# srv902/FOCUS

Hardware: AMD Instinct MI355X
Metric: clips/sec (fwd+bwd+opt step) ORViT-MF 16x224 (higher is better)
Workload: dtype bf16; 1 GPU; ORViT-Motionformer 16x224, 4 objects, batch=8 per GPU (BASELINE configs[1]); global_batch=8, frames=16, crop=224, objects=4, parallelism=dp1, optimizer=adamw+clipnorm

## Files before the change

### focus_amd/csrc/misc.hip

```cpp
#include "focus_common.h"
#include "focus_debug.h"

namespace {

template <typename T>
__global__ __launch_bounds__(256) void colsum_kernel(const T* __restrict__ x, float* __restrict__ out, int M, int N,
                                                     int64_t ld_, int rows_per_block, int accumulate) {
    __shared__ float red[4][64];
    const int c = blockIdx.x * 64 + (threadIdx.x & 63), r4 = threadIdx.x >> 6;
    const int m_begin = blockIdx.y * rows_per_block;
    const int m_end = min(M, m_begin + rows_per_block);
    float s = 0.f;
    if (c < N)
        for (int m = m_begin + r4; m < m_end; m += 4) s += ld<T>(x + (int64_t)m * ld_ + c);
    red[r4][threadIdx.x & 63] = s;
    __syncthreads();
    if (r4 == 0 && c < N) {
        const int l = threadIdx.x;
        const float t = red[0][l] + red[1][l] + red[2][l] + red[3][l];
        if (gridDim.y == 1 && !accumulate) out[c] = t; else atomicAdd(out + c, t);
    }
}

__global__ __launch_bounds__(256) void colsum_bf16_vec_kernel(const bf16_t* __restrict__ x, float* __restrict__ out,
// ... 118 lines not shown
                                                      const int64_t* __restrict__ target,
                                                      float* __restrict__ loss_rows, float* __restrict__ dlogits, int R,
                                                      int Ncls, float smoothing) {
    __shared__ float red[16];
    const int r = blockIdx.x;
    const float* x = logits + (int64_t)r * Ncls;
    float m = -INFINITY;
    for (int i = threadIdx.x; i < Ncls; i += 256) m = fmaxf(m, x[i]);
    m = block_max(m, red);
    float s = 0.f, sx = 0.f;
    for (int i = threadIdx.x; i < Ncls; i += 256) { s += expf(x[i] - m); sx += x[i]; }
    s = block_sum(s, red);
    sx = block_sum(sx, red);
    const float lse = m + logf(s);
    const int t = (int)target[r];
    const float conf = 1.f - smoothing;
    if (threadIdx.x == 0) {
        const float nll = lse - x[t];
        const float smooth = lse - sx / (float)Ncls;
        loss_rows[r] = conf * nll + smoothing * smooth;
    }
    for (int i = threadIdx.x; i < Ncls; i += 256) {
        const float p = expf(x[i] - lse);
        dlogits[(int64_t)r * Ncls + i] = (p - (i == t ? conf : 0.f) - smoothing / (float)Ncls) / (float)R;
    }
}

__device__ __forceinline__ float sigm(float x) { return 1.f / (1.f + expf(-x)); }
template <typename T>
__global__ void gru_fwd_kernel(T* __restrict__ gi, T* __restrict__ gh, const T* __restrict__ h, T* __restrict__ hn,
                               const float* __restrict__ b_ih, const float* __restrict__ b_hh, int R, int D) {
    const int64_t i = (int64_t)blockIdx.x * blockDim.x + threadIdx.x;
    if (i >= (int64_t)R * D) return;
    const int64_t r = i / D;
    const int c = (int)(i % D);
    T* a = gi + r * 3 * D;
    T* b = gh + r * 3 * D;
    float ar = ld<T>(a + c), az = ld<T>(a + D + c), an = ld<T>(a + 2 * D + c);
    float br = ld<T>(b + c), bz = ld<T>(b + D + c), bn = ld<T>(b + 2 * D + c);
    if (b_ih) {
        ar += b_ih[c]; az += b_ih[D + c]; an += b_ih[2 * D + c];
        br += b_hh[c]; bz += b_hh[D + c]; bn += b_hh[2 * D + c];
        st<T>(a + c, ar); st<T>(a + D + c, az); st<T>(a + 2 * D + c, an);
        st<T>(b + c, br); st<T>(b + D + c, bz); st<T>(b + 2 * D + c, bn);
        ar = ld<T>(a + c); az = ld<T>(a + D + c); an = ld<T>(a + 2 * D + c);
        br = ld<T>(b + c); bz = ld<T>(b + D + c); bn = ld<T>(b + 2 * D + c);
    }
    const float rg = sigm(ar + br);
    const float zg = sigm(az + bz);
    const float ng = tanhf(an + rg * bn);
    st<T>(hn + i, (1.f - zg) * ng + zg * ld<T>(h + i));
}
template <typename T>
__global__ void gru_bwd_kernel(const T* __restrict__ gi, const T* __restrict__ gh, const T* __restrict__ h,
                               const T* __restrict__ dhn, T* __restrict__ dgi, T* __restrict__ dgh,
                               T* __restrict__ dh, T* __restrict__ zero_out, int R, int D) {
    const int64_t i = (int64_t)blockIdx.x * blockDim.x + threadIdx.x;
    if (i >= (int64_t)R * D) return;
    if (zero_out) st<T>(zero_out + i, 0.f);
    const int64_t r = i / D;
    const int c = (int)(i % D);
    const T* a = gi + r * 3 * D;
    const T* b = gh + r * 3 * D;
    const float hn_ = ld<T>(b + 2 * D + c);
    const float rg = sigm(ld<T>(a + c) + ld<T>(b + c));
    const float zg = sigm(ld<T>(a + D + c) + ld<T>(b + D + c));
    const float ng = tanhf(ld<T>(a + 2 * D + c) + rg * hn_);
    const float hv = ld<T>(h + i), g = ld<T>(dhn + i);
    const float dn = g * (1.f - zg), dz = g * (hv - ng);
    const float dpre_n = dn * (1.f - ng * ng);
    const float dr = dpre_n * hn_;
    const float dpre_r = dr * rg * (1.f - rg), dpre_z = dz * zg * (1.f - zg);
    st<T>(dgi + r * 3 * D + c, dpre_r);
    st<T>(dgi + r * 3 * D + D + c, dpre_z);
    st<T>(dgi + r * 3 * D + 2 * D + c, dpre_n);
    st<T>(dgh + r * 3 * D + c, dpre_r);
    st<T>(dgh + r * 3 * D + D + c, dpre_z);
    st<T>(dgh + r * 3 * D + 2 * D + c, dpre_n * rg);
    st<T>(dh + i, g * zg);
}

template <typename T>
__global__ void cell_amax_fwd_kernel(const T* __restrict__ x, T* __restrict__ y, int32_t* __restrict__ arg, int K,
                                     int cells, int C) {
    const int64_t i = (int64_t)blockIdx.x * blockDim.x + threadIdx.x;
    if (i >= (int64_t)K * C) return;
    const int64_t k = i / C;
    const int c = (int)(i % C);
    const T* p = x + k * cells * C + c;
    float m = ld<T>(p);
    int a = 0;
    for (int j = 1; j < cells; ++j) {
        const float v = ld<T>(p + (int64_t)j * C);
        if (v > m) { m = v; a = j; }
    }
    st<T>(y + i, m);
    arg[i] = a;
}
__global__ __launch_bounds__(256) void cell_amax_fwd_vec_kernel(const bf16_t* __restrict__ x, bf16_t* __restrict__ y,
                                                                int32_t* __restrict__ arg, int cells, int C) {
    __shared__ float sm[8][256];
    __shared__ int sa[8][256];
    const int k = blockIdx.y, cb = blockIdx.x * 256;
    const int cg = threadIdx.x & 31, ph = threadIdx.x >> 5;
    const bf16_t* p = x + (int64_t)k * cells * C + cb + cg * 8;
    float m[8];
    int a[8];
#pragma unroll
    for (int e = 0; e < 8; ++e) { m[e] = -INFINITY; a[e] = 0x7fffffff; }
#pragma unroll 5
    for (int j = ph; j < cells; j += 8) {
        const uint4 r = *reinterpret_cast<const uint4*>(p + (int64_t)j * C);
        const float v[8] = {__uint_as_float(r.x << 16), __uint_as_float(r.x & 0xffff0000u), __uint_as_float(r.y << 16),
                            __uint_as_float(r.y & 0xffff0000u), __uint_as_float(r.z << 16), __uint_as_float(r.z & 0xffff0000u),
                            __uint_as_float(r.w << 16), __uint_as_float(r.w & 0xffff0000u)};
#pragma unroll
        for (int e = 0; e < 8; ++e)
            if (v[e] > m[e] || a[e] == 0x7fffffff) { m[e] = v[e]; a[e] = j; }
    }
#pragma unroll
    for (int e = 0; e < 8; ++e) { sm[ph][cg * 8 + e] = m[e]; sa[ph][cg * 8 + e] = a[e]; }
    __syncthreads();
    const int c = threadIdx.x;
    float bm = sm[0][c];
    int ba = sa[0][c];
#pragma unroll
    for (int q = 1; q < 8; ++q) {
        const float vm = sm[q][c];
        const int va = sa[q][c];
        if (va != 0x7fffffff && (ba == 0x7fffffff || vm > bm || (vm == bm && va < ba))) { bm = vm; ba = va; }
    }
    y[(int64_t)k * C + cb + c] = f32_to_bf16(bm);
    arg[(int64_t)k * C + cb + c] = ba == 0x7fffffff ? 0 : ba;
}
template <typename T>
__global__ void cell_amax_bwd_kernel(const T* __restrict__ dy, const int32_t* __restrict__ arg, T* __restrict__ dx,
                                     int K, int cells, int C) {
    const int64_t i = (int64_t)blockIdx.x * blockDim.x + threadIdx.x;
    if (i >= (int64_t)K * cells * C) return;
    const int c = (int)(i % C);
    const int j = (int)((i / C) % cells);
    const int64_t k = i / ((int64_t)C * cells);
    st<T>(dx + i, arg[k * C + c] == j ? ld<T>(dy + k * C + c) : 0.f);
}
__global__ __launch_bounds__(256) void cell_amax_bwd_vec_kernel(const bf16_t* __restrict__ dy, const int32_t* __restrict__ arg,
                                                                bf16_t* __restrict__ dx, int64_t n8, int cells, int C) {
    const int64_t i = (int64_t)blockIdx.x * 256 + threadIdx.x;
    if (i >= n8) return;
    const int c8 = C >> 3;
    const int cg = (int)(i % c8);
    const int j = (int)((i / c8) % cells);
    const int64_t k = i / ((int64_t)c8 * cells);
    const int4 a0 = *reinterpret_cast<const int4*>(arg + k * C + cg * 8);
    const int4 a1 = *reinterpret_cast<const int4*>(arg + k * C + cg * 8 + 4);
    const uint4 g = *reinterpret_cast<const uint4*>(dy + k * C + cg * 8);
    uint4 o;
    o.x = (a0.x == j ? (g.x & 0x0000ffffu) : 0u) | (a0.y == j ? (g.x & 0xffff0000u) : 0u);
    o.y = (a0.z == j ? (g.y & 0x0000ffffu) : 0u) | (a0.w == j ? (g.y & 0xffff0000u) : 0u);
    o.z = (a1.x == j ? (g.z & 0x0000ffffu) : 0u) | (a1.y == j ? (g.z & 0xffff0000u) : 0u);
    o.w = (a1.z == j ? (g.w & 0x0000ffffu) : 0u) | (a1.w == j ? (g.w & 0xffff0000u) : 0u);
    *reinterpret_cast<uint4*>(dx + i * 8) = o;
}

inline unsigned nblk(int64_t n, int per) { return (unsigned)cdiv64(n, per); }

}

#define DISPATCH_T(dtype, EXPR_T)                       \
    do {                                                \
        if ((dtype) == FOCUS_BF16) { typedef bf16_t T; EXPR_T; } \
        else { typedef float T; EXPR_T; }               \
    } while (0)

extern "C" int focus_colsum(const void* x, float* out, int M, int N, int64_t row_stride, int accumulate, int dtype,
                            void* stream) {
    if (!x || !out) return FOCUS_ERR_NULL;
    if (M <= 0 || N <= 0) return FOCUS_OK;
    hipStream_t s = (hipStream_t)stream;
    const bool vec = dtype == FOCUS_BF16 && (N & 7) == 0 && (row_stride & 7) == 0 && focus_aligned(x, 16);
    const bool small = (int64_t)M * N <= (4 << 20);
    const bool one_strip = small || M <= (vec ? 512 : 256);
    if (!accumulate && !one_strip && hipMemsetAsync(out, 0, sizeof(float) * N, s) != hipSuccess) return FOCUS_ERR_LAUNCH;
    if (vec) {
        const int rpb = one_strip ? M : 512;
        hipLaunchKernelGGL(colsum_bf16_vec_kernel, dim3((N + 255) / 256, (M + rpb - 1) / rpb), dim3(256), 0, s,
                           (const bf16_t*)x, out, M, N, row_stride, rpb, accumulate);
        FOCUS_CHECK_LAUNCH();
        return FOCUS_OK;
    }
    const int rpb = one_strip ? M : 256;
    dim3 grid((N + 63) / 64, (M + rpb - 1) / rpb);
    DISPATCH_T(dtype, hipLaunchKernelGGL((colsum_kernel<T>), grid, dim3(256), 0, s, (const T*)x, out, M, N,
                                         row_stride, rpb, accumulate));
    FOCUS_CHECK_LAUNCH();
    return FOCUS_OK;
}

__global__ __launch_bounds__(256) void shadow_refresh_kernel(const focus_shadow_item* __restrict__ items) {
    __shared__ bf16_t tile[64][68];
    const focus_shadow_item it = items[blockIdx.y];
    const int tiles_c = (it.cols + 63) >> 6, tiles_r = (it.rows + 63) >> 6;
    if ((int)blockIdx.x >= tiles_r * tiles_c) return;
    const int tr = blockIdx.x / tiles_c, tc = blockIdx.x - tr * tiles_c;
    const int t = threadIdx.x, lr = t >> 4, lc = (t & 15) * 4;
    bf16_t* dst = static_cast<bf16_t*>(it.dst);
    bf16_t* dstT = static_cast<bf16_t*>(it.dstT);
#pragma unroll
    for (int k = 0; k < 4; ++k) {
        const int r = tr * 64 + lr + 16 * k, c = tc * 64 + lc;
        uint2 o = make_uint2(0, 0);
        if (r < it.rows && c < it.cols) {
            const float4 v = *reinterpret_cast<const float4*>(it.src + (int64_t)r * it.cols + c);
            o.x = (uint32_t)f32_to_bf16(v.x) | ((uint32_t)f32_to_bf16(v.y) << 16);
            o.y = (uint32_t)f32_to_bf16(v.z) | ((uint32_t)f32_to_bf16(v.w) << 16);
            if (dst) *reinterpret_cast<uint2*>(dst + (int64_t)r * it.cols + c) = o;
        }
        *reinterpret_cast<uint2*>(&tile[lr + 16 * k][lc]) = o;
    }
    if (!dstT) return;
    __syncthreads();
#pragma unroll
    for (int k = 0; k < 4; ++k) {
        const int oc = tc * 64 + lr + 16 * k, orr = tr * 64 + lc;
        if (oc < it.cols && orr < it.rows) {
            uint2 o;
            o.x = (uint32_t)tile[lc + 0][lr + 16 * k] | ((uint32_t)tile[lc + 1][lr + 16 * k] << 16);
            o.y = (uint32_t)tile[lc + 2][lr + 16 * k] | ((uint32_t)tile[lc + 3][lr + 16 * k] << 16);
            *reinterpret_cast<uint2*>(dstT + (int64_t)oc * it.rows + orr) = o;
        }
    }
}

extern "C" int focus_shadow_refresh(const focus_shadow_item* items, int n_items, int max_rows, int max_cols, void* stream) {
    if (!items) return FOCUS_ERR_NULL;
    if (n_items <= 0) return FOCUS_OK;
    if (n_items > 65535 || max_rows <= 0 || max_cols <= 0) return FOCUS_ERR_SHAPE;
    const int tiles = ((max_rows + 63) / 64) * ((max_cols + 63) / 64);
    hipLaunchKernelGGL(shadow_refresh_kernel, dim3(tiles, n_items), dim3(256), 0, (hipStream_t)stream, items);
// ... 29 lines not shown
    dim3 grid((Cc + 63) / 64, (unsigned)cdiv64(dst_ld, 64), batch);
    if (grid.y > 65535) return FOCUS_ERR_SHAPE;
#define TP(TS, TD) hipLaunchKernelGGL((transpose_pad_kernel<TS, TD>), grid, dim3(256), 0, s, (const TS*)src, src_ld, src_bs, (TD*)dst, dst_ld, dst_bs, R, Cc)
    if (sd == FOCUS_F32 && dd == FOCUS_F32) TP(float, float);
    else if (sd == FOCUS_F32 && dd == FOCUS_BF16) TP(float, bf16_t);
    else if (sd == FOCUS_BF16 && dd == FOCUS_BF16) TP(bf16_t, bf16_t);
    else TP(bf16_t, float);
#undef TP
    FOCUS_CHECK_LAUNCH();
    return FOCUS_OK;
}

extern "C" int focus_diag_gather(const void* xt, void* xdiag, int B, int S, int F, int C, int dtype, void* stream) {
    if (!xt || !xdiag) return FOCUS_ERR_NULL;
    if ((C & 3) || F <= 0 || S % F) return FOCUS_ERR_SHAPE;
    const int64_t rows = (int64_t)B * S;
    DISPATCH_T(dtype, hipLaunchKernelGGL((diag_gather_kernel<T>), dim3(nblk(rows * C / 4, 256)), dim3(256), 0,
                                         (hipStream_t)stream, (const T*)xt, (T*)xdiag, rows, S, F, S / F, C));
    FOCUS_CHECK_LAUNCH();
    return FOCUS_OK;
}
extern "C" int focus_diag_scatter_add(const void* dxdiag, void* dxt, int B, int S, int F, int C, int dtype,
                                      void* stream) {
    if (!dxdiag || !dxt) return FOCUS_ERR_NULL;
    if ((C & 3) || F <= 0 || S % F) return FOCUS_ERR_SHAPE;
    const int64_t rows = (int64_t)B * S;
    DISPATCH_T(dtype, hipLaunchKernelGGL((diag_scatter_add_kernel<T>), dim3(nblk(rows * C / 4, 256)), dim3(256), 0,
                                         (hipStream_t)stream, (const T*)dxdiag, (T*)dxt, rows, S, F, S / F, C));
    FOCUS_CHECK_LAUNCH();
    return FOCUS_OK;
}

extern "C" int focus_im2col_patches(const float* x, void* cols, int B, int Cin, int Tn, int H, int W, int kt, int kh,
                                    int kw, int dtype, void* stream) {
    if (!x || !cols) return FOCUS_ERR_NULL;
    if (kt <= 0 || kh <= 0 || kw <= 0 || Tn % kt || H % kh || W % kw || (kw & 3) || (W & 3)) return FOCUS_ERR_SHAPE;
    if (!focus_aligned(x, 16)) return FOCUS_ERR_ALIGN;
    const int64_t total = (int64_t)B * (Tn / kt) * (H / kh) * (W / kw) * Cin * kt * kh * kw / 4;
    DISPATCH_T(dtype, hipLaunchKernelGGL((im2col_kernel<T>), dim3(nblk(total, 256)), dim3(256), 0,
                                         (hipStream_t)stream, x, (T*)cols, B, Cin, Tn, H, W, kt, kh, kw));
    FOCUS_CHECK_LAUNCH();
    return FOCUS_OK;
}

extern "C" int focus_embed_assemble(const void* patch, const float* cls, const float* pos, const float* temp,
                                    void* tokens, int B, int Tn, int P, int C, int dtype, void* stream) {
    if (!patch || !cls || !pos || !temp || !tokens) return FOCUS_ERR_NULL;
    if (C & 3) return FOCUS_ERR_SHAPE;
    const int64_t total = (int64_t)B * (1 + (int64_t)Tn * P) * C / 4;
    DISPATCH_T(dtype, hipLaunchKernelGGL((embed_assemble_kernel<T>), dim3(nblk(total, 256)), dim3(256), 0,
                                         (hipStream_t)stream, (const T*)patch, cls, pos, temp, (T*)tokens, B, Tn, P, C));
    FOCUS_CHECK_LAUNCH();
    return FOCUS_OK;
}

extern "C" int focus_xent_ls(const float* logits, const int64_t* target, float* loss_rows, float* dlogits, int R,
                             int Ncls, float smoothing, void* stream) {
    if (!logits || !target || !loss_rows || !dlogits) return FOCUS_ERR_NULL;
    if (R <= 0 || Ncls <= 0) return FOCUS_ERR_SHAPE;
    hipLaunchKernelGGL(xent_ls_kernel, dim3(R), dim3(256), 0, (hipStream_t)stream, logits, target, loss_rows, dlogits,
                       R, Ncls, smoothing);
    FOCUS_CHECK_LAUNCH();
    return FOCUS_OK;
}

extern "C" int focus_gru_gates_fwd(void* gi, void* gh, const void* h, void* hn, const float* b_ih, const float* b_hh, int R,
                                   int D, int dtype, void* stream) {
    if (!gi || !gh || !h || !hn || (!b_ih != !b_hh)) return FOCUS_ERR_NULL;
    DISPATCH_T(dtype, hipLaunchKernelGGL((gru_fwd_kernel<T>), dim3(nblk((int64_t)R * D, 256)), dim3(256), 0,
                                         (hipStream_t)stream, (T*)gi, (T*)gh, (const T*)h, (T*)hn, b_ih, b_hh, R, D));
    FOCUS_CHECK_LAUNCH();
    return FOCUS_OK;
}
extern "C" int focus_gru_gates_bwd(const void* gi, const void* gh, const void* h, const void* dhn, void* dgi,
                                   void* dgh, void* dh, void* zero_out, int R, int D, int dtype, void* stream) {
    if (!gi || !gh || !h || !dhn || !dgi || !dgh || !dh) return FOCUS_ERR_NULL;
    DISPATCH_T(dtype, hipLaunchKernelGGL((gru_bwd_kernel<T>), dim3(nblk((int64_t)R * D, 256)), dim3(256), 0,
                                         (hipStream_t)stream, (const T*)gi, (const T*)gh, (const T*)h, (const T*)dhn,
                                         (T*)dgi, (T*)dgh, (T*)dh, (T*)zero_out, R, D));
    FOCUS_CHECK_LAUNCH();
    return FOCUS_OK;
}

extern "C" int focus_cell_amax_fwd(const void* x, void* y, int32_t* arg, int K, int cells, int C, int dtype,
                                   void* stream) {
    if (!x || !y || !arg) return FOCUS_ERR_NULL;
    if (cells <= 0) return FOCUS_ERR_SHAPE;
    if (K <= 0) return FOCUS_OK;
    if (dtype == FOCUS_BF16 && (C & 255) == 0 && K <= 65535 && focus_aligned(x, 16)) {
        hipLaunchKernelGGL(cell_amax_fwd_vec_kernel, dim3(C / 256, K), dim3(256), 0, (hipStream_t)stream, (const bf16_t*)x,
                           (bf16_t*)y, arg, cells, C);
        FOCUS_CHECK_LAUNCH();
        return FOCUS_OK;
    }
    DISPATCH_T(dtype, hipLaunchKernelGGL((cell_amax_fwd_kernel<T>), dim3(nblk((int64_t)K * C, 256)), dim3(256), 0,
                                         (hipStream_t)stream, (const T*)x, (T*)y, arg, K, cells, C));
    FOCUS_CHECK_LAUNCH();
    return FOCUS_OK;
}
extern "C" int focus_cell_amax_bwd(const void* dy, const int32_t* arg, void* dx, int K, int cells, int C, int dtype,
                                   void* stream) {
    if (!dy || !arg || !dx) return FOCUS_ERR_NULL;
    if (K <= 0 || cells <= 0) return FOCUS_OK;
    if (dtype == FOCUS_BF16 && (C & 7) == 0 && focus_aligned(dy, 16) && focus_aligned(dx, 16) && focus_aligned(arg, 16)) {
        const int64_t n8 = (int64_t)K * cells * (C >> 3);
        hipLaunchKernelGGL(cell_amax_bwd_vec_kernel, dim3(nblk(n8, 256)), dim3(256), 0, (hipStream_t)stream,
                           (const bf16_t*)dy, arg, (bf16_t*)dx, n8, cells, C);
        FOCUS_CHECK_LAUNCH();
        return FOCUS_OK;
    }
    DISPATCH_T(dtype, hipLaunchKernelGGL((cell_amax_bwd_kernel<T>), dim3(nblk((int64_t)K * cells * C, 256)),
                                         dim3(256), 0, (hipStream_t)stream, (const T*)dy, arg, (T*)dx, K, cells, C));
    FOCUS_CHECK_LAUNCH();
    return FOCUS_OK;
}

template <typename T>
__global__ void scale_add_kernel(const T* __restrict__ x, const T* __restrict__ y, const float* __restrict__ scale,
                                 float keep, T* __restrict__ out, int64_t total, int64_t per) {
    const int64_t i = ((int64_t)blockIdx.x * blockDim.x + threadIdx.x) * 8;
    if (i >= total) return;
    float sc = scale[i / per];
    if (keep > 0.f) sc = __fdiv_rn(floorf(__fadd_rn(keep, sc)), keep);
    float a[8] = {0.f, 0.f, 0.f, 0.f, 0.f, 0.f, 0.f, 0.f}, b[8];
    ld8<T>(y + i, b);
    if (x) ld8<T>(x + i, a);
#pragma unroll
    for (int e = 0; e < 8; ++e) a[e] += sc * b[e];
    st8<T>(out + i, a);
}
extern "C" int focus_scale_add(const void* x, const void* y, const float* scale, float keep, void* out, int B,
                               int64_t per, int dtype, void* stream) {
    if (!y || !scale || !out) return FOCUS_ERR_NULL;
    if (B <= 0 || per <= 0) return FOCUS_OK;
    if (per & 7) return FOCUS_ERR_SHAPE;
    if (!focus_aligned(y, 16) || !focus_aligned(out, 16) || (x && !focus_aligned(x, 16))) return FOCUS_ERR_ALIGN;
    const int64_t total = (int64_t)B * per;
    DISPATCH_T(dtype, hipLaunchKernelGGL((scale_add_kernel<T>), dim3(nblk(total / 8, 256)), dim3(256), 0,
                                         (hipStream_t)stream, (const T*)x, (const T*)y, scale, keep, (T*)out, total, per));
    FOCUS_CHECK_LAUNCH();
    return FOCUS_OK;
}

typedef __attribute__((ext_vector_type(4))) short s16x4;
__global__ void tr16_probe_kernel(int16_t* out) {
    __shared__ __attribute__((aligned(16))) int16_t img[16 * 64];
    for (int i = threadIdx.x; i < 16 * 64; i += 64) img[i] = (int16_t)(100 * (i / 64) + (i % 64));
    __syncthreads();
    const int l = threadIdx.x, g = l >> 4, q = (l & 15) >> 2, pp = l & 3;
    auto* ptr = (__attribute__((address_space(3))) s16x4*)(img + (4 * g + q) * 64 + 4 * pp);
    const s16x4 v = __builtin_amdgcn_ds_read_tr16_b64_v4i16(ptr);
    for (int i = 0; i < 4; ++i) out[l * 4 + i] = v[i];
}
extern "C" int focus_debug_tr16_probe(int16_t* out, void* stream) {
    if (!out) return FOCUS_ERR_NULL;
    hipLaunchKernelGGL(tr16_probe_kernel, dim3(1), dim3(64), 0, (hipStream_t)stream, out);
    FOCUS_CHECK_LAUNCH();
    return FOCUS_OK;
}

static const char* kErr[] = {"ok", "bad shape", "unsupported dtype", "misaligned pointer or stride",
                             "HIP launch failure", "null pointer", "workspace too small"};
extern "C" const char* focus_strerror(int status) {
    const int i = -status;
    return (i >= 0 && i <= 6) ? kErr[i] : "unknown focus status";
}
extern "C" int focus_abi_version(void) { return 2; }
```

### focus_amd/csrc/orvit_tokens.hip

```cpp
#include "focus_common.h"

namespace {

struct RowMap { int b, t, p; bool cls; };
__device__ __forceinline__ RowMap map_all_row(int64_t r, int T, int HW, int O) {
    const int per = 1 + T * (HW + O);
    RowMap m;
    m.b = (int)(r / per);
    const int lr = (int)(r - (int64_t)m.b * per);
    m.cls = lr == 0;
    m.t = m.cls ? 0 : (lr - 1) / (HW + O);
    m.p = m.cls ? 0 : (lr - 1) - m.t * (HW + O);
    return m;
}

template <bool FWD>
__global__ __launch_bounds__(256) void orvit_assemble_kernel(const uint4* __restrict__ a, const uint4* __restrict__ o_in,
                                                             uint4* __restrict__ out_a, uint4* __restrict__ out_o, int64_t npieces,
                                                             int vpr, int T, int HW, int O) {
    const int64_t i = (int64_t)blockIdx.x * 256 + threadIdx.x;
    if (i >= npieces) return;
    const int64_t r = i / vpr;
    const int v = (int)(i - r * vpr);
    const RowMap m = map_all_row(r, T, HW, O);
    const int64_t xrow = (int64_t)m.b * (1 + T * HW) + (m.cls ? 0 : 1 + m.t * HW + m.p);
    const int64_t orow = ((int64_t)m.b * T + m.t) * O + (m.p - HW);
    const bool is_obj = !m.cls && m.p >= HW;
    if (FWD) out_a[i] = is_obj ? o_in[orow * vpr + v] : a[xrow * vpr + v];
    else if (is_obj) out_o[orow * vpr + v] = a[i];
    else out_a[xrow * vpr + v] = a[i];
}

template <typename T> struct Vec;
template <> struct Vec<float> { static constexpr int N = 4; };
template <> struct Vec<bf16_t> { static constexpr int N = 8; };
template <typename T> __device__ __forceinline__ void unpack(const uint4& r, float* v);
template <> __device__ __forceinline__ void unpack<float>(const uint4& r, float* v) {
    v[0] = __uint_as_float(r.x); v[1] = __uint_as_float(r.y); v[2] = __uint_as_float(r.z); v[3] = __uint_as_float(r.w);
}
template <> __device__ __forceinline__ void unpack<bf16_t>(const uint4& r, float* v) {
    v[0] = __uint_as_float(r.x << 16); v[1] = __uint_as_float(r.x & 0xffff0000u);
    v[2] = __uint_as_float(r.y << 16); v[3] = __uint_as_float(r.y & 0xffff0000u);
    v[4] = __uint_as_float(r.z << 16); v[5] = __uint_as_float(r.z & 0xffff0000u);
    v[6] = __uint_as_float(r.w << 16); v[7] = __uint_as_float(r.w & 0xffff0000u);
}
template <typename T> __device__ __forceinline__ uint4 pack(const float* v);
template <> __device__ __forceinline__ uint4 pack<float>(const float* v) {
    return make_uint4(__float_as_uint(v[0]), __float_as_uint(v[1]), __float_as_uint(v[2]), __float_as_uint(v[3]));
}
template <> __device__ __forceinline__ uint4 pack<bf16_t>(const float* v) {
    uint4 o;
    o.x = (uint32_t)f32_to_bf16(v[0]) | ((uint32_t)f32_to_bf16(v[1]) << 16);
    o.y = (uint32_t)f32_to_bf16(v[2]) | ((uint32_t)f32_to_bf16(v[3]) << 16);
    o.z = (uint32_t)f32_to_bf16(v[4]) | ((uint32_t)f32_to_bf16(v[5]) << 16);
    o.w = (uint32_t)f32_to_bf16(v[6]) | ((uint32_t)f32_to_bf16(v[7]) << 16);
    return o;
}

template <typename T>
__global__ __launch_bounds__(256) void orvit_merge_kernel(const uint4* __restrict__ x, const uint4* __restrict__ y,
                                                          const uint4* __restrict__ mm, const float* __restrict__ scale,
                                                          uint4* __restrict__ out, int64_t npieces, int vpr, int Tn, int HW,
                                                          int O) {
    const int64_t i = (int64_t)blockIdx.x * 256 + threadIdx.x;
    if (i >= npieces) return;
    const int64_t r = i / vpr;
    const int v = (int)(i - r * vpr);
    const int per = 1 + Tn * HW;
    const int b = (int)(r / per), lr = (int)(r - (int64_t)b * per);
    const int t = lr ? (lr - 1) / HW : 0, p = lr ? (lr - 1) - t * HW : 0;
    const int64_t yrow = (int64_t)b * (1 + Tn * (HW + O)) + (lr ? 1 + t * (HW + O) + p : 0);
    constexpr int N = Vec<T>::N;
    float xv[N], yv[N];
    unpack<T>(x[i], xv);
    unpack<T>(y[yrow * vpr + v], yv);
    if (mm && lr) {
        float mv[N];
        unpack<T>(mm[((int64_t)b * Tn * HW + (lr - 1)) * vpr + v], mv);
#pragma unroll
        for (int e = 0; e < N; ++e) yv[e] += mv[e];
    }
    const float s = scale ? scale[b] : 1.f;
#pragma unroll
    for (int e = 0; e < N; ++e) xv[e] = fmaf(s, yv[e], xv[e]);
    out[i] = pack<T>(xv);
}

template <typename T>
__global__ __launch_bounds__(256) void orvit_merge_bwd_kernel(const uint4* __restrict__ dout, const float* __restrict__ scale,
                                                              uint4* __restrict__ dy, uint4* __restrict__ dmm, int64_t npieces,
                                                              int vpr, int Tn, int HW, int O) {
    const int64_t i = (int64_t)blockIdx.x * 256 + threadIdx.x;
    if (i >= npieces) return;
    const int64_t r = i / vpr;
    const int v = (int)(i - r * vpr);
    const RowMap m = map_all_row(r, Tn, HW, O);
    if (!m.cls && m.p >= HW) { dy[i] = make_uint4(0, 0, 0, 0); return; }
    const int lr = m.cls ? 0 : 1 + m.t * HW + m.p;
    uint4 g = dout[((int64_t)m.b * (1 + Tn * HW) + lr) * vpr + v];
    if (scale) {
        constexpr int N = Vec<T>::N;
        float gv[N];
        unpack<T>(g, gv);
        const float s = scale[m.b];
#pragma unroll
        for (int e = 0; e < N; ++e) gv[e] *= s;
        g = pack<T>(gv);
    }
    dy[i] = g;
    if (dmm && lr) dmm[((int64_t)m.b * Tn * HW + (lr - 1)) * vpr + v] = g;
}

inline int64_t cdiv(int64_t a, int64_t b) { return (a + b - 1) / b; }
inline int esize(int dtype) { return dtype == FOCUS_BF16 ? 2 : 4; }
inline bool shape_ok(int B, int T, int HW, int O, int C, int dtype) {
    return B > 0 && T > 0 && HW > 0 && O >= 0 && C > 0 && (dtype == FOCUS_BF16 || dtype == FOCUS_F32) && (C * esize(dtype)) % 16 == 0 &&
           (int64_t)B * (1 + (int64_t)T * (HW + O)) * C < (1LL << 40);
}

}

extern "C" int focus_orvit_assemble(const void* x, const void* obj, void* all, int B, int T, int HW, int O, int C, int dtype,
                                    void* stream) {
    if (!x || !all || (O > 0 && !obj)) return FOCUS_ERR_NULL;
    if (!shape_ok(B, T, HW, O, C, dtype)) return FOCUS_ERR_SHAPE;
    if (!focus_aligned(x, 16) || !focus_aligned(all, 16) || (obj && !focus_aligned(obj, 16))) return FOCUS_ERR_ALIGN;
    const int vpr = C * esize(dtype) / 16;
    const int64_t n = (int64_t)B * (1 + (int64_t)T * (HW + O)) * vpr;
    hipLaunchKernelGGL((orvit_assemble_kernel<true>), dim3((unsigned)cdiv(n, 256)), dim3(256), 0, (hipStream_t)stream,
                       (const uint4*)x, (const uint4*)obj, (uint4*)all, (uint4*)nullptr, n, vpr, T, HW, O);
    FOCUS_CHECK_LAUNCH();
    return FOCUS_OK;
}

extern "C" int focus_orvit_assemble_bwd(const void* dall, void* dx, void* dobj, int B, int T, int HW, int O, int C, int dtype,
                                        void* stream) {
    if (!dall || !dx || (O > 0 && !dobj)) return FOCUS_ERR_NULL;
    if (!shape_ok(B, T, HW, O, C, dtype)) return FOCUS_ERR_SHAPE;
    if (!focus_aligned(dall, 16) || !focus_aligned(dx, 16) || (dobj && !focus_aligned(dobj, 16))) return FOCUS_ERR_ALIGN;
    const int vpr = C * esize(dtype) / 16;
    const int64_t n = (int64_t)B * (1 + (int64_t)T * (HW + O)) * vpr;
    hipLaunchKernelGGL((orvit_assemble_kernel<false>), dim3((unsigned)cdiv(n, 256)), dim3(256), 0, (hipStream_t)stream,
                       (const uint4*)dall, (const uint4*)nullptr, (uint4*)dx, (uint4*)dobj, n, vpr, T, HW, O);
    FOCUS_CHECK_LAUNCH();
    return FOCUS_OK;
}

extern "C" int focus_orvit_merge(const void* x, const void* y, const void* mm, const float* scale, void* out, int B, int T,
                                 int HW, int O, int C, int dtype, void* stream) {
    if (!x || !y || !out) return FOCUS_ERR_NULL;
    if (!shape_ok(B, T, HW, O, C, dtype)) return FOCUS_ERR_SHAPE;
    if (!focus_aligned(x, 16) || !focus_aligned(y, 16) || !focus_aligned(out, 16) || (mm && !focus_aligned(mm, 16)))
        return FOCUS_ERR_ALIGN;
    const int vpr = C * esize(dtype) / 16;
    const int64_t n = (int64_t)B * (1 + (int64_t)T * HW) * vpr;
    const dim3 grid((unsigned)cdiv(n, 256));
    if (dtype == FOCUS_BF16)
        hipLaunchKernelGGL((orvit_merge_kernel<bf16_t>), grid, dim3(256), 0, (hipStream_t)stream, (const uint4*)x, (const uint4*)y,
                           (const uint4*)mm, scale, (uint4*)out, n, vpr, T, HW, O);
    else
        hipLaunchKernelGGL((orvit_merge_kernel<float>), grid, dim3(256), 0, (hipStream_t)stream, (const uint4*)x, (const uint4*)y,
                           (const uint4*)mm, scale, (uint4*)out, n, vpr, T, HW, O);
    FOCUS_CHECK_LAUNCH();
    return FOCUS_OK;
}

extern "C" int focus_orvit_merge_bwd(const void* dout, const float* scale, void* dy, void* dmm, int B, int T, int HW, int O,
                                     int C, int dtype, void* stream) {
    if (!dout || !dy) return FOCUS_ERR_NULL;
    if (!shape_ok(B, T, HW, O, C, dtype)) return FOCUS_ERR_SHAPE;
    if (!focus_aligned(dout, 16) || !focus_aligned(dy, 16) || (dmm && !focus_aligned(dmm, 16))) return FOCUS_ERR_ALIGN;
    const int vpr = C * esize(dtype) / 16;
    const int64_t n = (int64_t)B * (1 + (int64_t)T * (HW + O)) * vpr;
    const dim3 grid((unsigned)cdiv(n, 256));
    if (dtype == FOCUS_BF16)
        hipLaunchKernelGGL((orvit_merge_bwd_kernel<bf16_t>), grid, dim3(256), 0, (hipStream_t)stream, (const uint4*)dout, scale,
                           (uint4*)dy, (uint4*)dmm, n, vpr, T, HW, O);
    else
        hipLaunchKernelGGL((orvit_merge_bwd_kernel<float>), grid, dim3(256), 0, (hipStream_t)stream, (const uint4*)dout, scale,
                           (uint4*)dy, (uint4*)dmm, n, vpr, T, HW, O);
    FOCUS_CHECK_LAUNCH();
    return FOCUS_OK;
}
```

### focus_amd/csrc/traj_time2.hip

```cpp
#include "focus_common.h"
#include <cstdlib>
#include "traj_internal.h"

namespace {

typedef __attribute__((ext_vector_type(8))) __bf16 bf16x8;
typedef __attribute__((ext_vector_type(4))) float f32x4;

constexpr int CH = 64;
constexpr int TQ = 16;
constexpr int MAXH = 16;

union Pk4 { uint2 u; bf16_t e[4]; };

__device__ __forceinline__ void unpack8(const uint4& r, float* v) {
    v[0] = __uint_as_float(r.x << 16); v[1] = __uint_as_float(r.x & 0xffff0000u);
    v[2] = __uint_as_float(r.y << 16); v[3] = __uint_as_float(r.y & 0xffff0000u);
    v[4] = __uint_as_float(r.z << 16); v[5] = __uint_as_float(r.z & 0xffff0000u);
    v[6] = __uint_as_float(r.w << 16); v[7] = __uint_as_float(r.w & 0xffff0000u);
}
__device__ __forceinline__ uint4 pack8(const float* v) {
    uint4 o;
    o.x = (uint32_t)f32_to_bf16(v[0]) | ((uint32_t)f32_to_bf16(v[1]) << 16);
    o.y = (uint32_t)f32_to_bf16(v[2]) | ((uint32_t)f32_to_bf16(v[3]) << 16);
// ... 346 lines not shown
#pragma unroll
        for (int i = 0; i < NFR; ++i) {
            const int fi = min(w + 8 * i, FT - 1);
#pragma unroll
            for (int ks = 0; ks < 2; ++ks) xf[i][ks] = *reinterpret_cast<const bf16x8*>(sx + (16 * fi + col) * XP + (32 * ks + 8 * kg) * 2);
#pragma unroll
            for (int j = 0; j < QPF; ++j)
#pragma unroll
                for (int ks = 0; ks < 2; ++ks)
                    ub[i][j][ks] = *reinterpret_cast<const bf16x8*>(sU + (QPF * fi + j) * urow + hl * FWD_HP + (32 * ks + 8 * kg) * 2);
        }
        QFrag<NHW> qf;
        read_q(qf, k ^ 1);
        lds_barrier();
        asm volatile("s_waitcnt vmcnt(%0)" ::"n"(LG) : "memory");
        __builtin_amdgcn_sched_barrier(0);
        pin_pre(pre[k]);
        stash(pre[k], k);
        asm volatile("" ::: "memory");
        pin_pre(pre[k]);
        issue(pre[k], t + 4);
        if (it + 1 < niter) compute_u_tile<UPW, false>(wf, qf, sUb + (k ^ 1) * (TQ * urow), urow, heads, w, lane);
#pragma unroll
        for (int i = 0; i < NFR; ++i) {
            f32x4 acc[QPF];
#pragma unroll
            for (int j = 0; j < QPF; ++j) {
                acc[j] = (f32x4){0.f, 0.f, 0.f, 0.f};
#pragma unroll
                for (int ks = 0; ks < 2; ++ks)
                    acc[j] = __builtin_amdgcn_mfma_f32_16x16x32_bf16(xf[i][ks], ub[i][j][ks], acc[j], 0, 0, 0);
            }
            f32x4 v = acc[0];
#pragma unroll
            for (int j = 1; j < QPF; ++j)
                if ((4 * kg) / FT == j) v = acc[j];
            const int fi = w + 8 * i;
            const int jq = (4 * kg) / FT, f0 = (4 * kg) % FT;
            const int row = row0 + QPF * fi + jq;
            if (fi < FT && row < rows && col < heads) {
                float4 o = make_float4(v[0] * scale, v[1] * scale, v[2] * scale, v[3] * scale);
                *reinterpret_cast<float4*>(slab + (((int64_t)cc * rows + row) * heads + col) * FT + f0) = o;
            }
        }
        lds_barrier();
      }
    }
    asm volatile("s_waitcnt vmcnt(0)" ::: "memory");
}

template <int FT>
__global__ __launch_bounds__(256) void time2_softmax_kernel(const float* __restrict__ slab, float* __restrict__ attn2,
                                                            int64_t n, int nchunk) {
    const int64_t i = (int64_t)blockIdx.x * 256 + threadIdx.x;
    if (i >= n) return;
    float lg[FT];
#pragma unroll
    for (int f = 0; f < FT; ++f) lg[f] = 0.f;
#pragma unroll 4
    for (int c = 0; c < nchunk; ++c) {
        const float4* p = reinterpret_cast<const float4*>(slab + ((int64_t)c * n + i) * FT);
#pragma unroll
        for (int f4 = 0; f4 < FT / 4; ++f4) {
            const float4 v = p[f4];
            lg[4 * f4] += v.x; lg[4 * f4 + 1] += v.y; lg[4 * f4 + 2] += v.z; lg[4 * f4 + 3] += v.w;
        }
    }
    float m = -INFINITY;
#pragma unroll
    for (int f = 0; f < FT; ++f) m = fmaxf(m, lg[f]);
    float den = 0.f;
#pragma unroll
    for (int f = 0; f < FT; ++f) { lg[f] = __expf(lg[f] - m); den += lg[f]; }
    const float inv = 1.f / den;
    float4* o = reinterpret_cast<float4*>(attn2 + i * FT);
#pragma unroll
    for (int f4 = 0; f4 < FT / 4; ++f4)
        o[f4] = make_float4(lg[4 * f4] * inv, lg[4 * f4 + 1] * inv, lg[4 * f4 + 2] * inv, lg[4 * f4 + 3] * inv);
}

template <int FT>
__global__ __launch_bounds__(256) void time2_out_kernel(const bf16_t* __restrict__ xt, const float* __restrict__ attn2,
                                                        bf16_t* __restrict__ out, int64_t obs, int64_t ngroups, int S,
                                                        int heads) {
    const int64_t gi = (int64_t)blockIdx.x * 256 + threadIdx.x;
    const bool act = gi < ngroups;
    const int64_t g = act ? gi : ngroups - 1;
    const int gpr = heads * 8;
    const int row = (int)(g / gpr);
    const int cg = (int)(g - (int64_t)row * gpr);
    const int C = gpr * 8;
    uint4 xr[FT];
#pragma unroll
    for (int f = 0; f < FT; ++f) xr[f] = *reinterpret_cast<const uint4*>(xt + (((int64_t)row * FT + f) * C) + cg * 8);
    const float* arow = attn2 + ((int64_t)row * heads + (cg >> 3)) * FT;
    float o[8] = {0.f, 0.f, 0.f, 0.f, 0.f, 0.f, 0.f, 0.f};
#pragma unroll
    for (int f = 0; f < FT; ++f) {
        const float a = arow[f];
        float xv[8];
        unpack8(xr[f], xv);
#pragma unroll
        for (int e = 0; e < 8; ++e) o[e] = fmaf(a, xv[e], o[e]);
    }
    const int b = row / S, s = row - b * S;
    if (act) *reinterpret_cast<uint4*>(out + b * obs + (int64_t)s * C + cg * 8) = pack8(o);
}

template <int FT>
__global__ __launch_bounds__(256) void time2_dlg_kernel(const bf16_t* __restrict__ xt, const float* __restrict__ attn2,
                                                        const bf16_t* __restrict__ dout, int64_t dobs,
                                                        bf16_t* __restrict__ dl, bf16_t* __restrict__ gout, int rows,
                                                        int S, int HEADS, int RPB, float scale) {
    const int GPR = HEADS * 8, C = HEADS * CH;
    __shared__ float sdl[32][FT][MAXH];
    const int tid = threadIdx.x, rl = min(tid / GPR, RPB - 1), cg = tid - (tid / GPR) * GPR, h = cg >> 3;
    const int row_raw = blockIdx.x * RPB + rl;
    const bool act = row_raw < rows && tid < RPB * GPR;
    const int row = act ? row_raw : rows - 1;
    const int b = row / S, s = row - b * S;
    uint4 xr[FT];
#pragma unroll
    for (int f = 0; f < FT; ++f) xr[f] = *reinterpret_cast<const uint4*>(xt + (((int64_t)row * FT + f) * C) + cg * 8);
    float gv[8];
    unpack8(*reinterpret_cast<const uint4*>(dout + b * dobs + (int64_t)s * C + cg * 8), gv);
    const float* arow = attn2 + ((int64_t)row * HEADS + h) * FT;
    float a[FT], da[FT], dot = 0.f;
#pragma unroll
    for (int f = 0; f < FT; ++f) {
        a[f] = arow[f];
        float xv[8];
        unpack8(xr[f], xv);
        float p = 0.f;
#pragma unroll
        for (int e = 0; e < 8; ++e) p = fmaf(gv[e], xv[e], p);
        da[f] = sum8lanes(p);
        dot = fmaf(a[f], da[f], dot);
    }
    if (tid < RPB * GPR && (cg & 7) == 0) {
#pragma unroll
        for (int f = 0; f < FT; ++f) sdl[rl][f][h] = scale * a[f] * (da[f] - dot);
    }
    if (tid < RPB * GPR && cg < MAXH - HEADS) {
#pragma unroll
        for (int f = 0; f < FT; ++f) sdl[rl][f][HEADS + cg] = 0.f;
    }
    __syncthreads();
    if (act) {
        for (int pc = cg; pc < FT * 2; pc += GPR) {
            const int f = pc >> 1, h0 = (pc & 1) * 8;
            float v[8];
#pragma unroll
            for (int k = 0; k < 8; ++k) v[k] = sdl[rl][f][h0 + k];
            *reinterpret_cast<uint4*>(dl + ((int64_t)row * FT + f) * MAXH + h0) = pack8(v);
        }
    }
    float xv[FT][8];
#pragma unroll
    for (int f = 0; f < FT; ++f) unpack8(xr[f], xv[f]);
    for (int hh = 0; hh < HEADS; ++hh) {
        float g8[8] = {0.f, 0.f, 0.f, 0.f, 0.f, 0.f, 0.f, 0.f};
#pragma unroll
        for (int f = 0; f < FT; ++f) {
            const float d = sdl[rl][f][hh];
#pragma unroll
            for (int k = 0; k < 8; ++k) g8[k] = fmaf(d, xv[f][k], g8[k]);
        }
        if (act) *reinterpret_cast<uint4*>(gout + ((int64_t)hh * rows + row) * C + cg * 8) = pack8(g8);
    }
// ... 269 lines not shown
        QFrag<NHW> qf;
        read_q(qf, k ^ 1);
        lds_barrier();
        asm volatile("s_waitcnt vmcnt(%0)" ::"n"(NQP + 2 * NX) : "memory");
        __builtin_amdgcn_sched_barrier(0);
        pin_pq(pq[k]);
        stash_q(pq[k], k);
        asm volatile("" ::: "memory");
        pin_pq(pq[k]);
        issue_q(pq[k], t + 4);
        asm volatile("s_waitcnt vmcnt(%0)" ::"n"(2 * NQP + NX) : "memory");
        __builtin_amdgcn_sched_barrier(0);
        pin_d(dr[k]);
        if (it + 1 < niter) compute_u_tile<UPW, true>(wf, qf, smem + (k ^ 1) * (TQ * BWD_UROW), 0, heads, w, lane);
        uint4 o[NNT][2];
#pragma unroll
        for (int i = 0; i < NNT; ++i) {
            f32x4 acc[4];
#pragma unroll
            for (int mt = 0; mt < 4; ++mt) acc[mt] = (f32x4){0.f, 0.f, 0.f, 0.f};
#pragma unroll
            for (int ks = 0; ks < KS; ++ks) {
                const int jp = QPF >= 2 ? (kg & 1) + 2 * ks : 0;
                const bool keep = QPF >= 2 ? jp == j : kg < 2;
                bf16x8 bfr = dr[k].dl[i];
#pragma unroll
                for (int e = 0; e < 8; ++e) bfr[e] = keep ? bfr[e] : (__bf16)0.f;
#pragma unroll
                for (int mt = 0; mt < 4; ++mt)
                    acc[mt] = __builtin_amdgcn_mfma_f32_16x16x32_bf16(af[i][ks][mt].v, bfr, acc[mt], 0, 0, 0);
            }
            float dv[16], v[16];
            unpack8(*reinterpret_cast<const uint4*>(&dr[k].dout[i][0]), dv);
            unpack8(*reinterpret_cast<const uint4*>(&dr[k].dout[i][1]), dv + 8);
            const float av = dr[k].a[i];
#pragma unroll
            for (int mt = 0; mt < 4; ++mt)
#pragma unroll
                for (int r = 0; r < 4; ++r) v[4 * mt + r] = fmaf(av, dv[4 * mt + r], acc[mt][r]);
            o[i][0] = pack8(v);
            o[i][1] = pack8(v + 8);
            pin(o[i][0]); pin(o[i][1]);
        }
        asm volatile("" ::: "memory");
        pin_d(dr[k]);
        load_d(dr[k], t + 2);
#pragma unroll
        for (int i = 0; i < NNT; ++i) {
            const int nt = w + 8 * i;
            const int row = row0 + QPF * nt + j;
            if (nt < FT && row < rows) {
                uint4* dp = reinterpret_cast<uint4*>(dxt + ((int64_t)row * FT + f) * C + cc * CH + 16 * kg);
                dp[0] = o[i][0];
                dp[1] = o[i][1];
            }
        }
        lds_barrier();
      }
    }
    asm volatile("s_waitcnt vmcnt(0)" ::: "memory");
}

int spread_mode() {
    static const int v = getenv("FOCUS_T2_SPREAD") ? atoi(getenv("FOCUS_T2_SPREAD")) : 0;
    return v;
}

size_t time2_lds_fwd(int heads) { return (size_t)2 * TQ * fwd_urow(heads); }
size_t time2_lds_bwd() { return (size_t)2 * TQ * BWD_UROW; }

}

bool focus_traj_time2_ok(int F, int heads, int d, int dtype) {
    static const bool enabled = !(getenv("FOCUS_TIME2") && atoi(getenv("FOCUS_TIME2")) == 0);
    return enabled && dtype == FOCUS_BF16 && d == CH && heads >= 1 && heads <= MAXH && (F == 4 || F == 8 || F == 16) &&
           time2_lds_fwd(heads) <= 160 * 1024;
}

extern "C" size_t focus_traj_time2_workspace_bytes(int B, int S, int F, int heads, int d) {
    if (B <= 0 || S <= 0 || F <= 0 || heads <= 0 || d != CH) return 0;
    return (size_t)heads * B * heads * S * F * sizeof(float);
}

extern "C" int focus_traj_time2_fwd(const void* q2, const void* xt, const void* wkT, int64_t ldw, void* out,
                                    int64_t out_bstride, float* attn2, void* ws, size_t ws_bytes, int B, int S, int F,
                                    int heads, int d, int dtype, void* stream) {
    if (!q2 || !xt || !wkT || !out || !attn2 || !ws) return FOCUS_ERR_NULL;
    if (B <= 0 || S <= 0 || !focus_traj_time2_ok(F, heads, d, dtype)) return FOCUS_ERR_SHAPE;
    const int C = heads * CH;
    const int64_t rows = (int64_t)B * S;
    if (ldw < C || (ldw & 7) || (out_bstride & 7) || out_bstride < (int64_t)S * C || rows * F * C > 0x7fffffffLL * 8)
        return FOCUS_ERR_SHAPE;
    if (!focus_aligned(q2, 16) || !focus_aligned(xt, 16) || !focus_aligned(wkT, 16) || !focus_aligned(out, 16) ||
        !focus_aligned(ws, 16) || !focus_aligned(attn2, 16))
        return FOCUS_ERR_ALIGN;
    if (ws_bytes < focus_traj_time2_workspace_bytes(B, S, F, heads, d)) return FOCUS_ERR_WORKSPACE;
    hipStream_t s = (hipStream_t)stream;
    const int nchunk = C / CH;
    const float scale = 1.f / sqrtf((float)d);
    const int upw = (2 * heads + 7) / 8;
    static const bool staged_on = !(getenv("FOCUS_T2_LDS") && atoi(getenv("FOCUS_T2_LDS")) == 0);
    const bool staged = staged_on && F <= 8 && time2_lds_staged(heads, F) <= 160 * 1024;
    const size_t lds = staged ? time2_lds_staged(heads, F) : time2_lds_fwd(heads);
#define TL(FT, UPW) do { \
        if (staged) { \
            static bool once_s = (hipFuncSetAttribute((const void*)time2_logits_lds_kernel<FT, UPW>, hipFuncAttributeMaxDynamicSharedMemorySize, 160 * 1024) == hipSuccess); \
            (void)once_s; \
            hipLaunchKernelGGL((time2_logits_lds_kernel<FT, UPW>), dim3(256), dim3(512), lds, s, (const bf16_t*)q2, (const bf16_t*)xt, (const bf16_t*)wkT, ldw, (float*)ws, (int)rows, heads, scale, spread_mode()); \
            break; } \
        static bool once = (hipFuncSetAttribute((const void*)time2_logits_kernel<FT, UPW>, hipFuncAttributeMaxDynamicSharedMemorySize, 160 * 1024) == hipSuccess); \
        (void)once; \
        hipLaunchKernelGGL((time2_logits_kernel<FT, UPW>), dim3(256), dim3(512), lds, s, (const bf16_t*)q2, (const bf16_t*)xt, (const bf16_t*)wkT, ldw, (float*)ws, (int)rows, heads, scale, spread_mode()); } while (0)
#define TLU(FT) do { if (upw == 1) TL(FT, 1); else if (upw == 2) TL(FT, 2); else if (upw == 3) TL(FT, 3); else TL(FT, 4); } while (0)
    if (F == 8) TLU(8); else if (F == 4) TLU(4); else TLU(16);
#undef TLU
#undef TL
    FOCUS_CHECK_LAUNCH();
    const int64_t n = rows * heads;
#define TS(FT) hipLaunchKernelGGL((time2_softmax_kernel<FT>), dim3((unsigned)cdiv64(n, 256)), dim3(256), 0, s, (const float*)ws, attn2, n, nchunk)
    if (F == 8) TS(8); else if (F == 4) TS(4); else TS(16);
#undef TS
    FOCUS_CHECK_LAUNCH();
    const int64_t ng = rows * heads * 8;
    dim3 gv((unsigned)cdiv64(ng, 256));
#define TO(FT) hipLaunchKernelGGL((time2_out_kernel<FT>), gv, dim3(256), 0, s, (const bf16_t*)xt, attn2, (bf16_t*)out, out_bstride, ng, S, heads)
    if (F == 8) TO(8); else if (F == 4) TO(4); else TO(16);
#undef TO
    FOCUS_CHECK_LAUNCH();
    return FOCUS_OK;
}

extern "C" int focus_traj_time2_bwd(const void* q2, const void* xt, const void* wkT, int64_t ldw, const float* attn2,
                                    const void* dout, int64_t dout_bstride, void* dxt, void* g, void* dl, int B, int S,
                                    int F, int heads, int d, int dtype, void* stream) {
    if (!q2 || !xt || !wkT || !attn2 || !dout || !dxt || !g || !dl) return FOCUS_ERR_NULL;
    if (B <= 0 || S <= 0 || !focus_traj_time2_ok(F, heads, d, dtype)) return FOCUS_ERR_SHAPE;
    const int C = heads * CH;
    const int64_t rows = (int64_t)B * S;
    if (ldw < C || (ldw & 7) || (dout_bstride & 7) || dout_bstride < (int64_t)S * C || rows * F * C > 0x7fffffffLL * 8)
        return FOCUS_ERR_SHAPE;
    if (!focus_aligned(q2, 16) || !focus_aligned(xt, 16) || !focus_aligned(wkT, 16) || !focus_aligned(dout, 16) ||
        !focus_aligned(dxt, 16) || !focus_aligned(g, 16) || !focus_aligned(dl, 16))
        return FOCUS_ERR_ALIGN;
    hipStream_t s = (hipStream_t)stream;
    const int nchunk = C / CH;
    const float scale = 1.f / sqrtf((float)d);
    {
        const int gpr = heads * 8, rpb = 256 / gpr;
        dim3 gd((unsigned)cdiv64(rows, rpb));
#define TD(FT) hipLaunchKernelGGL((time2_dlg_kernel<FT>), gd, dim3(256), 0, s, (const bf16_t*)xt, attn2, (const bf16_t*)dout, dout_bstride, (bf16_t*)dl, (bf16_t*)g, (int)rows, S, heads, rpb, scale)
        if (F == 8) TD(8); else if (F == 4) TD(4); else TD(16);
#undef TD
        FOCUS_CHECK_LAUNCH();
    }
    const int upw = (2 * heads + 7) / 8;
    static const bool staged_on = !(getenv("FOCUS_T2_LDS") && atoi(getenv("FOCUS_T2_LDS")) == 0);
    const size_t lds_staged = time2_lds_bwd() + (size_t)2 * TQ * q_pitch(heads);
    const bool staged = staged_on && lds_staged <= 160 * 1024 && !(upw == 4 && F != 8);
    const size_t lds = staged ? lds_staged : time2_lds_bwd();
#define TB(FT, UPW) do { \
        if constexpr (!((UPW) == 4 && (FT) != 8)) if (staged) { \
            static bool once_s = (hipFuncSetAttribute((const void*)time2_dx_lds_kernel<FT, UPW>, hipFuncAttributeMaxDynamicSharedMemorySize, 160 * 1024) == hipSuccess); \
            (void)once_s; \
            hipLaunchKernelGGL((time2_dx_lds_kernel<FT, UPW>), dim3(256), dim3(512), lds, s, (const bf16_t*)q2, (const bf16_t*)wkT, ldw, attn2, (const bf16_t*)dl, (const bf16_t*)dout, dout_bstride, (bf16_t*)dxt, (int)rows, S, heads, spread_mode()); \
            break; } \
        static bool once = (hipFuncSetAttribute((const void*)time2_dx_kernel<FT, UPW>, hipFuncAttributeMaxDynamicSharedMemorySize, 160 * 1024) == hipSuccess); \
        (void)once; \
        hipLaunchKernelGGL((time2_dx_kernel<FT, UPW>), dim3(256), dim3(512), lds, s, (const bf16_t*)q2, (const bf16_t*)wkT, ldw, attn2, (const bf16_t*)dl, (const bf16_t*)dout, dout_bstride, (bf16_t*)dxt, (int)rows, S, heads, spread_mode()); } while (0)
#define TBU(FT) do { if (upw == 1) TB(FT, 1); else if (upw == 2) TB(FT, 2); else if (upw == 3) TB(FT, 3); else TB(FT, 4); } while (0)
    if (F == 8) TBU(8); else if (F == 4) TBU(4); else TBU(16);
#undef TBU
#undef TB
    FOCUS_CHECK_LAUNCH();
    return FOCUS_OK;
}
```

### focus_amd/csrc/traj_time2_gw.hip

```cpp
#include "focus_common.h"
#include <algorithm>

namespace {

typedef __attribute__((ext_vector_type(8))) __bf16 bf16x8;
typedef __attribute__((ext_vector_type(4))) short s16x4;
typedef __attribute__((ext_vector_type(4))) float f32x4;
typedef __attribute__((address_space(3))) s16x4 lds_s16x4;

constexpr int HD = 64, TR = 32;
constexpr int C_ = 768;
constexpr int NSUB = C_ / 128;
constexpr int GT_BYTES = TR * C_ * 2, QT_BYTES = TR * HD * 2, STAGE = GT_BYTES + QT_BYTES;

union Frag { bf16x8 v; s16x4 t[2]; uint4 u; };

__device__ __forceinline__ int offb(int row, int ch) { return 256 * row + 16 * (ch ^ (((row & 3) << 2) | ((row >> 2) & 3))); }

__device__ __forceinline__ bf16x8 tr_frag_g(const char* sub, int r0, int c0, int lane) {
    const int i = lane & 15, q = i >> 2, p = i & 3;
    const int ch = (c0 >> 3) + (p >> 1), bo = 8 * (p & 1);
    Frag f;
    f.t[0] = __builtin_amdgcn_ds_read_tr16_b64_v4i16((lds_s16x4*)(sub + offb(r0 + q, ch) + bo));
    f.t[1] = __builtin_amdgcn_ds_read_tr16_b64_v4i16((lds_s16x4*)(sub + offb(r0 + 4 + q, ch) + bo));
// ... 22 lines not shown

    bf16x8 wf[C_ / 32];
    {
        const bf16_t* wrow = wk + (int64_t)(h * HD + nbq * 16 + row16_) * wk_ld + kq_ * 8;
#pragma unroll
        for (int ks = 0; ks < C_ / 32; ++ks) wf[ks] = *reinterpret_cast<const bf16x8*>(wrow + ks * 32);
    }
    f32x4 accw[4][6];
#pragma unroll
    for (int a = 0; a < 4; ++a)
#pragma unroll
        for (int j = 0; j < 6; ++j) accw[a][j] = (f32x4){0.f, 0.f, 0.f, 0.f};
    asm volatile("s_waitcnt vmcnt(0)" ::: "memory");
#pragma unroll
    for (int ks = 0; ks < C_ / 32; ++ks) asm volatile("" : "+v"(wf[ks]));

    const uint32_t sm_a = lds_addr_of(smem);
    auto dma = [&](int t, int st) __attribute__((always_inline)) {
        const int64_t r0 = (int64_t)t * TR;
        const uint32_t base = sm_a + st * STAGE;
#pragma unroll
        for (int j = 0; j < 6; ++j) {
            const int p = w * 6 + j, sub = p >> 3, rg = p & 7;
            const int row = rg * 4 + (lane >> 4), pos = lane & 15;
            const int ch = pos ^ (((row & 3) << 2) | ((row >> 2) & 3));
            glds16(gh + (r0 + row) * C_ + sub * 128 + ch * 8, __builtin_amdgcn_readfirstlane(base + sub * 8192 + rg * 1024));
        }
        if (w < 4) {
            const int row = w * 8 + (lane >> 3);
            glds16(q2 + (r0 + row) * (int64_t)(heads * HD) + h * HD + (lane & 7) * 8,
                   __builtin_amdgcn_readfirstlane(base + GT_BYTES + w * 1024));
        }
    };
    if (t_begin >= t_end) return;
    dma(t_begin, 0);
    int st = 0;
    for (int t = t_begin; t < t_end; ++t) {
        const bool more = t + 1 < t_end;
        if (more) dma(t + 1, st ^ 1);
        if (more) { if (w < 4) asm volatile("s_waitcnt vmcnt(7)" ::: "memory"); else asm volatile("s_waitcnt vmcnt(6)" ::: "memory"); }
        else asm volatile("s_waitcnt vmcnt(0)" ::: "memory");
        __builtin_amdgcn_s_barrier();
        const char* gt = smem + st * STAGE;
        const char* qt = gt + GT_BYTES;
        int lane_o = lane;
        asm volatile("" : "+v"(lane_o));
        const int row16 = lane_o & 15, kq = lane_o >> 4;
        f32x4 accq = {0.f, 0.f, 0.f, 0.f};
#pragma unroll
        for (int ks = 0; ks < C_ / 32; ++ks) {
            const int col = ks * 32 + kq * 8;
            const bf16x8 af = *reinterpret_cast<const bf16x8*>(gt + (col >> 7) * 8192 + offb(mb * 16 + row16, (col & 127) >> 3));
            accq = __builtin_amdgcn_mfma_f32_16x16x32_bf16(af, wf[ks], accq, 0, 0, 0);
        }
        {
            bf16_t* o = dq2 + ((int64_t)t * TR + mb * 16 + kq * 4) * (heads * HD) + h * HD + nbq * 16 + row16;
#pragma unroll
            for (int r = 0; r < 4; ++r) o[(int64_t)r * (heads * HD)] = f32_to_bf16(accq[r]);
        }
#pragma unroll
        for (int j = 0; j < 6; ++j) {
            const int c = w * 96 + j * 16;
            const bf16x8 gb = tr_frag_g(gt + (c >> 7) * 8192, 8 * kq, c & 127, lane_o);
#pragma unroll
            for (int a = 0; a < 4; ++a) {
                const bf16x8 qa = tr_frag_q(qt, 8 * kq, a * 16, lane_o);
                accw[a][j] = __builtin_amdgcn_mfma_f32_16x16x32_bf16(qa, gb, accw[a][j], 0, 0, 0);
            }
        }
        asm volatile("s_waitcnt lgkmcnt(0)" ::: "memory");
        __builtin_amdgcn_s_barrier();
        st ^= 1;
    }
    float* out = slabs + ((int64_t)sp * heads * HD + h * HD) * C_;
#pragma unroll
    for (int a = 0; a < 4; ++a)
#pragma unroll
        for (int j = 0; j < 6; ++j)
#pragma unroll
            for (int r = 0; r < 4; ++r) out[(int64_t)(a * 16 + kq_ * 4 + r) * C_ + w * 96 + j * 16 + row16_] = accw[a][j][r];
}

__global__ __launch_bounds__(256) void time2_gw_reduce_kernel(const float* __restrict__ slabs, float* __restrict__ dwk, int64_t n4,
                                                              int splits) {
    const int64_t i = (int64_t)blockIdx.x * 256 + threadIdx.x;
    if (i >= n4) return;
    float4 s = reinterpret_cast<const float4*>(slabs)[i];
#pragma unroll 4
    for (int k = 1; k < splits; ++k) {
        const float4 v = reinterpret_cast<const float4*>(slabs)[(int64_t)k * n4 + i];
        s.x += v.x; s.y += v.y; s.z += v.z; s.w += v.w;
    }
    reinterpret_cast<float4*>(dwk)[i] = s;
}

int gw_splits(int R, int heads) {
    const int tiles = R / TR;
    return std::max(1, std::min(tiles, 256 / std::max(heads, 1)));
}

}

extern "C" int focus_traj_time2_gw_ok(int R, int heads, int d, int dtype) {
    return dtype == FOCUS_BF16 && d == HD && heads * d == C_ && R >= TR && R % TR == 0;
}

extern "C" size_t focus_traj_time2_gw_workspace_bytes(int R, int heads, int d) {
    if (!focus_traj_time2_gw_ok(R, heads, d, FOCUS_BF16)) return 0;
    return (size_t)gw_splits(R, heads) * C_ * C_ * sizeof(float);
}

extern "C" int focus_traj_time2_gw(const void* g, const void* q2, const void* wk, int64_t wk_ld, void* dq2, float* dwk, void* ws,
                                   size_t ws_bytes, int R, int heads, int d, int dtype, void* stream) {
    if (!g || !q2 || !wk || !dq2 || !dwk || !ws) return FOCUS_ERR_NULL;
    if (!focus_traj_time2_gw_ok(R, heads, d, dtype) || (wk_ld & 7)) return FOCUS_ERR_SHAPE;
    if (!focus_aligned(g, 16) || !focus_aligned(q2, 16) || !focus_aligned(wk, 16) || !focus_aligned(dwk, 16)) return FOCUS_ERR_ALIGN;
    if (ws_bytes < focus_traj_time2_gw_workspace_bytes(R, heads, d)) return FOCUS_ERR_WORKSPACE;
    hipStream_t s = static_cast<hipStream_t>(stream);
    const int splits = gw_splits(R, heads), tiles = R / TR;
    const int tps = (tiles + splits - 1) / splits;
    const int used = (tiles + tps - 1) / tps;
    auto k = time2_gw_kernel;
    const size_t lds = 2 * (size_t)STAGE;
    static bool once = (hipFuncSetAttribute((const void*)k, hipFuncAttributeMaxDynamicSharedMemorySize, lds) == hipSuccess);
    (void)once;
    hipLaunchKernelGGL(k, dim3(used, heads), dim3(512), lds, s, (const bf16_t*)g, (const bf16_t*)q2, (const bf16_t*)wk, wk_ld,
                       (bf16_t*)dq2, (float*)ws, R, heads, tps);
    FOCUS_CHECK_LAUNCH();
    const int64_t n4 = (int64_t)C_ * C_ / 4;
    hipLaunchKernelGGL(time2_gw_reduce_kernel, dim3((unsigned)cdiv64(n4, 256)), dim3(256), 0, s, (const float*)ws, dwk, n4, used);
    FOCUS_CHECK_LAUNCH();
    return FOCUS_OK;
}
```

### focus_amd/ops.py

```python
import ctypes
import weakref

import torch

from . import _lib
from ._lib import BF16, F32, GemmDesc

EPI_NONE, EPI_GELU, EPI_RELU, EPI_TANH = _lib.EPI_NONE, _lib.EPI_GELU, _lib.EPI_RELU, _lib.EPI_TANH
_DEPI = {EPI_GELU: _lib.EPI_DGELU, EPI_RELU: _lib.EPI_DRELU, EPI_TANH: _lib.EPI_DTANH}


def _dt(t):
    if t.dtype == torch.float32:
        return F32
    if t.dtype == torch.bfloat16:
        return BF16
    raise RuntimeError("focus_amd: unsupported dtype %s (float32 or bfloat16)" % t.dtype)


def _need_gpu(*ts):
    for t in ts:
        if t is not None and not t.is_cuda:
            raise RuntimeError("focus_amd: the hot path runs on the MI355X only (got a %s tensor); "
                               "there is no CPU fallback" % t.device)
# ... 33 lines not shown
    d.batch0, d.batch1 = batch
    (ta, oa), (tb, ob), (tc, oc) = A, B, C
    d.A, d.B, d.C = _p(ta, oa).value, _p(tb, ob).value, _p(tc, oc).value
    d.rsA, d.csA, d.bsA0, d.bsA1 = sA
    d.rsB, d.csB, d.bsB0, d.bsB1 = sB
    d.rsC, d.csC, d.bsC0, d.bsC1 = sC
    d.bias = bias.data_ptr() if bias is not None else None
    d.residual = (residual[0].data_ptr() + residual[1] * residual[0].element_size()) if residual is not None else None
    d.aux = (aux[0].data_ptr() + aux[1] * aux[0].element_size()) if aux is not None else None
    d.alpha = alpha
    d.accumulate = int(accumulate)
    d.epilogue = epilogue
    d.dtype_ab = _dt(ta)
    d.dtype_c = _dt(tc)
    if b_scale is not None:
        assert tb.dtype == torch.uint8 and ta.dtype == torch.bfloat16, "fp8 weights go with bf16 activations"
        d.dtype_b = _lib.FP8_E4M3
        d.b_scale = b_scale.data_ptr()
    else:
        assert ta.dtype == tb.dtype
    kind = _mfma_path(ta, sA, sB, K) if GEMM_TIMING is not None else None
    if kind:
        e0, e1 = torch.cuda.Event(enable_timing=True), torch.cuda.Event(enable_timing=True)
        e0.record()
        _lib.check(_lib.lib().focus_gemm(ctypes.byref(d), _stream()), "gemm")
        e1.record()
        if kind == "nt" and _lib.lib().focus_gemm_last_kernel() == 2:
            kind = "nt_ws8" if b_scale is not None else "nt_ws"
        GEMM_TIMING.append((2.0 * M * N * K * batch[0] * batch[1], e0, e1, kind, (M, N, K, batch[0] * batch[1], epilogue)))
        return
    _lib.check(_lib.lib().focus_gemm(ctypes.byref(d), _stream()), "gemm")


def mm_nt(a, b, bias=None, residual=None, aux=None, epilogue=EPI_NONE, out_dtype=None, alpha=1.0, out=None, b_scale=None):
    M, K = a.shape
    N = b.shape[0]
    c = out if out is not None else torch.empty(M, N, device=a.device, dtype=out_dtype or a.dtype)
    gemm(M, N, K, (a, 0), (a.stride(0), 1, 0, 0), (b, 0), (1, b.stride(0), 0, 0), (c, 0), (N, 1, 0, 0),
         bias=bias, residual=(residual, 0) if residual is not None else None,
         aux=(aux, 0) if aux is not None else None, alpha=alpha, epilogue=epilogue, b_scale=b_scale)
    return c


def mm_nn(a, b, aux=None, epilogue=EPI_NONE, alpha=1.0):
    M, K = a.shape
    N = b.shape[1]
    c = torch.empty(M, N, device=a.device, dtype=a.dtype)
    gemm(M, N, K, (a, 0), (a.stride(0), 1, 0, 0), (b, 0), (b.stride(0), 1, 0, 0), (c, 0), (N, 1, 0, 0),
         aux=(aux, 0) if aux is not None else None, epilogue=epilogue, alpha=alpha)
    return c


def transpose_pad(x, pad_to=64, dtype=None):
    R, Cc = x.shape
    Rp = (R + pad_to - 1) // pad_to * pad_to
    out = torch.empty(Cc, Rp, device=x.device, dtype=dtype or x.dtype)
    _lib.check(_lib.lib().focus_transpose_pad(_p(x), _dt(x), x.stride(0), 0, _p(out), _dt(out), Rp, 0, R, Cc, 1,
                                              _stream()), "transpose_pad")
    return out


def mm_tn(a, b):
    M, N = a.shape
    K = b.shape[1]
    if a.dtype == torch.bfloat16 and USE_TN_GEMM and N % 8 == 0 and K % 8 == 0 and N >= 8 and K >= 8:
        c = torch.empty(N, K, device=a.device, dtype=torch.float32)
        nb = _lib.lib().focus_gemm_tn_workspace_bytes(N, K, M)
        ws = torch.empty(nb // 4, device=a.device, dtype=torch.float32)
        gemm(N, K, M, (a, 0), (1, a.stride(0), 0, 0), (b, 0), (b.stride(0), 1, 0, 0), (c, 0), (K, 1, 0, 0),
             aux=(ws, 0))
    elif a.dtype == torch.bfloat16:
        at, bt = transpose_pad(a), transpose_pad(b)
        Mp = at.shape[1]
        c = torch.zeros(N, K, device=a.device, dtype=torch.float32)
        gemm(N, K, Mp, (at, 0), (Mp, 1, 0, 0), (bt, 0), (1, Mp, 0, 0), (c, 0), (K, 1, 0, 0), accumulate=True)
    else:
        c = torch.empty(N, K, device=a.device, dtype=torch.float32)
        gemm(N, K, M, (a, 0), (1, a.stride(0), 0, 0), (b, 0), (b.stride(0), 1, 0, 0), (c, 0), (K, 1, 0, 0))
    return c


import os as _os


def wgrad_async(dy, x, want_bias):
    dw, db = linear_wgrad(dy, x, want_bias)
    return dw, db, None


def linear_wgrad(dy, x, want_bias):
    M, N = dy.shape
    K = x.shape[1]
    ok = (dy.dtype == torch.bfloat16 and USE_TN_GEMM and N % 8 == 0 and K % 8 == 0 and N >= 8 and K >= 8
          and dy.stride(1) == 1 and x.stride(1) == 1 and dy.stride(0) % 8 == 0 and x.stride(0) % 8 == 0)
    if not ok:
        return mm_tn(dy, x), (colsum(dy) if want_bias else None)
    L = _lib.lib()
    dw = torch.empty(N, K, device=dy.device, dtype=torch.float32)
    db = torch.empty(N, device=dy.device, dtype=torch.float32) if want_bias else None
    nb = L.focus_linear_wgrad_workspace_bytes(N, K, M)
    ws = torch.empty(max(nb, 16) // 4, device=dy.device, dtype=torch.float32)
    if GEMM_TIMING is not None:
        e0, e1 = torch.cuda.Event(enable_timing=True), torch.cuda.Event(enable_timing=True)
        e0.record()
    _lib.check(L.focus_linear_wgrad(_p(dy), _p(x), _p(dw), _p(db) if want_bias else None, _p(ws), nb, M, N, K,
                                    dy.stride(0), x.stride(0), _dt(dy), _stream()), "linear_wgrad")
    if GEMM_TIMING is not None:
        e1.record()
        GEMM_TIMING.append((2.0 * M * N * K, e0, e1, "tn", (N, K, M, 1, 0)))
    return dw, db


def colsum(x):
    M, N = x.shape
    out = torch.empty(N, device=x.device, dtype=torch.float32)
    _lib.check(_lib.lib().focus_colsum(_p(x), _p(out), M, N, x.stride(0), 0, _dt(x), _stream()), "colsum")
    return out


def cast(x, dtype):
    if x.dtype == dtype:
        return x
    x = x.contiguous()
    out = torch.empty(x.shape, device=x.device, dtype=dtype)
    _lib.check(_lib.lib().focus_cast(_p(x), _dt(x), _p(out), _dt(out), x.numel(), _stream()), "cast")
    return out


_shadow_cache = {}
_shadow_gen = 0
_shadow_epoch = 0


def shadow_epoch():
    return _shadow_epoch


def invalidate_shadows():
    global _shadow_gen
    _shadow_gen += 1
    _refresh_shadows_batched()
    if _stacked:
        refresh_stacked()
    if _fp8_cache:
        refresh_fp8_shadows()


_shadow_tables = {}


def _refresh_shadows_batched():
    import numpy as np
    by_dev = {}
    for key, (ref, stamp, out) in list(_shadow_cache.items()):
        w = ref()
        if w is None or key[1] != torch.bfloat16 or w.dtype != torch.float32 or w.dim() != 2 or not w.is_cuda:
            continue
        if w.shape[0] % 4 or w.shape[1] % 4 or not w.is_contiguous() or w.data_ptr() % 16:
            continue
        by_dev.setdefault(w.device, {}).setdefault(id(w), [w, None, None])[2 if key[2] else 1] = (key, out)
    for dev, ws in by_dev.items():
        sig = tuple((i, e[0].data_ptr(), e[1][1].data_ptr() if e[1] else 0, e[2][1].data_ptr() if e[2] else 0)
                    for i, e in sorted(ws.items()))
        tab = _shadow_tables.get(dev)
        if tab is None or tab[0] != sig:
            rec = np.zeros((len(sig), 4), dtype=np.int64)
            mr = mc = 0
            for n, (i, sp, dp, tp) in enumerate(sig):
                w = ws[i][0]
                rec[n, 0], rec[n, 1], rec[n, 2] = sp, dp, tp
                rec[n, 3] = int(w.shape[0]) | (int(w.shape[1]) << 32)
                mr, mc = max(mr, w.shape[0]), max(mc, w.shape[1])
            tab = (sig, torch.from_numpy(rec).to(dev), mr, mc)
            _shadow_tables[dev] = tab
        with torch.cuda.device(dev):
            _lib.check(_lib.lib().focus_shadow_refresh(_p(tab[1]), len(sig), tab[2], tab[3], _stream()), "shadow_refresh")
        for e in ws.values():
            w = e[0]
            for slot in (e[1], e[2]):
                if slot is not None:
                    key, out = slot
                    _shadow_cache[key] = (_shadow_cache[key][0], (w._version, w.data_ptr(), _shadow_gen), out)


def cached_shadow(w, dtype, transposed):
    hit = _shadow_cache.get((id(w), dtype, transposed))
    if hit is not None and hit[0]() is w:
        return hit[2]
    return None


def shadows_written(entries):
    global _shadow_gen
    _shadow_gen += 1
    for w, dst, dstT in entries:
        for out, tr in ((dst, False), (dstT, True)):
            if out is None:
                continue
            key = (id(w), torch.bfloat16, tr)
            hit = _shadow_cache.get(key)
            if hit is not None and hit[2] is out:
                _shadow_cache[key] = (hit[0], (w._version, w.data_ptr(), _shadow_gen), out)
    if _stacked:
        refresh_stacked()
    if _fp8_cache:
        refresh_fp8_shadows()


def drop_caches():
    global _shadow_epoch
    _shadow_epoch += 1
    _shadow_cache.clear()
    _shadow_tables.clear()
    _stacked.clear()
    _fp8_cache.clear()
    _fp8_tables.clear()


def shadow(w, dtype, transposed=False):
    w = getattr(w, "_focus_base", w)
    if dtype == torch.float32 and not transposed:
        return w.detach()
    key = (id(w), dtype, transposed)
    hit = _shadow_cache.get(key)
    if hit is not None and hit[0]() is w and hit[1] == (w._version, w.data_ptr(), _shadow_gen):
        return hit[2]
    wd = w.detach()
    if transposed:
        N, K = wd.shape
        out = torch.empty(K, N, device=w.device, dtype=dtype)
        _lib.check(_lib.lib().focus_transpose_pad(_p(wd), _dt(wd), K, 0, _p(out), _dt(out), N, 0, N, K, 1, _stream()),
                   "shadow^T")
    else:
        out = cast(wd, dtype)
    global _shadow_epoch
    _shadow_epoch += 1
    _shadow_cache[key] = (weakref.ref(w, lambda _r, k=key: _shadow_cache.pop(k, None)),
                          (w._version, w.data_ptr(), _shadow_gen), out)
    return out


FP8_WEIGHTS = False
_FP8_MIN_ROWS = 1024
_fp8_cache = {}
_fp8_tables = {}


class fp8_weights:
    def __init__(self, on=True):
        self.on = bool(on)

    def __enter__(self):
        global FP8_WEIGHTS
        self.prev = FP8_WEIGHTS
        FP8_WEIGHTS = self.on
        return self

    def __exit__(self, *exc):
        global FP8_WEIGHTS
        FP8_WEIGHTS = self.prev
        return False


def fp8_ok(w, rows, dtype):
    w = getattr(w, "_focus_base", w)
    return (FP8_WEIGHTS and dtype == torch.bfloat16 and w.dim() == 2 and w.dtype == torch.float32 and w.is_cuda
            and rows >= _FP8_MIN_ROWS and w.shape[0] % 64 == 0 and w.shape[1] % 64 == 0 and w.is_contiguous()
            and w.data_ptr() % 16 == 0)


def _fp8_run(dev, entries):
    import numpy as np
    sig = tuple((e[2].data_ptr(), e[3].data_ptr(), e[4].data_ptr(), w.data_ptr()) for w, e in entries)
    tab = _fp8_tables.get(dev)
    if tab is None or tab[0] != sig:
        rec = np.zeros((len(entries), 5), dtype=np.int64)
        mr = mc = 0
        for n, (w, e) in enumerate(entries):
            rec[n, 0], rec[n, 1], rec[n, 2], rec[n, 3] = w.data_ptr(), e[2].data_ptr(), e[3].data_ptr(), e[4].data_ptr()
            rec[n, 4] = int(w.shape[0]) | (int(w.shape[1]) << 32)
            mr, mc = max(mr, w.shape[0]), max(mc, w.shape[1])
        tab = (sig, torch.from_numpy(rec).to(dev), mr, mc, torch.empty(len(entries), dtype=torch.int32, device=dev))
        if len(entries) > 1:
            _fp8_tables[dev] = tab
    with torch.cuda.device(dev):
        _lib.check(_lib.lib().focus_fp8_refresh(_p(tab[1]), len(entries), tab[2], tab[3], _p(tab[4]), _stream()), "fp8_refresh")
    for w, e in entries:
        e[1] = (w._version, w.data_ptr(), _shadow_gen)


def refresh_fp8_shadows():
    by_dev = {}
    for key, e in list(_fp8_cache.items()):
        w = e[0]()
        if w is None:
            _fp8_cache.pop(key, None)
            continue
        by_dev.setdefault(w.device, []).append((w, e))
    for dev, entries in by_dev.items():
        _fp8_run(dev, entries)


def shadow_fp8(w, transposed=False):
    w = getattr(w, "_focus_base", w)
    e = _fp8_cache.get(id(w))
    if e is None or e[0]() is not w:
        N, K = w.shape
        e = _fp8_cache[id(w)] = [weakref.ref(w, lambda _r, k=id(w): _fp8_cache.pop(k, None)), None,
                                 torch.empty(N, K, dtype=torch.uint8, device=w.device),
                                 torch.empty(K, N, dtype=torch.uint8, device=w.device),
                                 torch.empty(1, dtype=torch.float32, device=w.device)]
        _fp8_tables.pop(w.device, None)
    if e[1] != (w._version, w.data_ptr(), _shadow_gen):
        _fp8_run(w.device, [(w.detach(), e)])
        e[1] = (w._version, w.data_ptr(), _shadow_gen)
    return (e[3] if transposed else e[2]), e[4]

# ... 843 lines not shown
        B, S, F_, C = xt.shape
        dout = dout.contiguous()
        dq2, dk2, dxt = torch.empty_like(q2), torch.empty_like(k2), torch.empty_like(xt)
        _lib.check(_lib.lib().focus_traj_time_bwd(_p(q2), _p(k2), _p(xt), _p(attn2), _p(dout), S * C, _p(dq2), _p(dk2),
                                                  _p(dxt), 0, B, S, F_, ctx.heads, C // ctx.heads, _dt(xt),
                                                  _stream()), "traj_time_bwd")
        return dq2, dk2, dxt, None


def traj_time(q2, k2, xt, heads):
    return _TrajTimeFn.apply(q2, k2, xt, heads)


class _TrajTimeBlockFn(torch.autograd.Function):

    @staticmethod
    def forward(ctx, q2, xt, w_kv, b_kv, cls_out, heads):
        _need_gpu(q2, xt, w_kv)
        q2, xt = q2.contiguous(), xt.contiguous()
        B, S, F_, C = xt.shape
        d = C // heads
        wk = shadow(w_kv, xt.dtype)[:C]
        bk = b_kv.detach()[:C] if b_kv is not None else None
        k2 = mm_nt(xt.view(-1, C), wk, bias=bk).view(B, S, F_, C)
        out = torch.empty(B, S + 1, C, device=xt.device, dtype=xt.dtype)
        out[:, 0].copy_(cls_out.reshape(B, C))
        attn2 = torch.empty(B, heads, S, F_, device=xt.device, dtype=torch.float32)
        _lib.check(_lib.lib().focus_traj_time_fwd(_p(q2), _p(k2), _p(xt), _p(out, C), (S + 1) * C, _p(attn2), B, S, F_,
                                                  heads, d, _dt(xt), _stream()), "traj_time_fwd")
        ctx.save_for_backward(q2, k2, xt, attn2, w_kv)
        ctx.heads, ctx.has_b, ctx.cls_shape = heads, b_kv is not None, cls_out.shape
        return out

    @staticmethod
    def backward(ctx, dcat):
        q2, k2, xt, attn2, w_kv = ctx.saved_tensors
        B, S, F_, C = xt.shape
        dcat = dcat.contiguous()
        dq2, dk2, dxt_a = torch.empty_like(q2), torch.empty_like(k2), torch.empty_like(xt)
        _lib.check(_lib.lib().focus_traj_time_bwd(_p(q2), _p(k2), _p(xt), _p(attn2), _p(dcat, C), (S + 1) * C, _p(dq2),
                                                  _p(dk2), _p(dxt_a), 0, B, S, F_, ctx.heads, C // ctx.heads, _dt(xt),
                                                  _stream()), "traj_time_bwd")
        dk2f, xt2 = dk2.view(-1, C), xt.view(-1, C)
        dw = db = dwk = dbk = None
        join = None
        if ctx.needs_input_grad[2]:
            dwk, dbk, join = wgrad_async(dk2f, xt2, ctx.has_b and ctx.needs_input_grad[3])
        dxt = None
        if ctx.needs_input_grad[1]:
            if xt.dtype == torch.bfloat16 and C % 64 == 0:
                wt = shadow(w_kv, xt.dtype, transposed=True)
                dxt = mm_nt(dk2f, wt[:, :C], residual=dxt_a.view(-1, C))
            else:
                dxt = mm_nn(dk2f, shadow(w_kv, xt.dtype)[:C]).add_(dxt_a.view(-1, C))
            dxt = dxt.view(B, S, F_, C)
        if join is not None:
            join()
        if dwk is not None:
            dw = torch.empty(2 * C, C, device=xt.device, dtype=torch.float32)
            dw[:C].copy_(dwk)
            dw[C:].zero_()
            if dbk is not None:
                db = torch.zeros(2 * C, device=xt.device, dtype=torch.float32)
                db[:C].copy_(dbk)
        dcls = dcat[:, :1].reshape(ctx.cls_shape) if ctx.needs_input_grad[4] else None
        return dq2, dxt, dw, db, dcls, None


def traj_time_block(q2, xt, w_kv, b_kv, cls_out, heads):
    return _TrajTimeBlockFn.apply(q2, xt, w_kv, b_kv, cls_out, heads)


class _TrajTime2BlockFn(torch.autograd.Function):

    @staticmethod
    def forward(ctx, q2, xt, w_kv, b_kv, cls_out, heads):
        _need_gpu(q2, xt, w_kv)
        q2, xt = q2.contiguous(), xt.contiguous()
        B, S, F_, C = xt.shape
        d = C // heads
        L = _lib.lib()
        wkT = shadow(w_kv, xt.dtype, transposed=True)
        out = torch.empty(B, S + 1, C, device=xt.device, dtype=xt.dtype)
        out[:, 0].copy_(cls_out.reshape(B, C))
        attn2 = torch.empty(B, S, heads, F_, device=xt.device, dtype=torch.float32)
        nb = L.focus_traj_time2_workspace_bytes(B, S, F_, heads, d)
        ws = torch.empty(nb // 4, device=xt.device, dtype=torch.float32)
        _lib.check(L.focus_traj_time2_fwd(_p(q2), _p(xt), _p(wkT), wkT.stride(0), _p(out, C), (S + 1) * C, _p(attn2),
                                          _p(ws), nb, B, S, F_, heads, d, _dt(xt), _stream()), "traj_time2_fwd")
        ctx.save_for_backward(q2, xt, attn2, w_kv)
        ctx.heads, ctx.has_b, ctx.cls_shape = heads, b_kv is not None, cls_out.shape
        return out

    @staticmethod
    def backward(ctx, dcat):
        q2, xt, attn2, w_kv = ctx.saved_tensors
        heads = ctx.heads
        B, S, F_, C = xt.shape
        d = C // heads
        dev = xt.device
        L = _lib.lib()
        dcat = dcat.contiguous()
        wkT = shadow(w_kv, xt.dtype, transposed=True)
        dxt = torch.empty_like(xt)
        g = torch.empty(heads, B * S, C, device=dev, dtype=xt.dtype)
        dl = torch.empty(B, S, F_, 16, device=dev, dtype=xt.dtype)
        _lib.check(L.focus_traj_time2_bwd(_p(q2), _p(xt), _p(wkT), wkT.stride(0), _p(attn2), _p(dcat, C), (S + 1) * C,
                                          _p(dxt), _p(g), _p(dl), B, S, F_, heads, d, _dt(xt), _stream()), "traj_time2_bwd")
        R = B * S
        dq2 = dw = db = None
        if (ctx.needs_input_grad[0] and ctx.needs_input_grad[2] and L.focus_traj_time2_gw_ok(R, heads, d, _dt(xt))
                and _os.environ.get("FOCUS_TIME2_GW", "1") != "0"):
            wk = shadow(w_kv, xt.dtype)
            dq2 = torch.empty(B, S, C, device=dev, dtype=xt.dtype)
            dw = torch.empty(2 * C, C, device=dev, dtype=torch.float32)
            nbw = L.focus_traj_time2_gw_workspace_bytes(R, heads, d)
            wsw = torch.empty(nbw // 4, device=dev, dtype=torch.float32)
            _lib.check(L.focus_traj_time2_gw(_p(g), _p(q2), _p(wk), wk.stride(0), _p(dq2), _p(dw), _p(wsw), nbw, R, heads, d,
                                             _dt(xt), _stream()), "traj_time2_gw")
            dw[C:].zero_()
            if ctx.has_b and ctx.needs_input_grad[3]:
                db = torch.zeros(2 * C, device=dev, dtype=torch.float32)
            dcls = dcat[:, :1].reshape(ctx.cls_shape) if ctx.needs_input_grad[4] else None
            return dq2, dxt, dw, db, dcls, None
        if ctx.needs_input_grad[0]:
            wk = shadow(w_kv, xt.dtype)
            dq2 = torch.empty(B, S, C, device=dev, dtype=xt.dtype)
            gemm(R, d, C, (g, 0), (C, 1, 0, R * C), (wk, 0), (1, C, 0, d * C), (dq2, 0), (C, 1, 0, d),
                 batch=(1, heads))
        if ctx.needs_input_grad[2]:
            dw = torch.empty(2 * C, C, device=dev, dtype=torch.float32)
            nbw = L.focus_gemm_tn_batched_workspace_bytes(d, C, R, heads)
            wsw = torch.empty(max(nbw, 16) // 4, device=dev, dtype=torch.float32)
            gemm(d, C, R, (q2, 0), (1, C, 0, d), (g, 0), (C, 1, 0, R * C), (dw, 0), (C, 1, 0, d * C),
                 batch=(1, heads), aux=(wsw, 0))
            dw[C:].zero_()
            if ctx.has_b and ctx.needs_input_grad[3]:
                db = torch.zeros(2 * C, device=dev, dtype=torch.float32)
        dcls = dcat[:, :1].reshape(ctx.cls_shape) if ctx.needs_input_grad[4] else None
        return dq2, dxt, dw, db, dcls, None


def traj_time2_ok(xt, heads):
    if _os.environ.get("FOCUS_TIME2", "1") == "0" or xt.dtype != torch.bfloat16:
        return False
    B, S, F_, C = xt.shape
    return C % heads == 0 and C // heads == 64 and heads <= 16 and F_ in (4, 8, 16)


def traj_time2_block(q2, xt, w_kv, b_kv, cls_out, heads):
    return _TrajTime2BlockFn.apply(q2, xt, w_kv, b_kv, cls_out, heads)


class _SmallAttnFn(torch.autograd.Function):

    @staticmethod
    def forward(ctx, q, k, v, heads, scale, causal, drop):
        _need_gpu(q, k, v)
        B, N, C = q.shape
        M = k.shape[1]
        d = C // heads
        dev, dt = q.device, q.dtype
        att = torch.empty(B, heads, N, M, device=dev, dtype=dt)
        L = _lib.lib()
        ctx.heads, ctx.scale = heads, scale

        def rows_ok(t):
            return t.stride(2) == 1 and t.stride(0) == t.shape[1] * t.stride(1) and t.stride(1) >= C

        ctx.fused = (not causal and drop is None and bool(L.focus_small_attn_ok(N, M, d))
                     and rows_ok(q) and rows_ok(k) and rows_ok(v))
        if ctx.fused:
            out = torch.empty(B, N, C, device=dev, dtype=dt)
            _lib.check(L.focus_small_attn_fwd(_p(q), _p(k), _p(v), q.stride(1), k.stride(1), v.stride(1), _p(att), _p(out), B,
                                              heads, N, M, d, scale, _dt(q), _stream()), "small_attn_fwd")
            ctx.save_for_backward(q, k, v, att, None)
            return out
        q, k, v = q.contiguous(), k.contiguous(), v.contiguous()
        sa = (M, 1, heads * N * M, N * M)
        gemm(N, M, d, (q, 0), (C, 1, N * C, d), (k, 0), (1, C, M * C, d), (att, 0), sa, batch=(B, heads))
        if causal:
            assert N == M, "causal self-attention"
            _lib.check(L.focus_softmax_causal_fwd(_p(att), _p(att), B * heads * N, M, M, N, scale, _dt(att), _stream()),
                       "softmax_causal_fwd")
        else:
            _lib.check(L.focus_softmax_fwd(_p(att), _p(att), B * heads * N, M, M, scale, _dt(att), _stream()),
                       "softmax_fwd")
        attd = att if drop is None else att * drop
        out = torch.empty(B, N, C, device=dev, dtype=dt)
        gemm(N, d, M, (attd, 0), sa, (v, 0), (C, 1, M * C, d), (out, 0), (C, 1, N * C, d), batch=(B, heads))
        ctx.save_for_backward(q, k, v, att, drop)
        return out

    @staticmethod
    def backward(ctx, dout):
        q, k, v, att, drop = ctx.saved_tensors
        heads, scale = ctx.heads, ctx.scale
        B, N, C = q.shape
        M = k.shape[1]
        d = C // heads
        dout = dout.contiguous()
        if ctx.fused:
            es = q.element_size()
            if (N == M and q.stride(1) == 3 * C == k.stride(1) == v.stride(1) and k.data_ptr() == q.data_ptr() + C * es
                    and v.data_ptr() == k.data_ptr() + C * es):
# ... 118 lines not shown
        if tok_T:
            B = feat.shape[0]
            assert feat.shape[1] == 1 + tok_T * H * W
            NI, ipb, bstride, off = B * tok_T, tok_T, (1 + tok_T * H * W) * C, C
        else:
            NI, HW, _ = feat.shape
            assert HW == H * W
            ipb, bstride, off = NI, NI * H * W * C, 0
        K = rois.shape[0]
        out = torch.empty(K, PH * PW, C, device=feat.device, dtype=feat.dtype)
        _lib.check(_lib.lib().focus_roi_align_fwd(_p(feat, off), H * W * C, ipb, bstride, _p(rois), _p(roi_img), _p(out), NI,
                                                  C, H, W, K, PH, PW, scale, sampling_ratio, int(aligned), int(relu),
                                                  _dt(feat), _stream()), "roi_align_fwd")
        ctx.relu = bool(relu)
        ctx.save_for_backward(rois, roi_img, out if relu else None)
        ctx.args = (NI, C, H, W, K, PH, PW, scale, sampling_ratio, int(aligned), feat.dtype, ipb, bstride, off, feat.shape)
        return out

    @staticmethod
    def backward(ctx, dout):
        rois, roi_img, relu_out = ctx.saved_tensors
        NI, C, H, W, K, PH, PW, scale, sr, al, dt, ipb, bstride, off, shp = ctx.args
        dout = dout.contiguous()
        L = _lib.lib()
        dfeat = torch.empty(shp, device=dout.device, dtype=dt)
        if off:
            dfeat[:, 0].zero_()
        nb = L.focus_roi_align_bwd_workspace_bytes(NI, C, H, W, PH, PW)
        ws = torch.empty(nb // 4, device=dout.device, dtype=torch.float32) if nb else None
        _lib.check(L.focus_roi_align_bwd(_p(dout), _p(relu_out), _p(rois), _p(roi_img), _p(dfeat, off), H * W * C, ipb, bstride,
                                         _p(ws), nb, NI, C, H, W, K, PH, PW, scale, sr, al, _dt(dout), _stream()),
                   "roi_align_bwd")
        return dfeat, None, None, None, None, None, None, None, None, None, None, None


def roi_align_tokens(feat, rois, roi_img, H, W, PH, PW, spatial_scale, sampling_ratio=-1, aligned=True):
    return _RoiAlignFn.apply(feat, rois, roi_img, 0, H, W, PH, PW, float(spatial_scale), sampling_ratio, aligned, False)


def roi_align_stream(x, rois, roi_img, T, H, W, PH, PW, spatial_scale, sampling_ratio=-1, aligned=True, relu=False):
    B, _, C = x.shape
    if _lib.lib().focus_roi_align_bwd_workspace_bytes(B * T, C, H, W, PH, PW):
        out = roi_align_tokens(x[:, 1:].reshape(B * T, H * W, C), rois, roi_img, H, W, PH, PW, spatial_scale,
                               sampling_ratio, aligned)
        return torch.relu(out) if relu else out
    return _RoiAlignFn.apply(x, rois, roi_img, T, H, W, PH, PW, float(spatial_scale), sampling_ratio, aligned, relu)


def roi_stream_supports_fused(x, T, H, W, PH, PW):
    B, _, C = x.shape
    return _lib.lib().focus_roi_align_bwd_workspace_bytes(B * T, C, H, W, PH, PW) == 0


class _OrvitAssembleFn(torch.autograd.Function):

    @staticmethod
    def forward(ctx, x, obj, T, HW):
        _need_gpu(x, obj)
        x, obj = x.contiguous(), obj.contiguous()
        B, _, C = x.shape
        O = obj.shape[2]
        assert x.shape[1] == 1 + T * HW and obj.shape[:2] == (B, T) and obj.dtype == x.dtype
        out = torch.empty(B, 1 + T * (HW + O), C, device=x.device, dtype=x.dtype)
        _lib.check(_lib.lib().focus_orvit_assemble(_p(x), _p(obj), _p(out), B, T, HW, O, C, _dt(x), _stream()),
                   "orvit_assemble")
        ctx.args = (B, T, HW, O, C)
        return out

    @staticmethod
    def backward(ctx, dall):
        B, T, HW, O, C = ctx.args
        dall = dall.contiguous()
        dx = torch.empty(B, 1 + T * HW, C, device=dall.device, dtype=dall.dtype)
        dobj = torch.empty(B, T, O, C, device=dall.device, dtype=dall.dtype)
        _lib.check(_lib.lib().focus_orvit_assemble_bwd(_p(dall), _p(dx), _p(dobj), B, T, HW, O, C, _dt(dall), _stream()),
                   "orvit_assemble_bwd")
        return dx, dobj, None, None


def orvit_assemble(x, obj, T, HW):
    return _OrvitAssembleFn.apply(x, obj, T, HW)


class _OrvitMergeFn(torch.autograd.Function):

    @staticmethod
    def forward(ctx, x, y, mm, draws, keep, T, HW):
        _need_gpu(x, y)
        x, y = x.contiguous(), y.contiguous()
        B, _, C = x.shape
        O = (y.shape[1] - 1) // T - HW
        assert y.shape[1] == 1 + T * (HW + O) and x.shape[1] == 1 + T * HW
        scale = None
        if draws is not None:
            scale = torch.floor(keep + draws) / keep
        if mm is not None:
            mm = mm.contiguous()
        out = torch.empty_like(x)
        _lib.check(_lib.lib().focus_orvit_merge(_p(x), _p(y), _p(mm) if mm is not None else None,
                                                _p(scale) if scale is not None else None, _p(out), B, T, HW, O, C, _dt(x),
                                                _stream()), "orvit_merge")
        ctx.scale = scale
        ctx.args = (B, T, HW, O, C, mm is not None)
        return out

    @staticmethod
    def backward(ctx, dout):
        B, T, HW, O, C, has_mm = ctx.args
        dout = dout.contiguous()
        dy = torch.empty(B, 1 + T * (HW + O), C, device=dout.device, dtype=dout.dtype)
        dmm = torch.empty(B, T * HW, C, device=dout.device, dtype=dout.dtype) if has_mm else None
        sc = ctx.scale
        _lib.check(_lib.lib().focus_orvit_merge_bwd(_p(dout), _p(sc) if sc is not None else None, _p(dy),
                                                    _p(dmm) if has_mm else None, B, T, HW, O, C, _dt(dout), _stream()),
                   "orvit_merge_bwd")
        return dout, dy, dmm, None, None, None, None


def orvit_merge(x, y, mm, T, HW, drop_prob=0.0, training=False):
    draws = None
    keep = 1.0 - drop_prob
    if drop_prob > 0.0 and training:
        draws = torch.rand(x.shape[0], dtype=torch.float32, device=x.device)
    return _OrvitMergeFn.apply(x, y, mm, draws, keep, T, HW)


def roi_align_indices(rois, H, W, PH, PW, spatial_scale, sampling_ratio=-1, aligned=True):
    _need_gpu(rois)
    K = rois.shape[0]
    grid = torch.empty(K, 2, device=rois.device, dtype=torch.int32)
    nbr = torch.empty(K, PH, PW, 4, device=rois.device, dtype=torch.int32)
    _lib.check(_lib.lib().focus_roi_align_indices(_p(rois), _p(grid), _p(nbr), H, W, K, PH, PW, float(spatial_scale),
                                                  sampling_ratio, int(aligned), _stream()), "roi_align_indices")
    return grid, nbr


class _CellAmaxFn(torch.autograd.Function):
    @staticmethod
    def forward(ctx, x):
        _need_gpu(x)
        x = x.contiguous()
        K, cells, C = x.shape
        y = torch.empty(K, C, device=x.device, dtype=x.dtype)
        arg = torch.empty(K, C, device=x.device, dtype=torch.int32)
        _lib.check(_lib.lib().focus_cell_amax_fwd(_p(x), _p(y), _p(arg), K, cells, C, _dt(x), _stream()), "cell_amax")
        ctx.save_for_backward(arg)
        ctx.cells = cells
        return y

    @staticmethod
    def backward(ctx, dy):
        (arg,) = ctx.saved_tensors
        K, C = arg.shape
        dy = dy.contiguous()
        dx = torch.empty(K, ctx.cells, C, device=dy.device, dtype=dy.dtype)
        _lib.check(_lib.lib().focus_cell_amax_bwd(_p(dy), _p(arg), _p(dx), K, ctx.cells, C, _dt(dy), _stream()),
                   "cell_amax_bwd")
        return dx


def cell_amax(x):
    return _CellAmaxFn.apply(x)


class _BoxLayoutFn(torch.autograd.Function):
    @staticmethod
    def forward(ctx, vecs, boxes, H, W):
        _need_gpu(vecs, boxes)
        vecs, boxes = vecs.contiguous(), boxes.contiguous().float()
        NF, O, C = vecs.shape
        out = torch.empty(NF, H * W, C, device=vecs.device, dtype=vecs.dtype)
        _lib.check(_lib.lib().focus_box_layout_fwd(_p(vecs), _p(boxes), _p(out), NF, O, C, H, W, _dt(vecs), _stream()),
                   "box_layout_fwd")
        ctx.save_for_backward(boxes)
        ctx.args = (NF, O, C, H, W)
        return out

    @staticmethod
    def backward(ctx, dout):
        (boxes,) = ctx.saved_tensors
        NF, O, C, H, W = ctx.args
        dout = dout.contiguous()
        dv = torch.empty(NF, O, C, device=dout.device, dtype=dout.dtype)
        _lib.check(_lib.lib().focus_box_layout_bwd(_p(dout), _p(boxes), _p(dv), NF, O, C, H, W, _dt(dout), _stream()),
                   "box_layout_bwd")
        return dv, None, None, None


def box_layout(vecs, boxes, H, W):
    return _BoxLayoutFn.apply(vecs, boxes, H, W)


def im2col_patches(x, kt, kh, kw, dtype):
    _need_gpu(x)
    x = x.contiguous().float()
    B, Cin, T, H, W = x.shape
    rows = B * (T // kt) * (H // kh) * (W // kw)
    cols = torch.empty(rows, Cin * kt * kh * kw, device=x.device, dtype=dtype)
    _lib.check(_lib.lib().focus_im2col_patches(_p(x), _p(cols), B, Cin, T, H, W, kt, kh, kw, _dt(cols), _stream()),
               "im2col")
    return cols


class _EmbedAssembleFn(torch.autograd.Function):
    @staticmethod
    def forward(ctx, patch, cls, pos, temp):
        _need_gpu(patch, cls, pos, temp)
        B, S, C = patch.shape
        T = temp.shape[0]
        P = S // T
        patch = patch.contiguous()
        tok = torch.empty(B, 1 + S, C, device=patch.device, dtype=patch.dtype)
        _lib.check(_lib.lib().focus_embed_assemble(_p(patch), _p(cls), _p(pos), _p(temp), _p(tok), B, T, P, C,
                                                   _dt(patch), _stream()), "embed_assemble")
        ctx.dims = (B, T, P, C)
        return tok

    @staticmethod
    def backward(ctx, dtok):
        B, T, P, C = ctx.dims
        g = dtok.float()
        gp = g[:, 1:].reshape(B, T, P, C)
        dcls = g[:, 0].sum(0)
        dpos = torch.cat([dcls[None], gp.sum((0, 1))], 0)
        dtemp = gp.sum((0, 2))
        return dtok[:, 1:], dcls, dpos, dtemp


def embed_assemble(patch, cls, pos, temp):
    return _EmbedAssembleFn.apply(patch, cls.contiguous(), pos.contiguous(), temp.contiguous())


def rows_ok(t):
    return (t.is_cuda and t.dim() == 2 and t.is_contiguous() and t.dtype in (torch.float32, torch.bfloat16)
            and t.data_ptr() % 16 == 0 and bool(_lib.lib().focus_rows_ok(t.shape[0], t.shape[1], _dt(t))))


class _XentLsFn(torch.autograd.Function):
    @staticmethod
    def forward(ctx, logits, target, smoothing):
        _need_gpu(logits, target)
        ctx.rows = rows_ok(logits)
        R, Ncls = logits.shape
        loss_rows = torch.empty(R, device=logits.device, dtype=torch.float32)
        if ctx.rows:
# ... 582 lines not shown
```

### focus_amd/slowfast/models/ORViT/orvit.py

```python
import torch
from torch import nn

from focus_amd import ops
from focus_amd.slowfast.models.attention import SeltAttentionBlock, TrajectoryAttention

from ..common import DropPath
from .utils import Mlp, ObjectsCrops, box2spatial_layout


import os

_SIDE_STREAMS = {}
_USE_SIDE_STREAM = os.environ.get("FOCUS_MOTION_SIDE_STREAM", "1") != "0"
_COMMUTE_PATCH_TO_D = os.environ.get("FOCUS_ORVIT_COMMUTE", "1") != "0"


def _side_stream(device):
    s = _SIDE_STREAMS.get(device)
    if s is None:
        s = _SIDE_STREAMS[device] = torch.cuda.Stream(device=device)
    return s


def _relu_pair(seq, x, dtype=None):
    hid = torch.relu(ops.linear(x.float(), seq[0].weight))
    if dtype is not None and dtype != hid.dtype:
        hid = hid.to(dtype)
    return torch.relu(ops.linear(hid, seq[2].weight))


class ORViT(nn.Module):
    def __init__(self, cfg, dim=768, dim_out=None, num_heads=12, attn_type="trajectory", mlp_ratio=4.0,
                 qkv_bias=False, drop=0.0, attn_drop=0.0, drop_path=0.0, act_layer=nn.GELU, norm_layer=nn.LayerNorm,
                 use_original_code=False, nb_frames=None):
        super().__init__()
        self.cfg = cfg
        self.in_dim = dim
        self.dim = dim
        self.nb_frames = nb_frames
        self.with_cls_token = True
        self.with_motion_stream = cfg.ORVIT.USE_MOTION_STREAM

        self.crop_layer = ObjectsCrops(cfg)
        self.patch_to_d = nn.Sequential(nn.Linear(dim, dim // 2, bias=False), nn.ReLU(inplace=True),
                                        nn.Linear(dim // 2, dim, bias=False), nn.ReLU())
        self.box_categories = nn.Parameter(torch.zeros(nb_frames, cfg.ORVIT.O, dim))
        self.c_coord_to_feature = nn.Sequential(nn.Linear(4, dim // 2, bias=False), nn.ReLU(inplace=True),
                                                nn.Linear(dim // 2, dim, bias=False), nn.ReLU())
        mlp_hidden_dim = int(dim * mlp_ratio)
        self.norm1 = norm_layer(dim)
        self.norm2 = norm_layer(dim)
        self.drop_path = DropPath(drop_path) if drop_path > 0.0 else nn.Identity()
        self.mlp = Mlp(in_features=dim, hidden_features=mlp_hidden_dim, act_layer=act_layer, drop=drop)
        self.attn = TrajectoryAttention(dim, num_heads=num_heads, qkv_bias=qkv_bias, attn_drop=attn_drop,
                                        proj_drop=drop)
        if self.with_motion_stream:
            self.motion_stream = MotionStream(cfg, dim=dim, num_heads=num_heads,
                                              attn_type=cfg.ORVIT.MOTION_STREAM_ATTN_TYPE, mlp_ratio=mlp_ratio,
                                              qkv_bias=qkv_bias, drop=drop, attn_drop=attn_drop, drop_path=drop_path,
                                              act_layer=act_layer, norm_layer=norm_layer, nb_frames=nb_frames)
            self.motion_mlp = Mlp(in_features=cfg.ORVIT.MOTION_STREAM_DIM if cfg.ORVIT.MOTION_STREAM_DIM > 0 else dim,
                                  hidden_features=mlp_hidden_dim, out_features=dim, act_layer=act_layer, drop=drop)
        if cfg.ORVIT.INIT_WEIGHTS:
            self.apply(self._init_weights)

    def _init_weights(self, m):
        if isinstance(m, nn.Linear):
            nn.init.trunc_normal_(m.weight, std=0.02)
            if m.bias is not None:
                nn.init.constant_(m.bias, 0)
        elif isinstance(m, nn.LayerNorm):
            nn.init.constant_(m.bias, 0)
            nn.init.constant_(m.weight, 1.0)
        else:
            for p in m.parameters():
                nn.init.normal_(p, std=0.02)

    def _linear_params(self):
        a, m, mm, p2d = self.attn, self.mlp, getattr(self, "motion_mlp", None), self.patch_to_d
        ps = [a.qkv.weight, a.qkv.bias, a.proj_q.weight, a.proj_q.bias, a.proj.weight, a.proj.bias,
              m.fc1.weight, m.fc1.bias, m.fc2.weight, m.fc2.bias, p2d[0].weight, p2d[2].weight]
        if mm is not None:
            ps += [mm.fc1.weight, mm.fc1.bias, mm.fc2.weight, mm.fc2.bias]
        return ps

    def forward(self, x, metadata, thw):
        with ops.wgrad_group(self._linear_params()):
            return self._forward(x, metadata, thw)

    def _forward(self, x, metadata, thw):
        box_tensors = metadata["orvit_bboxes"]
        assert box_tensors is not None
        BS, _, d = x.shape
        T, H, W = thw
        assert T == self.nb_frames
        Tratio = box_tensors.shape[1] // T
        box_tensors = box_tensors[:, ::Tratio].float()
        O = box_tensors.shape[-2]
        HW = H * W

        motion_emb, side = None, None
        if self.with_motion_stream:
            if x.is_cuda and _USE_SIDE_STREAM:
                main, side = torch.cuda.current_stream(), _side_stream(x.device)
                if torch.distributed.is_available() and torch.distributed.is_initialized():
                    from focus_amd import parallel
                    parallel.note_grad_stream(main)
                    parallel.note_grad_stream(side)
                side.wait_stream(main)
                box_tensors.record_stream(side)
                with torch.cuda.stream(side):
                    motion_emb = self.motion_stream(box_tensors, H, W, dtype=x.dtype)
            else:
                motion_emb = self.motion_stream(box_tensors, H, W, dtype=x.dtype)

        p2d = self.patch_to_d
        with ops.fp8_activations(False):
            if _COMMUTE_PATCH_TO_D:
                z = ops.linear(x, p2d[0].weight)
                crops = self.crop_layer.crop_stream(z, box_tensors, T, H, W, relu=True)
                pre = ops.linear(crops, p2d[2].weight)
            else:
                crops = self.crop_layer.crop_stream(x, box_tensors, T, H, W)
                pre = ops.mlp(crops, p2d[0].weight, None, p2d[2].weight, None, act=ops.EPI_RELU)
        obj = torch.relu(ops.cell_amax(pre)).view(BS, T, O, d)
        box_emb = _relu_pair(self.c_coord_to_feature, box_tensors, x.dtype)
        obj = obj + self.box_categories.to(x.dtype) + box_emb

        all_tokens = ops.orvit_assemble(x, obj, T, HW)
        n1 = self.norm1
        y, _ = self.attn(ops.layer_norm(all_tokens, n1.weight, n1.bias, n1.eps), [T, HW + O, 1])
        mm = None
        if self.with_motion_stream:
            if side is not None:
                torch.cuda.current_stream().wait_stream(side)
                motion_emb.record_stream(torch.cuda.current_stream())
            mm = self.motion_mlp(motion_emb)
        dp = 0.0 if isinstance(self.drop_path, nn.Identity) else self.drop_path.drop_prob
        x = ops.orvit_merge(x, y, mm, T, HW, dp, self.training)
        n2 = self.norm2
        xr, h = ops.layer_norm_fork(x, n2.weight, n2.bias, n2.eps)
        if dp == 0.0 or not self.training:
            x = self.mlp(h, residual=xr)
        else:
            x = ops.residual_drop_path(xr, self.mlp(h), dp, True)
        return x, thw


class Object2Spatial(nn.Module):
    def __init__(self, cfg, _type):
        super().__init__()
        self.cfg = cfg
        self._type = _type

    def forward(self, all_features, context, boxes, H, W, t_avg_pooling=False):
        BS, T, O, d = all_features.shape
        if self._type != "layout":
            raise NotImplementedError("%s: only the 'layout' mapping is used (orvit.py:252)" % self._type)
        ret = box2spatial_layout(boxes, all_features, H, W).permute(0, 2, 3, 4, 1)
        if t_avg_pooling:
            Tratio = int(T / self.cfg.MF.TEMPORAL_RESOLUTION)
            if Tratio > 1:
                ret = ret.reshape(BS, -1, Tratio, H, W, d).mean(2)
        return ret.flatten(1, 3)


class MotionStream(nn.Module):
    def __init__(self, cfg, dim=768, num_heads=12, attn_type="trajectory", mlp_ratio=4.0, qkv_bias=False, drop=0.0,
                 attn_drop=0.0, drop_path=0.0, act_layer=nn.GELU, norm_layer=nn.LayerNorm, nb_frames=None):
        super().__init__()
        self.cfg = cfg
        self.in_dim = cfg.ORVIT.MOTION_STREAM_DIM if cfg.ORVIT.MOTION_STREAM_DIM > 0 else dim
        self.dim = dim
        self.nb_frames = nb_frames
        if cfg.ORVIT.MOTION_STREAM_SEP_POS_EMB:
            self.box_categories_T = nn.Parameter(torch.zeros(nb_frames, 1, self.in_dim))
            self.box_categories_O = nn.Parameter(torch.zeros(1, cfg.ORVIT.O, self.in_dim))
        else:
            self.box_categories = nn.Parameter(torch.zeros(nb_frames, cfg.ORVIT.O, self.in_dim))
        self.c_coord_to_feature = nn.Sequential(nn.Linear(4, self.in_dim // 2, bias=False), nn.ReLU(inplace=True),
                                                nn.Linear(self.in_dim // 2, self.in_dim, bias=False), nn.ReLU())
        self.attn_type = attn_type
        if attn_type != "joint":
            raise NotImplementedError("ORVIT.MOTION_STREAM_ATTN_TYPE must be 'joint' (orvit.py:238)")
        self.attn = SeltAttentionBlock(dim=self.in_dim, num_heads=num_heads, mlp_ratio=mlp_ratio, qkv_bias=qkv_bias,
                                       drop_rate=attn_drop, drop_path=drop_path, act_layer=act_layer,
                                       norm_layer=norm_layer)
        self.obj2spatial = Object2Spatial(cfg, _type="layout")

    def forward(self, box_tensors, H, W, dtype=None):
        BS = box_tensors.shape[0]
        dtype = dtype or box_tensors.dtype
        box_emb = _relu_pair(self.c_coord_to_feature, box_tensors, dtype)
        if self.cfg.ORVIT.MOTION_STREAM_SEP_POS_EMB:
            shape = (self.nb_frames, self.cfg.ORVIT.O, self.in_dim)
            cat = self.box_categories_T.expand(shape) + self.box_categories_O.expand(shape)
        else:
            cat = self.box_categories
        box_emb = cat.to(dtype).unsqueeze(0) + box_emb
        oshape = box_emb.shape
        box_emb, _ = self.attn(box_emb.flatten(1, -2), None, None)
        box_emb = box_emb.reshape(oshape)
        return self.obj2spatial(box_emb, None, box_tensors, H, W, t_avg_pooling=True)
```

### focus_amd/slowfast/models/optimizer.py

```python
import os

import torch


class FusedAdamW(torch.optim.AdamW):

    def __init__(self, params, lr=1e-3, betas=(0.9, 0.999), eps=1e-8, weight_decay=1e-2):
        super().__init__(params, lr=lr, betas=betas, eps=eps, weight_decay=weight_decay, fused=False, foreach=False)
        self._table = None
        self._groups = None
        self._ws = None
        self.last_total_norm = None
        self.write_clipped_grads = True

    def load_state_dict(self, state_dict):
        super().load_state_dict(state_dict)
        self._table = None

    def _prepare(self):
        import numpy as np
        from focus_amd import _lib, ops
        L = _lib.lib()
        live = []
        for gi, group in enumerate(self.param_groups):
            if group.get("amsgrad") or group.get("maximize"):
                raise NotImplementedError("FusedAdamW: amsgrad / maximize are not built")
            for p in group["params"]:
                if p.grad is not None:
                    live.append((p, gi))
        if not live:
            return None
        dev = live[0][0].device
        ident = (tuple(id(p) for p, _ in live), ops.shadow_epoch())
        tab = self._table
        if tab is None or tab["ident"] != ident:
            n = len(live)
            for p, _ in live:
                if p.grad.is_sparse or p.dtype != torch.float32 or not p.is_cuda or not p.is_contiguous():
                    raise RuntimeError("FusedAdamW wants dense contiguous fp32 parameters on the GPU")
                st = self.state[p]
                if len(st) == 0:
                    st["step"] = torch.zeros((), dtype=torch.float32, device=p.device)
                    st["exp_avg"] = torch.zeros_like(p, memory_format=torch.preserve_format)
                    st["exp_avg_sq"] = torch.zeros_like(p, memory_format=torch.preserve_format)
            steps = torch.stack([self.state[p]["step"].to(dev, torch.float32).reshape(()) for p, _ in live])
            rec = np.zeros((n, 8), dtype=np.int64)
            unit, entries = 0, []
            for i, (p, gi) in enumerate(live):
                st = self.state[p]
                st["step"] = steps[i]
                rows, cols = (p.shape[0], p.numel() // p.shape[0]) if p.dim() >= 2 else (1, p.numel())
                tile = int(p.dim() == 2 and rows % 4 == 0 and cols % 4 == 0 and p.data_ptr() % 16 == 0
                           and st["exp_avg"].data_ptr() % 16 == 0 and st["exp_avg_sq"].data_ptr() % 16 == 0)
                dst = ops.cached_shadow(p, torch.bfloat16, False) if p.dim() == 2 else None
                dstT = ops.cached_shadow(p, torch.bfloat16, True) if tile else None
                rec[i, 0], rec[i, 1], rec[i, 2] = p.data_ptr(), st["exp_avg"].data_ptr(), st["exp_avg_sq"].data_ptr()
                rec[i, 3] = dst.data_ptr() if dst is not None else 0
                rec[i, 4] = dstT.data_ptr() if dstT is not None else 0
                rec[i, 5] = int(rows) | (int(cols) << 32)
                rec[i, 6] = int(gi) | (int(unit) << 32)
                rec[i, 7] = tile
                entries.append((p, dst, dstT))
                unit += L.focus_adamw_units(int(rows), int(cols), tile)
            tab = self._table = {"ident": ident, "items": torch.from_numpy(rec).pin_memory().to(dev, non_blocking=True),
                                 "units": unit, "steps": steps, "entries": entries, "tile": rec[:, 7].copy(),
                                 "gsig": None, "gptrs": None}
        grads = []
        for i, (p, _) in enumerate(live):
            g = p.grad
            if g.dtype != torch.float32 or not g.is_contiguous() or (tab["tile"][i] and g.data_ptr() % 16):
                p.grad = g = g.float().contiguous().clone() if tab["tile"][i] and g.data_ptr() % 16 else g.float().contiguous()
            grads.append(g.data_ptr())
        gsig = tuple(grads)
        if tab["gsig"] != gsig:
            tab["gsig"] = gsig
            tab["gptrs"] = torch.tensor(grads, dtype=torch.int64).pin_memory().to(dev, non_blocking=True)
        vals = tuple((float(g["lr"]), float(g["weight_decay"])) for g in self.param_groups)
        if self._groups is None or self._groups[0] != vals or self._groups[1].device != dev:
            self._groups = (vals, torch.tensor(vals, dtype=torch.float32).reshape(-1, 2).pin_memory().to(dev, non_blocking=True))
        if self._ws is None or self._ws.device != dev:
            self._ws = torch.empty(L.focus_adamw_workspace_bytes() // 4 + 1, dtype=torch.float32, device=dev)
        return dev

    @torch.no_grad()
    def step_clipped(self, max_norm=0.0, closure=None):
        import ctypes
        from focus_amd import _lib, ops
        loss = None
        if closure is not None:
            with torch.enable_grad():
                loss = closure()
        dev = self._prepare()
        if dev is None:
            return loss
        tab = self._table
        b1, b2 = self.param_groups[0]["betas"]
        eps = self.param_groups[0]["eps"]
        for g in self.param_groups[1:]:
            if tuple(g["betas"]) != (b1, b2) or g["eps"] != eps:
                raise NotImplementedError("FusedAdamW: one (betas, eps) for all groups")
        L = _lib.lib()
        vp = lambda t: ctypes.c_void_p(t.data_ptr())
        norm = self._ws[-1:]
        with torch.cuda.device(dev):
            _lib.check(L.focus_adamw_step(vp(tab["items"]), vp(tab["gptrs"]), len(tab["entries"]), tab["units"],
                                          vp(self._groups[1]), vp(tab["steps"]), vp(self._ws), (self._ws.numel() - 1) * 4,
                                          vp(norm), b1, b2, eps, float(max_norm or 0.0), int(self.write_clipped_grads),
                                          ctypes.c_void_p(torch.cuda.current_stream().cuda_stream)), "adamw_step")
        self.last_total_norm = norm[0]
        ops.shadows_written(tab["entries"])
        return loss

    def step(self, closure=None):
        return self.step_clipped(0.0, closure)


def construct_optimizer(model, cfg):
    skip = set()
    base = model.module if hasattr(model, "module") else model
    if hasattr(base, "no_weight_decay"):
        skip = base.no_weight_decay()
    decay, no_decay = [], []
    for name, p in base.named_parameters():
        if not p.requires_grad:
            continue
        if name in skip or (cfg.SOLVER.ZERO_WD_1D_PARAM and p.dim() == 1):
            no_decay.append(p)
        else:
            decay.append(p)
    groups = [{"params": decay, "weight_decay": cfg.SOLVER.WEIGHT_DECAY},
              {"params": no_decay, "weight_decay": 0.0}]
    assert len(decay) + len(no_decay) == len([p for p in base.parameters() if p.requires_grad])
    method = cfg.SOLVER.OPTIMIZING_METHOD
    if method == "adamw":
        on_gpu = all(p.is_cuda and p.dtype == torch.float32 for p in decay + no_decay)
        if on_gpu and os.environ.get("FOCUS_FUSED_OPT", "1") != "0":
            return FusedAdamW(groups, lr=cfg.SOLVER.BASE_LR, eps=1e-08)
# ... 38 lines not shown
```

### focus_amd/slowfast/models/stem_helper.py

```python
import torch.nn as nn
import torch.nn.functional as F

from focus_amd import ops


class PatchEmbed(nn.Module):
    def __init__(self, dim_in=3, dim_out=768, kernel=(1, 16, 16), stride=(1, 4, 4), padding=(1, 7, 7), conv_2d=False):
        super().__init__()
        if conv_2d:
            raise NotImplementedError("MVIT.PATCH_2D (image models) is not part of the video path")
        pads = list(padding) if hasattr(padding, "__iter__") else [padding] * 3
        self.patches = list(kernel) == list(stride) and all(p == 0 for p in pads)
        self.kernel = tuple(kernel)
        self.proj = nn.Conv3d(dim_in, dim_out, kernel_size=kernel, stride=stride, padding=padding)
        self.compute_dtype = None

    def forward(self, x):
        if not self.patches:
            y = F.conv3d(x.float(), self.proj.weight, self.proj.bias, self.proj.stride, self.proj.padding)
            return y.flatten(2).transpose(1, 2).to(self.compute_dtype or x.dtype).contiguous()
        kt, kh, kw = self.kernel
        B, Cin, T, H, W = x.shape
        cols = ops.im2col_patches(x, kt, kh, kw, self.compute_dtype or x.dtype)
        w = self.proj.weight.view(self.proj.weight.shape[0], -1)
        y = ops.linear(cols, w, self.proj.bias)
        return y.view(B, (T // kt) * (H // kh) * (W // kw), -1)
```

### include/focus_amd.h

```cpp
#ifndef FOCUS_AMD_H
#define FOCUS_AMD_H

#include <stddef.h>
#include <stdint.h>

#ifdef __cplusplus
extern "C" {
#endif

enum focus_dtype { FOCUS_F32 = 0, FOCUS_BF16 = 1, FOCUS_FP8_E4M3 = 2  };

enum focus_status {
    FOCUS_OK = 0,
    FOCUS_ERR_SHAPE = -1,
    FOCUS_ERR_DTYPE = -2,
    FOCUS_ERR_ALIGN = -3,
    FOCUS_ERR_LAUNCH = -4,
    FOCUS_ERR_NULL = -5,
    FOCUS_ERR_WORKSPACE = -6
};

const char* focus_strerror(int status);
int focus_abi_version(void);

// ... 19 lines not shown
    float alpha;
    int32_t accumulate;
    int32_t epilogue;
    int32_t dtype_ab;
    int32_t dtype_c;
    int32_t dtype_b;
    int32_t pad_;
    const float* b_scale;
} focus_gemm_desc;

int focus_gemm(const focus_gemm_desc* desc, void* stream);

enum focus_gemm_kernel {
    FOCUS_GEMM_KERNEL_GENERIC = 0,
    FOCUS_GEMM_KERNEL_NT = 1,
    FOCUS_GEMM_KERNEL_NT_WS = 2,
    FOCUS_GEMM_KERNEL_TN = 3,
    FOCUS_GEMM_KERNEL_NT_SMALL = 4,
    FOCUS_GEMM_KERNEL_NT_MX = 5
};
int focus_gemm_last_kernel(void);

int focus_gemm_tile_override(int bm);

int focus_mx_quant(const void* x, int64_t ldx, int rows, int cols, int dtype, void* codes, int64_t ld_codes, void* scales,
                   int64_t ld_scales, void* stream);

int focus_gemm_mx(const focus_gemm_desc* desc, const void* a_scales, int64_t ld_a_scales, void* stream);

size_t focus_gemm_tn_workspace_bytes(int M, int N, int K);
size_t focus_gemm_tn_batched_workspace_bytes(int M, int N, int K, int batch);

size_t focus_linear_wgrad_workspace_bytes(int N, int K, int M);
int focus_linear_wgrad(const void* dy, const void* x, float* dw, float* db, void* ws, size_t ws_bytes, int M, int N,
                       int K, int64_t ld_dy, int64_t ld_x, int dtype, void* stream);

int focus_linear_fwd(const void* x, const void* w, const float* bias, const void* residual, void* y,
                     void* aux, int M, int N, int K, int epilogue, int dtype, void* stream);

int focus_colsum(const void* x, float* out, int M, int N, int64_t row_stride, int accumulate, int dtype,
                 void* stream);

int focus_layernorm_fwd(const void* x, const float* gamma, const float* beta, void* y, float* mean,
                        float* rstd, int rows, int D, float eps, int dtype, void* stream);
int focus_layernorm_bwd_blocks(int rows);
int focus_layernorm_bwd(const void* dy, const void* x, const float* gamma, const float* mean,
                        const float* rstd, const void* dres, void* dx, float* dgamma, float* dbeta, float* partial,
                        int rows, int D, int dtype, void* stream);
int focus_layernorm_fwd_blocks(const void* x, int rows_per_block, int64_t block_stride, const float* gamma,
                               const float* beta, void* y, float* mean, float* rstd, int rows, int D, float eps, int dtype,
                               void* stream);
int focus_layernorm_bwd_blocks_strided(const void* dy, const void* x, int rows_per_block, int64_t block_stride,
                                       const float* gamma, const float* mean, const float* rstd, void* dx, float* dgamma,
                                       float* dbeta, float* partial, int rows, int D, int dtype, void* stream);

int focus_softmax_fwd(const void* x, void* y, int64_t rows, int L, int64_t stride, float scale, int dtype,
                      void* stream);
int focus_softmax_bwd(const void* dy, const void* y, void* dx, int64_t rows, int L, int64_t stride,
                      float scale, int dtype, void* stream);
int focus_softmax_causal_fwd(const void* x, void* y, int64_t rows, int L, int64_t stride, int period, float scale,
                             int dtype, void* stream);

size_t focus_traj_space_workspace_bytes(int B, int F, int P, int heads, int d, int dtype, int backward);
int focus_traj_space_fwd(const void* qkv, void* xt, void* xdiag, void* cls_out, float* lse, float* cls_lse,
                         void* workspace, size_t workspace_bytes, int B, int F, int P, int heads, int d,
                         int dtype, void* stream);
int focus_traj_space_bwd(const void* qkv, const void* xt, const void* cls_out, const float* lse,
                         const float* cls_lse, const void* dxt, const void* dxdiag, const void* dcls,
                         void* dqkv, void* workspace, size_t workspace_bytes, int B, int F, int P,
                         int heads, int d, int dtype, void* stream);
int focus_traj_time_fwd(const void* q2, const void* k2, const void* xt, void* out, int64_t out_bstride, float* attn2,
                        int B, int S, int F, int heads, int d, int dtype, void* stream);
int focus_traj_time_bwd(const void* q2, const void* k2, const void* xt, const float* attn2, const void* dout,
                        int64_t dout_bstride, void* dq2, void* dk2, void* dxt, int dxt_accumulate, int B, int S, int F,
                        int heads, int d, int dtype, void* stream);

size_t focus_traj_time2_workspace_bytes(int B, int S, int F, int heads, int d);
int focus_traj_time2_fwd(const void* q2, const void* xt, const void* wkT, int64_t ldw, void* out, int64_t out_bstride,
                         float* attn2, void* ws, size_t ws_bytes, int B, int S, int F, int heads, int d, int dtype,
                         void* stream);
int focus_traj_time2_bwd(const void* q2, const void* xt, const void* wkT, int64_t ldw, const float* attn2,
                         const void* dout, int64_t dout_bstride, void* dxt, void* g, void* dl, int B, int S, int F,
                         int heads, int d, int dtype, void* stream);

int focus_roi_align_fwd(const void* feat, int64_t img_stride, int imgs_per_batch, int64_t batch_stride,
                        const float* rois, const int32_t* roi_img, void* out, int NI, int C, int H, int W, int K,
                        int PH, int PW, float spatial_scale, int sampling_ratio, int aligned, int relu, int dtype,
                        void* stream);
size_t focus_roi_align_bwd_workspace_bytes(int NI, int C, int H, int W, int PH, int PW);
int focus_roi_align_bwd(const void* dout, const void* relu_out, const float* rois, const int32_t* roi_img, void* dfeat, int64_t img_stride,
                        int imgs_per_batch, int64_t batch_stride, void* ws, size_t ws_bytes, int NI, int C, int H, int W, int K, int PH, int PW, float spatial_scale,
                        int sampling_ratio, int aligned, int dtype, void* stream);
int focus_roi_align_indices(const float* rois, int32_t* grid, int32_t* nbr, int H, int W, int K, int PH,
                            int PW, float spatial_scale, int sampling_ratio, int aligned, void* stream);

int focus_cell_amax_fwd(const void* x, void* y, int32_t* arg, int K, int cells, int C, int dtype,
                        void* stream);
int focus_cell_amax_bwd(const void* dy, const int32_t* arg, void* dx, int K, int cells, int C, int dtype,
                        void* stream);

int focus_orvit_assemble(const void* x, const void* obj, void* all, int B, int T, int HW, int O, int C, int dtype,
                         void* stream);
int focus_orvit_assemble_bwd(const void* dall, void* dx, void* dobj, int B, int T, int HW, int O, int C, int dtype,
                             void* stream);
int focus_orvit_merge(const void* x, const void* y, const void* mm, const float* scale, void* out, int B, int T, int HW,
                      int O, int C, int dtype, void* stream);
int focus_orvit_merge_bwd(const void* dout, const float* scale, void* dy, void* dmm, int B, int T, int HW, int O, int C,
                          int dtype, void* stream);

int focus_box_layout_fwd(const void* vecs, const float* boxes, void* out, int NF, int O, int C, int H,
                         int W, int dtype, void* stream);
int focus_box_layout_bwd(const void* dout, const float* boxes, void* dvecs, int NF, int O, int C, int H,
                         int W, int dtype, void* stream);

size_t focus_slot_attn_workspace_bytes(int B, int N, int K, int D);
int focus_slot_attn_fwd(const void* k_t, const void* v_t, int64_t kv_bstride, const void* q, void* attn_vis,
                        int64_t attn_bstride, void* upd, float* colsum, void* partial, size_t partial_bytes,
                        int B, int N, int K, int D, float eps, int dtype, void* stream);
int focus_slot_attn_bwd(const void* k_t, const void* v_t, int64_t kv_bstride, const void* q,
                        const void* attn_vis, int64_t attn_bstride, const float* colsum, const void* upd,
                        const void* dupd,
                        const void* dattn_vis, void* dk_t, void* dv_t, int accumulate, void* dq, void* partial,
                        size_t partial_bytes, int B, int N, int K, int D, float eps, int dtype, void* wl, void* stream);
int focus_slot_kv_grad_ok(int K, int D, int dtype, int iters);
int focus_slot_kv_grad(const void* wl0, const void* wl1, const void* wl2, const void* wl3, const void* q0, const void* q1,
                       const void* q2, const void* q3, const void* du0, const void* du1, const void* du2, const void* du3,
                       int iters, void* dk_t, void* dv_t, int64_t kv_bstride, int64_t kv_ld, int B, int N, int K, int D,
                       int dtype, void* stream);

int focus_small_attn_ok(int N, int M, int d);
int focus_small_attn_fwd(const void* q, const void* k, const void* v, int64_t ldq, int64_t ldk, int64_t ldv, void* att,
                         void* out, int B, int heads, int N, int M, int d, float scale, int dtype, void* stream);
int focus_small_attn_bwd(const void* q, const void* k, const void* v, int64_t ldq, int64_t ldk, int64_t ldv, const void* att,
                         const void* dout, void* dq, void* dk, void* dv, int B, int heads, int N, int M, int d, float scale,
                         int dtype, void* stream);

int focus_gru_gates_fwd(void* gi, void* gh, const void* h, void* hn, const float* b_ih, const float* b_hh, int R, int D,
                        int dtype, void* stream);
int focus_gru_gates_bwd(const void* gi, const void* gh, const void* h, const void* dhn, void* dgi, void* dgh,
                        void* dh, void* zero_out, int R, int D, int dtype, void* stream);

int focus_im2col_patches(const float* x, void* cols, int B, int Cin, int T, int H, int W, int kt, int kh,
                         int kw, int dtype, void* stream);

int focus_embed_assemble(const void* patch, const float* cls, const float* pos, const float* temp,
                         void* tokens, int B, int T, int P, int C, int dtype, void* stream);

int focus_xent_ls(const float* logits, const int64_t* target, float* loss_rows, float* dlogits, int R,
                  int Ncls, float smoothing, void* stream);

int focus_transpose_pad(const void* src, int src_dtype, int64_t src_ld, int64_t src_bstride, void* dst,
                        int dst_dtype, int64_t dst_ld, int64_t dst_bstride, int R, int Cc, int batch,
                        void* stream);

typedef struct focus_shadow_item {
    const float* src; void* dst; void* dstT;
    int32_t rows, cols;
} focus_shadow_item;
int focus_shadow_refresh(const focus_shadow_item* items, int n_items, int max_rows, int max_cols, void* stream);

typedef struct focus_adamw_item {
    float* p; float* m; float* v; void* dst; void* dstT;
    int32_t rows, cols, group, unit0, tile_mode, pad_;
} focus_adamw_item;
int focus_adamw_units(int rows, int cols, int tile_mode);
size_t focus_adamw_workspace_bytes(void);
int focus_adamw_step(const focus_adamw_item* items, float* const* grads, int n_items, int n_units, const float* groups, float* steps,
                     void* workspace, size_t workspace_bytes, float* total_norm, double beta1, double beta2, float eps,
                     float max_norm, int write_clipped_grads, void* stream);

typedef struct focus_fp8_item {
    const float* src; void* dst; void* dstT; float* scale;
    int32_t rows, cols;
} focus_fp8_item;
int focus_fp8_refresh(const focus_fp8_item* items, int n_items, int max_rows, int max_cols, void* amax_scratch, void* stream);

typedef struct focus_wgrad_item {
    const void* dy; const void* x; float* dw; float* db;
    int64_t ld_dy, ld_x;
    int32_t M, N, K, pad_;
} focus_wgrad_item;
int focus_linear_wgrad_group_units(const focus_wgrad_item* items, int n_items);
int focus_linear_wgrad_group_plan(const focus_wgrad_item* items, int n_items, void* host_units, size_t bytes);
int focus_linear_wgrad_group(const focus_wgrad_item* items, int n_items, const void* dev_units, void* stream);

typedef struct focus_slot_tail_args {
    int32_t R, D, H, do_gru, do_mlp, do_q;
    float ln1_eps, ln2_eps;
    const void* upd; const void* h;
    const void* w_ih; const void* w_hh; const float* b_ih; const float* b_hh;
    const float* ln1_g; const float* ln1_b; const void* w1; const float* b1; const void* w2; const float* b2;
    const float* ln2_g; const float* ln2_b; const void* wq;
    void* g; void* hn; void* y; float* mean1; float* rstd1; void* a; void* s;
    void* sn; float* mean2; float* rstd2; void* q;
} focus_slot_tail_args;
int focus_slot_tail_ok(int D, int H, int dtype);
int focus_slot_tail_fwd(const focus_slot_tail_args* args, void* stream);
typedef struct focus_slot_tail_bwd_args {
    int32_t R, D, H, do_gru, do_mlp, do_q;
    const void* dout; const void* dq;
    const void* h; const void* g; const void* hn; const void* a; const void* cur;
    const float* mean1; const float* rstd1; const float* mean2; const float* rstd2;
    const float* ln1_g; const float* ln2_g;
    const void* w_ih_t; const void* w_hh_t; const void* w1_t; const void* w2_t; const void* wq_t;
    void* dupd; void* dh; void* ds; void* dz; void* dg; float* part1; float* part2;
    void* ws_dsn; void* ws_dy1; void* ws_res;
} focus_slot_tail_bwd_args;
int focus_slot_tail_bwd_blocks(int R);
int focus_slot_tail_bwd(const focus_slot_tail_bwd_args* args, void* stream);

typedef struct focus_flash_args {
    const void* q; const void* k; const void* v; void* out; float* lse;
    const void* dout; float* delta; void* dq; void* dk; void* dv;
    const uint32_t* seed;
    int64_t ldq, ldk, ldv, ldo, lddo, lddq, lddk, lddv;
    int64_t bsq, bsk, bsv, bso, bsdo, bsdq, bsdk, bsdv;
    int32_t B, heads, Nq, Nk, d, dtype, causal;
    uint32_t drop_thr;
    float scale;
    int32_t pad_;
} focus_flash_args;
int focus_flash_attn_ok(int Nq, int Nk, int d, int dtype, int causal);
int focus_flash_attn_fwd(const focus_flash_args* args, void* stream);
int focus_flash_attn_bwd(const focus_flash_args* args, void* stream);

int focus_traj_time2_gw_ok(int R, int heads, int d, int dtype);
size_t focus_traj_time2_gw_workspace_bytes(int R, int heads, int d);
int focus_traj_time2_gw(const void* g, const void* q2, const void* wk, int64_t wk_ld, void* dq2, float* dwk, void* ws,
                        size_t ws_bytes, int R, int heads, int d, int dtype, void* stream);

int focus_rows_ok(int64_t R, int V, int dtype);
int focus_gumbel_fwd(const void* x, const float* e_soft, const float* e_hard, const void* seed, void* z, int64_t* target,
                     float* stats, int64_t R, int V, float tau, int hard, int dtype, int dtype_z, void* stream);
int focus_gumbel_bwd(const void* x, const float* e_soft, const void* seed, const float* stats, const void* dz, void* dx,
                     int64_t R, int V, float tau, int dtype, int dtype_z, void* stream);

int focus_xent_rows_fwd(const void* logits, const int64_t* target, float* loss_rows, float* lse, int64_t R, int V,
                        float smoothing, int dtype, void* stream);
int focus_xent_rows_bwd(const void* logits, const int64_t* target, const float* lse, const float* g, void* dlogits,
                        int64_t R, int V, float smoothing, int dtype, void* stream);

int focus_dropout_add(const void* y, const void* res, const void* seed, int thr, void* out, int64_t n, int dtype,
                      void* stream);

int focus_diag_gather(const void* xt, void* xdiag, int B, int S, int F, int C, int dtype, void* stream);
int focus_diag_scatter_add(const void* dxdiag, void* dxt, int B, int S, int F, int C, int dtype, void* stream);

int focus_scale_add(const void* x, const void* y, const float* scale, float keep, void* out, int B, int64_t per,
                    int dtype, void* stream);

int focus_cast(const void* src, int src_dtype, void* dst, int dst_dtype, int64_t n, void* stream);

#ifdef __cplusplus
}
#endif
#endif
```

Before: 299.3 clips/s.

## Fuse ORViT object-token glue: box MLP kernel, relu-amax, assemble with categories

Adds a dedicated fused kernel for the tiny 4-input box-coordinate MLP (two linears with ReLU) forward and backward, replacing several small GEMM and elementwise launches. Folds the ReLU into the cell-amax forward and backward, and fuses the category embedding and box-embedding add into the token assembly. Also extends bf16 shadow caching to higher-rank params and reuses the base weight for the stem projection, and declares new traj/time2 entry points. These cut launch count and intermediate tensors in the object branch, at the cost of more custom code paths that must match the reference rounding.

Result: slower. 212.3 clips/s (-29.1%).

```diff
diff --git a/focus_amd/csrc/box_mlp.hip b/focus_amd/csrc/box_mlp.hip
--- /dev/null
+++ b/focus_amd/csrc/box_mlp.hip
@@ -0,0 +1,219 @@
+#include "focus_common.h"
+
+namespace {
+
+constexpr int RT = 16;
+constexpr int KC = 32;
+constexpr int NT = 64;
+
+__device__ __forceinline__ float round_bf16(float v) { return bf16_to_f32(f32_to_bf16(v)); }
+
+__device__ __forceinline__ float pre1_of(const float4 xr, const float4 w0) {
+    float a = 0.f;
+    a = fmaf(xr.x, w0.x, a);
+    a = fmaf(xr.y, w0.y, a);
+    a = fmaf(xr.z, w0.z, a);
+    a = fmaf(xr.w, w0.w, a);
+    return a;
+}
+
+__device__ __forceinline__ float4 row_of(const float* __restrict__ x, int r, int R) {
+    return r < R ? *reinterpret_cast<const float4*>(x + (int64_t)r * 4) : make_float4(0.f, 0.f, 0.f, 0.f);
+}
+
+__global__ __launch_bounds__(256) void box_mlp_fwd_kernel(const float* __restrict__ x, const float* __restrict__ w0,
+                                                          const float* __restrict__ w1, bf16_t* __restrict__ out, int R,
+                                                          int H, int D) {
+    __shared__ float sW[NT][KC + 1];
+    __shared__ float sH[RT][KC];
+    const int t = threadIdx.x, col = t & 63, rg = t >> 6;
+    const int r0 = blockIdx.x * RT, n0 = blockIdx.y * NT;
+    float acc[4] = {0.f, 0.f, 0.f, 0.f};
+    for (int k0 = 0; k0 < H; k0 += KC) {
+        {
+            const int c = t >> 2, kq = (t & 3) * 8;
+            float wv[8];
+            ld8<float>(w1 + (int64_t)(n0 + c) * H + k0 + kq, wv);
+#pragma unroll
+            for (int e = 0; e < 8; ++e) sW[c][kq + e] = round_bf16(wv[e]);
+        }
+#pragma unroll
+        for (int i = 0; i < 2; ++i) {
+            const int idx = t + i * 256, rr = idx >> 5, kk = idx & 31;
+            const float4 xr = row_of(x, r0 + rr, R);
+            const float4 wr = *reinterpret_cast<const float4*>(w0 + (int64_t)(k0 + kk) * 4);
+            sH[rr][kk] = round_bf16(fmaxf(pre1_of(xr, wr), 0.f));
+        }
+        __syncthreads();
+#pragma unroll 8
+        for (int k = 0; k < KC; ++k) {
+            const float w = sW[col][k];
+#pragma unroll
+            for (int j = 0; j < 4; ++j) acc[j] = fmaf(sH[rg * 4 + j][k], w, acc[j]);
+        }
+        __syncthreads();
+    }
+#pragma unroll
+    for (int j = 0; j < 4; ++j) {
+        const int r = r0 + rg * 4 + j;
+        if (r < R) out[(int64_t)r * D + n0 + col] = f32_to_bf16(fmaxf(acc[j], 0.f));
+    }
+}
+
+__global__ __launch_bounds__(256) void box_mlp_bwd_hid_kernel(const float* __restrict__ x, const float* __restrict__ w0,
+                                                              const float* __restrict__ w1, const bf16_t* __restrict__ out,
+                                                              const bf16_t* __restrict__ dout, float* __restrict__ part,
+                                                              int R, int H, int D) {
+    __shared__ float sD[RT][NT];
+    __shared__ float sW[NT][KC + 1];
+    __shared__ float sP[RT][KC + 1];
+    const int t = threadIdx.x, hc = t & 31, rp = t >> 5;
+    const int r0 = blockIdx.x * RT, h0 = blockIdx.y * KC;
+    float acc[2] = {0.f, 0.f};
+    for (int n0 = 0; n0 < D; n0 += NT) {
+        {
+            const int c = t >> 2, hq = (t & 3) * 8;
+            float wv[8];
+            ld8<float>(w1 + (int64_t)(n0 + c) * H + h0 + hq, wv);
+#pragma unroll
+            for (int e = 0; e < 8; ++e) sW[c][hq + e] = round_bf16(wv[e]);
+        }
+        {
+            const int rr = t >> 4, c4 = (t & 15) * 4;
+            f4 g = {0.f, 0.f, 0.f, 0.f};
+            if (r0 + rr < R) {
+                const int64_t off = (int64_t)(r0 + rr) * D + n0 + c4;
+                const f4 o = ld4<bf16_t>(out + off);
+                g = ld4<bf16_t>(dout + off);
+                g.x = o.x > 0.f ? g.x : 0.f; g.y = o.y > 0.f ? g.y : 0.f;
+                g.z = o.z > 0.f ? g.z : 0.f; g.w = o.w > 0.f ? g.w : 0.f;
+            }
+            sD[rr][c4] = g.x; sD[rr][c4 + 1] = g.y; sD[rr][c4 + 2] = g.z; sD[rr][c4 + 3] = g.w;
+        }
+        __syncthreads();
+#pragma unroll 8
+        for (int n = 0; n < NT; ++n) {
+            const float w = sW[n][hc];
+            acc[0] = fmaf(sD[rp * 2][n], w, acc[0]);
+            acc[1] = fmaf(sD[rp * 2 + 1][n], w, acc[1]);
+        }
+        __syncthreads();
+    }
+    const float4 wr = *reinterpret_cast<const float4*>(w0 + (int64_t)(h0 + hc) * 4);
+#pragma unroll
+    for (int j = 0; j < 2; ++j) {
+        const int rr = rp * 2 + j;
+        const float pre = pre1_of(row_of(x, r0 + rr, R), wr);
+        sP[rr][hc] = pre > 0.f ? round_bf16(acc[j]) : 0.f;
+    }
+    __syncthreads();
+    if (t < KC * 4) {
+        const int h = t >> 2, k = t & 3;
+        float s = 0.f;
+        for (int rr = 0; rr < RT; ++rr) {
+            const int r = r0 + rr;
+            const float xv = r < R ? x[(int64_t)r * 4 + k] : 0.f;
+            s = fmaf(sP[rr][h], xv, s);
+        }
+        part[((int64_t)blockIdx.x * H + h0 + h) * 4 + k] = s;
+    }
+}
+
+__global__ __launch_bounds__(256) void box_mlp_bwd_w_kernel(const float* __restrict__ x, const float* __restrict__ w0,
+                                                            const bf16_t* __restrict__ out, const bf16_t* __restrict__ dout,
+                                                            const float* __restrict__ part, float* __restrict__ dw0,
+                                                            float* __restrict__ dw1, int R, int H, int D, int tiles,
+                                                            int rtiles) {
+    const int t = threadIdx.x;
+    if ((int)blockIdx.x >= tiles) {
+        const int i = ((int)blockIdx.x - tiles) * 256 + t;
+        if (i < H * 4) {
+            float s = 0.f;
+            for (int k = 0; k < rtiles; ++k) s += part[(int64_t)k * H * 4 + i];
+            dw0[i] = s;
+        }
+        return;
+    }
+    __shared__ float sD[RT][NT];
+    __shared__ float sH[RT][KC];
+    const int ht = H / KC;
+    const int n0 = ((int)blockIdx.x / ht) * NT, h0 = ((int)blockIdx.x % ht) * KC;
+    const int hc = t & 31, ng = t >> 5;
+    float acc[8] = {0.f, 0.f, 0.f, 0.f, 0.f, 0.f, 0.f, 0.f};
+    for (int r0 = 0; r0 < R; r0 += RT) {
+        {
+            const int rr = t >> 4, c4 = (t & 15) * 4;
+            f4 g = {0.f, 0.f, 0.f, 0.f};
+            if (r0 + rr < R) {
+                const int64_t off = (int64_t)(r0 + rr) * D + n0 + c4;
+                const f4 o = ld4<bf16_t>(out + off);
+                g = ld4<bf16_t>(dout + off);
+                g.x = o.x > 0.f ? g.x : 0.f; g.y = o.y > 0.f ? g.y : 0.f;
+                g.z = o.z > 0.f ? g.z : 0.f; g.w = o.w > 0.f ? g.w : 0.f;
+            }
+            sD[rr][c4] = g.x; sD[rr][c4 + 1] = g.y; sD[rr][c4 + 2] = g.z; sD[rr][c4 + 3] = g.w;
+        }
+#pragma unroll
+        for (int i = 0; i < 2; ++i) {
+            const int idx = t + i * 256, rr = idx >> 5, kk = idx & 31;
+            const float4 xr = row_of(x, r0 + rr, R);
+            const float4 wr = *reinterpret_cast<const float4*>(w0 + (int64_t)(h0 + kk) * 4);
+            sH[rr][kk] = round_bf16(fmaxf(pre1_of(xr, wr), 0.f));
+        }
+        __syncthreads();
+#pragma unroll 4
+        for (int rr = 0; rr < RT; ++rr) {
+            const float hv = sH[rr][hc];
+#pragma unroll
+            for (int j = 0; j < 8; ++j) acc[j] = fmaf(sD[rr][ng * 8 + j], hv, acc[j]);
+        }
+        __syncthreads();
+    }
+#pragma unroll
+    for (int j = 0; j < 8; ++j) dw1[(int64_t)(n0 + ng * 8 + j) * H + h0 + hc] = acc[j];
+}
+
+inline bool box_shape_ok(int R, int H, int D) {
+    return R > 0 && H > 0 && D > 0 && H % KC == 0 && D % NT == 0 && (int64_t)R * D < (1LL << 31) && R <= (1 << 20);
+}
+
+}
+
+extern "C" int focus_box_mlp_ok(int R, int H, int D) { return box_shape_ok(R, H, D) ? 1 : 0; }
+
+extern "C" size_t focus_box_mlp_workspace_bytes(int R, int H, int D) {
+    if (!box_shape_ok(R, H, D)) return 0;
+    return (size_t)((R + RT - 1) / RT) * H * 4 * sizeof(float);
+}
+
+extern "C" int focus_box_mlp_fwd(const float* x, const float* w0, const float* w1, void* out, int R, int H, int D,
+                                 void* stream) {
+    if (!x || !w0 || !w1 || !out) return FOCUS_ERR_NULL;
+    if (!box_shape_ok(R, H, D)) return FOCUS_ERR_SHAPE;
+    if (!focus_aligned(x, 16) || !focus_aligned(w0, 16) || !focus_aligned(w1, 16) || !focus_aligned(out, 8))
+        return FOCUS_ERR_ALIGN;
+    hipLaunchKernelGGL(box_mlp_fwd_kernel, dim3((R + RT - 1) / RT, D / NT), dim3(256), 0, (hipStream_t)stream, x, w0, w1,
+                       (bf16_t*)out, R, H, D);
+    FOCUS_CHECK_LAUNCH();
+    return FOCUS_OK;
+}
+
+extern "C" int focus_box_mlp_bwd(const float* x, const float* w0, const float* w1, const void* out, const void* dout,
+                                 float* dw0, float* dw1, void* ws, size_t ws_bytes, int R, int H, int D, void* stream) {
+    if (!x || !w0 || !w1 || !out || !dout || !dw0 || !dw1 || !ws) return FOCUS_ERR_NULL;
+    if (!box_shape_ok(R, H, D)) return FOCUS_ERR_SHAPE;
+    if (!focus_aligned(x, 16) || !focus_aligned(w0, 16) || !focus_aligned(w1, 16) || !focus_aligned(out, 8) ||
+        !focus_aligned(dout, 8) || !focus_aligned(ws, 16))
+        return FOCUS_ERR_ALIGN;
+    if (ws_bytes < focus_box_mlp_workspace_bytes(R, H, D)) return FOCUS_ERR_WORKSPACE;
+    hipStream_t s = (hipStream_t)stream;
+    const int rtiles = (R + RT - 1) / RT;
+    hipLaunchKernelGGL(box_mlp_bwd_hid_kernel, dim3(rtiles, H / KC), dim3(256), 0, s, x, w0, w1, (const bf16_t*)out,
+                       (const bf16_t*)dout, (float*)ws, R, H, D);
+    FOCUS_CHECK_LAUNCH();
+    const int tiles = (D / NT) * (H / KC);
+    hipLaunchKernelGGL(box_mlp_bwd_w_kernel, dim3(tiles + (H * 4 + 255) / 256), dim3(256), 0, s, x, w0, (const bf16_t*)out,
+                       (const bf16_t*)dout, (const float*)ws, dw0, dw1, R, H, D, tiles, rtiles);
+    FOCUS_CHECK_LAUNCH();
+    return FOCUS_OK;
+}
diff --git a/focus_amd/csrc/misc.hip b/focus_amd/csrc/misc.hip
--- a/focus_amd/csrc/misc.hip
+++ b/focus_amd/csrc/misc.hip
@@ -224,7 +224,7 @@
 
 template <typename T>
 __global__ void cell_amax_fwd_kernel(const T* __restrict__ x, T* __restrict__ y, int32_t* __restrict__ arg, int K,
-                                     int cells, int C) {
+                                     int cells, int C, int relu) {
     const int64_t i = (int64_t)blockIdx.x * blockDim.x + threadIdx.x;
     if (i >= (int64_t)K * C) return;
     const int64_t k = i / C;
@@ -236,11 +236,11 @@
         const float v = ld<T>(p + (int64_t)j * C);
         if (v > m) { m = v; a = j; }
     }
-    st<T>(y + i, m);
+    st<T>(y + i, relu && m <= 0.f ? 0.f : m);
     arg[i] = a;
 }
 __global__ __launch_bounds__(256) void cell_amax_fwd_vec_kernel(const bf16_t* __restrict__ x, bf16_t* __restrict__ y,
-                                                                int32_t* __restrict__ arg, int cells, int C) {
+                                                                int32_t* __restrict__ arg, int cells, int C, int relu) {
     __shared__ float sm[8][256];
     __shared__ int sa[8][256];
     const int k = blockIdx.y, cb = blockIdx.x * 256;
@@ -272,21 +272,23 @@
         const int va = sa[q][c];
         if (va != 0x7fffffff && (ba == 0x7fffffff || vm > bm || (vm == bm && va < ba))) { bm = vm; ba = va; }
     }
-    y[(int64_t)k * C + cb + c] = f32_to_bf16(bm);
+    y[(int64_t)k * C + cb + c] = f32_to_bf16(relu && bm <= 0.f ? 0.f : bm);
     arg[(int64_t)k * C + cb + c] = ba == 0x7fffffff ? 0 : ba;
 }
 template <typename T>
 __global__ void cell_amax_bwd_kernel(const T* __restrict__ dy, const int32_t* __restrict__ arg, T* __restrict__ dx,
-                                     int K, int cells, int C) {
+                                     int K, int cells, int C, const T* __restrict__ y) {
     const int64_t i = (int64_t)blockIdx.x * blockDim.x + threadIdx.x;
     if (i >= (int64_t)K * cells * C) return;
     const int c = (int)(i % C);
     const int j = (int)((i / C) % cells);
     const int64_t k = i / ((int64_t)C * cells);
-    st<T>(dx + i, arg[k * C + c] == j ? ld<T>(dy + k * C + c) : 0.f);
+    const bool on = arg[k * C + c] == j && (!y || ld<T>(y + k * C + c) > 0.f);
+    st<T>(dx + i, on ? ld<T>(dy + k * C + c) : 0.f);
 }
 __global__ __launch_bounds__(256) void cell_amax_bwd_vec_kernel(const bf16_t* __restrict__ dy, const int32_t* __restrict__ arg,
-                                                                bf16_t* __restrict__ dx, int64_t n8, int cells, int C) {
+                                                                bf16_t* __restrict__ dx, int64_t n8, int cells, int C,
+                                                                const bf16_t* __restrict__ y) {
     const int64_t i = (int64_t)blockIdx.x * 256 + threadIdx.x;
     if (i >= n8) return;
     const int c8 = C >> 3;
@@ -295,7 +297,15 @@
     const int64_t k = i / ((int64_t)c8 * cells);
     const int4 a0 = *reinterpret_cast<const int4*>(arg + k * C + cg * 8);
     const int4 a1 = *reinterpret_cast<const int4*>(arg + k * C + cg * 8 + 4);
-    const uint4 g = *reinterpret_cast<const uint4*>(dy + k * C + cg * 8);
+    uint4 g = *reinterpret_cast<const uint4*>(dy + k * C + cg * 8);
+    if (y) {
+        const uint4 yv = *reinterpret_cast<const uint4*>(y + k * C + cg * 8);
+        auto keep = [](uint32_t w) {
+            const uint32_t lo = w & 0xffffu, hi = w >> 16;
+            return ((lo - 1u) < 0x7f80u ? 0x0000ffffu : 0u) | ((hi - 1u) < 0x7f80u ? 0xffff0000u : 0u);
+        };
+        g.x &= keep(yv.x); g.y &= keep(yv.y); g.z &= keep(yv.z); g.w &= keep(yv.w);
+    }
     uint4 o;
     o.x = (a0.x == j ? (g.x & 0x0000ffffu) : 0u) | (a0.y == j ? (g.x & 0xffff0000u) : 0u);
     o.y = (a0.z == j ? (g.y & 0x0000ffffu) : 0u) | (a0.w == j ? (g.y & 0xffff0000u) : 0u);
@@ -491,37 +501,56 @@
     return FOCUS_OK;
 }
 
-extern "C" int focus_cell_amax_fwd(const void* x, void* y, int32_t* arg, int K, int cells, int C, int dtype,
-                                   void* stream) {
+static int cell_amax_fwd_impl(const void* x, void* y, int32_t* arg, int K, int cells, int C, int dtype, int relu,
+                              void* stream) {
     if (!x || !y || !arg) return FOCUS_ERR_NULL;
     if (cells <= 0) return FOCUS_ERR_SHAPE;
     if (K <= 0) return FOCUS_OK;
     if (dtype == FOCUS_BF16 && (C & 255) == 0 && K <= 65535 && focus_aligned(x, 16)) {
         hipLaunchKernelGGL(cell_amax_fwd_vec_kernel, dim3(C / 256, K), dim3(256), 0, (hipStream_t)stream, (const bf16_t*)x,
-                           (bf16_t*)y, arg, cells, C);
+                           (bf16_t*)y, arg, cells, C, relu);
         FOCUS_CHECK_LAUNCH();
         return FOCUS_OK;
     }
     DISPATCH_T(dtype, hipLaunchKernelGGL((cell_amax_fwd_kernel<T>), dim3(nblk((int64_t)K * C, 256)), dim3(256), 0,
-                                         (hipStream_t)stream, (const T*)x, (T*)y, arg, K, cells, C));
+                                         (hipStream_t)stream, (const T*)x, (T*)y, arg, K, cells, C, relu));
+    FOCUS_CHECK_LAUNCH();
+    return FOCUS_OK;
+}
+extern "C" int focus_cell_amax_fwd(const void* x, void* y, int32_t* arg, int K, int cells, int C, int dtype,
+                                   void* stream) {
+    return cell_amax_fwd_impl(x, y, arg, K, cells, C, dtype, 0, stream);
+}
+extern "C" int focus_cell_amax_relu_fwd(const void* x, void* y, int32_t* arg, int K, int cells, int C, int dtype,
+                                        void* stream) {
+    return cell_amax_fwd_impl(x, y, arg, K, cells, C, dtype, 1, stream);
+}
+static int cell_amax_bwd_impl(const void* dy, const void* y, const int32_t* arg, void* dx, int K, int cells, int C, int dtype,
+                              void* stream) {
+    if (!dy || !arg || !dx) return FOCUS_ERR_NULL;
+    if (K <= 0 || cells <= 0) return FOCUS_OK;
+    if (dtype == FOCUS_BF16 && (C & 7) == 0 && focus_aligned(dy, 16) && focus_aligned(dx, 16) && focus_aligned(arg, 16) &&
+        focus_aligned(y, 16)) {
+        const int64_t n8 = (int64_t)K * cells * (C >> 3);
+        hipLaunchKernelGGL(cell_amax_bwd_vec_kernel, dim3(nblk(n8, 256)), dim3(256), 0, (hipStream_t)stream,
+                           (const bf16_t*)dy, arg, (bf16_t*)dx, n8, cells, C, (const bf16_t*)y);
+        FOCUS_CHECK_LAUNCH();
+        return FOCUS_OK;
+    }
+    DISPATCH_T(dtype, hipLaunchKernelGGL((cell_amax_bwd_kernel<T>), dim3(nblk((int64_t)K * cells * C, 256)),
+                                         dim3(256), 0, (hipStream_t)stream, (const T*)dy, arg, (T*)dx, K, cells, C,
+                                         (const T*)y));
     FOCUS_CHECK_LAUNCH();
     return FOCUS_OK;
 }
 extern "C" int focus_cell_amax_bwd(const void* dy, const int32_t* arg, void* dx, int K, int cells, int C, int dtype,
                                    void* stream) {
-    if (!dy || !arg || !dx) return FOCUS_ERR_NULL;
-    if (K <= 0 || cells <= 0) return FOCUS_OK;
-    if (dtype == FOCUS_BF16 && (C & 7) == 0 && focus_aligned(dy, 16) && focus_aligned(dx, 16) && focus_aligned(arg, 16)) {
-        const int64_t n8 = (int64_t)K * cells * (C >> 3);
-        hipLaunchKernelGGL(cell_amax_bwd_vec_kernel, dim3(nblk(n8, 256)), dim3(256), 0, (hipStream_t)stream,
-                           (const bf16_t*)dy, arg, (bf16_t*)dx, n8, cells, C);
-        FOCUS_CHECK_LAUNCH();
-        return FOCUS_OK;
-    }
-    DISPATCH_T(dtype, hipLaunchKernelGGL((cell_amax_bwd_kernel<T>), dim3(nblk((int64_t)K * cells * C, 256)),
-                                         dim3(256), 0, (hipStream_t)stream, (const T*)dy, arg, (T*)dx, K, cells, C));
-    FOCUS_CHECK_LAUNCH();
-    return FOCUS_OK;
+    return cell_amax_bwd_impl(dy, nullptr, arg, dx, K, cells, C, dtype, stream);
+}
+extern "C" int focus_cell_amax_relu_bwd(const void* dy, const void* y, const int32_t* arg, void* dx, int K, int cells, int C,
+                                        int dtype, void* stream) {
+    if (!y) return FOCUS_ERR_NULL;
+    return cell_amax_bwd_impl(dy, y, arg, dx, K, cells, C, dtype, stream);
 }
 
 template <typename T>
diff --git a/focus_amd/csrc/orvit_tokens.hip b/focus_amd/csrc/orvit_tokens.hip
--- a/focus_amd/csrc/orvit_tokens.hip
+++ b/focus_amd/csrc/orvit_tokens.hip
@@ -55,6 +55,70 @@
     o.z = (uint32_t)f32_to_bf16(v[4]) | ((uint32_t)f32_to_bf16(v[5]) << 16);
     o.w = (uint32_t)f32_to_bf16(v[6]) | ((uint32_t)f32_to_bf16(v[7]) << 16);
     return o;
+}
+
+template <typename T> __device__ __forceinline__ float rnd(float v);
+template <> __device__ __forceinline__ float rnd<float>(float v) { return v; }
+template <> __device__ __forceinline__ float rnd<bf16_t>(float v) { return bf16_to_f32(f32_to_bf16(v)); }
+
+template <typename T>
+__global__ __launch_bounds__(256) void orvit_assemble_obj_kernel(const uint4* __restrict__ x, const uint4* __restrict__ obj,
+                                                                 const float* __restrict__ cat, const uint4* __restrict__ emb,
+                                                                 uint4* __restrict__ all, int64_t npieces, int vpr, int Tn,
+                                                                 int HW, int O) {
+    const int64_t i = (int64_t)blockIdx.x * 256 + threadIdx.x;
+    if (i >= npieces) return;
+    const int64_t r = i / vpr;
+    const int v = (int)(i - r * vpr);
+    const RowMap m = map_all_row(r, Tn, HW, O);
+    if (m.cls || m.p < HW) {
+        const int64_t xrow = (int64_t)m.b * (1 + Tn * HW) + (m.cls ? 0 : 1 + m.t * HW + m.p);
+        all[i] = x[xrow * vpr + v];
+        return;
+    }
+    constexpr int N = Vec<T>::N;
+    const int64_t orow = ((int64_t)m.b * Tn + m.t) * O + (m.p - HW);
+    const int64_t crow = (int64_t)m.t * O + (m.p - HW);
+    float ov[N], ev[N];
+    unpack<T>(obj[orow * vpr + v], ov);
+    unpack<T>(emb[orow * vpr + v], ev);
+    const float* c = cat + (crow * vpr + v) * N;
+#pragma unroll
+    for (int e = 0; e < N; ++e) ov[e] = rnd<T>(ov[e] + rnd<T>(c[e])) + ev[e];
+    all[i] = pack<T>(ov);
+}
+
+template <typename T>
+__global__ __launch_bounds__(256) void orvit_assemble_obj_bwd_kernel(const uint4* __restrict__ dall, uint4* __restrict__ dx,
+                                                                     uint4* __restrict__ dobj, float* __restrict__ dcat,
+                                                                     int64_t npieces, int vpr, int B, int Tn, int HW, int O) {
+    const int64_t i = (int64_t)blockIdx.x * 256 + threadIdx.x;
+    constexpr int N = Vec<T>::N;
+    if (i >= npieces) {
+        const int64_t j = i - npieces;
+        if (j >= (int64_t)Tn * O * vpr) return;
+        const int64_t crow = j / vpr;
+        const int v = (int)(j - crow * vpr);
+        const int t = (int)(crow / O), o = (int)(crow - (int64_t)t * O);
+        const int64_t per = 1 + (int64_t)Tn * (HW + O);
+        float s[N];
+#pragma unroll
+        for (int e = 0; e < N; ++e) s[e] = 0.f;
+        for (int b = 0; b < B; ++b) {
+            float g[N];
+            unpack<T>(dall[(b * per + 1 + (int64_t)t * (HW + O) + HW + o) * vpr + v], g);
+#pragma unroll
+            for (int e = 0; e < N; ++e) s[e] += g[e];
+        }
+#pragma unroll
+        for (int e = 0; e < N; ++e) dcat[j * N + e] = s[e];
+        return;
+    }
+    const int64_t r = i / vpr;
+    const int v = (int)(i - r * vpr);
+    const RowMap m = map_all_row(r, Tn, HW, O);
+    if (!m.cls && m.p >= HW) dobj[(((int64_t)m.b * Tn + m.t) * O + (m.p - HW)) * vpr + v] = dall[i];
+    else dx[((int64_t)m.b * (1 + Tn * HW) + (m.cls ? 0 : 1 + m.t * HW + m.p)) * vpr + v] = dall[i];
 }
 
 template <typename T>
@@ -146,6 +210,45 @@
     return FOCUS_OK;
 }
 
+extern "C" int focus_orvit_assemble_obj(const void* x, const void* obj, const float* cat, const void* emb, void* all, int B,
+                                        int T, int HW, int O, int C, int dtype, void* stream) {
+    if (!x || !all || !obj || !cat || !emb) return FOCUS_ERR_NULL;
+    if (!shape_ok(B, T, HW, O, C, dtype) || O <= 0) return FOCUS_ERR_SHAPE;
+    if (!focus_aligned(x, 16) || !focus_aligned(all, 16) || !focus_aligned(obj, 16) || !focus_aligned(emb, 16) ||
+        !focus_aligned(cat, 16))
+        return FOCUS_ERR_ALIGN;
+    const int vpr = C * esize(dtype) / 16;
+    const int64_t n = (int64_t)B * (1 + (int64_t)T * (HW + O)) * vpr;
+    const dim3 grid((unsigned)cdiv(n, 256));
+    if (dtype == FOCUS_BF16)
+        hipLaunchKernelGGL((orvit_assemble_obj_kernel<bf16_t>), grid, dim3(256), 0, (hipStream_t)stream, (const uint4*)x,
+                           (const uint4*)obj, cat, (const uint4*)emb, (uint4*)all, n, vpr, T, HW, O);
+    else
+        hipLaunchKernelGGL((orvit_assemble_obj_kernel<float>), grid, dim3(256), 0, (hipStream_t)stream, (const uint4*)x,
+                           (const uint4*)obj, cat, (const uint4*)emb, (uint4*)all, n, vpr, T, HW, O);
+    FOCUS_CHECK_LAUNCH();
+    return FOCUS_OK;
+}
+
+extern "C" int focus_orvit_assemble_obj_bwd(const void* dall, void* dx, void* dobj, float* dcat, int B, int T, int HW, int O,
+                                            int C, int dtype, void* stream) {
+    if (!dall || !dx || !dobj || !dcat) return FOCUS_ERR_NULL;
+    if (!shape_ok(B, T, HW, O, C, dtype) || O <= 0) return FOCUS_ERR_SHAPE;
+    if (!focus_aligned(dall, 16) || !focus_aligned(dx, 16) || !focus_aligned(dobj, 16) || !focus_aligned(dcat, 16))
+        return FOCUS_ERR_ALIGN;
+    const int vpr = C * esize(dtype) / 16;
+    const int64_t n = (int64_t)B * (1 + (int64_t)T * (HW + O)) * vpr;
+    const dim3 grid((unsigned)cdiv(n + (int64_t)T * O * vpr, 256));
+    if (dtype == FOCUS_BF16)
+        hipLaunchKernelGGL((orvit_assemble_obj_bwd_kernel<bf16_t>), grid, dim3(256), 0, (hipStream_t)stream, (const uint4*)dall,
+                           (uint4*)dx, (uint4*)dobj, dcat, n, vpr, B, T, HW, O);
+    else
+        hipLaunchKernelGGL((orvit_assemble_obj_bwd_kernel<float>), grid, dim3(256), 0, (hipStream_t)stream, (const uint4*)dall,
+                           (uint4*)dx, (uint4*)dobj, dcat, n, vpr, B, T, HW, O);
+    FOCUS_CHECK_LAUNCH();
+    return FOCUS_OK;
+}
+
 extern "C" int focus_orvit_merge(const void* x, const void* y, const void* mm, const float* scale, void* out, int B, int T,
                                  int HW, int O, int C, int dtype, void* stream) {
     if (!x || !y || !out) return FOCUS_ERR_NULL;
diff --git a/focus_amd/csrc/traj_time2.hip b/focus_amd/csrc/traj_time2.hip
--- a/focus_amd/csrc/traj_time2.hip
+++ b/focus_amd/csrc/traj_time2.hip
@@ -452,9 +452,21 @@
 template <int FT>
 __global__ __launch_bounds__(256) void time2_out_kernel(const bf16_t* __restrict__ xt, const float* __restrict__ attn2,
                                                         bf16_t* __restrict__ out, int64_t obs, int64_t ngroups, int S,
-                                                        int heads) {
+                                                        int heads, const bf16_t* __restrict__ cls, int64_t cls_bs,
+                                                        int64_t ncls) {
     const int64_t gi = (int64_t)blockIdx.x * 256 + threadIdx.x;
     const bool act = gi < ngroups;
+    if (!act && cls != nullptr) {
+        const int64_t j = gi - ngroups;
+        if (j < ncls) {
+            const int gpr_ = heads * 8;
+            const int64_t b_ = j / gpr_;
+            const int c_ = (int)(j - b_ * gpr_) * 8;
+            *reinterpret_cast<uint4*>(out + b_ * obs - (int64_t)gpr_ * 8 + c_) =
+                *reinterpret_cast<const uint4*>(cls + b_ * cls_bs + c_);
+        }
+        return;
+    }
     const int64_t g = act ? gi : ngroups - 1;
     const int gpr = heads * 8;
     const int row = (int)(g / gpr);
@@ -890,9 +902,9 @@
     return (size_t)heads * B * heads * S * F * sizeof(float);
 }
 
-extern "C" int focus_traj_time2_fwd(const void* q2, const void* xt, const void* wkT, int64_t ldw, void* out,
-                                    int64_t out_bstride, float* attn2, void* ws, size_t ws_bytes, int B, int S, int F,
-                                    int heads, int d, int dtype, void* stream) {
+static int time2_fwd_impl(const void* q2, const void* xt, const void* wkT, int64_t ldw, void* out, int64_t out_bstride,
+                          float* attn2, void* ws, size_t ws_bytes, int B, int S, int F, int heads, int d, int dtype,
+                          const void* cls, int64_t cls_bstride, void* stream) {
     if (!q2 || !xt || !wkT || !out || !attn2 || !ws) return FOCUS_ERR_NULL;
     if (B <= 0 || S <= 0 || !focus_traj_time2_ok(F, heads, d, dtype)) return FOCUS_ERR_SHAPE;
     const int C = heads * CH;
@@ -930,12 +942,32 @@
 #undef TS
     FOCUS_CHECK_LAUNCH();
     const int64_t ng = rows * heads * 8;
-    dim3 gv((unsigned)cdiv64(ng, 256));
-#define TO(FT) hipLaunchKernelGGL((time2_out_kernel<FT>), gv, dim3(256), 0, s, (const bf16_t*)xt, attn2, (bf16_t*)out, out_bstride, ng, S, heads)
+    const int64_t ncls = cls ? (int64_t)B * heads * 8 : 0;
+    dim3 gv((unsigned)cdiv64(ng + ncls, 256));
+#define TO(FT) hipLaunchKernelGGL((time2_out_kernel<FT>), gv, dim3(256), 0, s, (const bf16_t*)xt, attn2, (bf16_t*)out, out_bstride, ng, S, heads, (const bf16_t*)cls, cls_bstride, ncls)
     if (F == 8) TO(8); else if (F == 4) TO(4); else TO(16);
 #undef TO
     FOCUS_CHECK_LAUNCH();
     return FOCUS_OK;
+}
+
+extern "C" int focus_traj_time2_fwd(const void* q2, const void* xt, const void* wkT, int64_t ldw, void* out,
+                                    int64_t out_bstride, float* attn2, void* ws, size_t ws_bytes, int B, int S, int F,
+                                    int heads, int d, int dtype, void* stream) {
+    return time2_fwd_impl(q2, xt, wkT, ldw, out, out_bstride, attn2, ws, ws_bytes, B, S, F, heads, d, dtype, nullptr, 0,
+                          stream);
+}
+
+extern "C" int focus_traj_time2_fwd_cls(const void* q2, const void* xt, const void* wkT, int64_t ldw, const void* cls,
+                                        int64_t cls_bstride, void* out, int64_t out_bstride, float* attn2, void* ws,
+                                        size_t ws_bytes, int B, int S, int F, int heads, int d, int dtype, void* stream) {
+    if (!cls || !out) return FOCUS_ERR_NULL;
+    if (heads <= 0 || d <= 0) return FOCUS_ERR_SHAPE;
+    const int64_t C = (int64_t)heads * d;
+    if (cls_bstride < C || (cls_bstride & 7) || out_bstride < (int64_t)(S + 1) * C) return FOCUS_ERR_SHAPE;
+    if (!focus_aligned(cls, 16)) return FOCUS_ERR_ALIGN;
+    return time2_fwd_impl(q2, xt, wkT, ldw, (bf16_t*)out + C, out_bstride, attn2, ws, ws_bytes, B, S, F, heads, d, dtype,
+                          cls, cls_bstride, stream);
 }
 
 extern "C" int focus_traj_time2_bwd(const void* q2, const void* xt, const void* wkT, int64_t ldw, const float* attn2,
diff --git a/focus_amd/csrc/traj_time2_gw.hip b/focus_amd/csrc/traj_time2_gw.hip
--- a/focus_amd/csrc/traj_time2_gw.hip
+++ b/focus_amd/csrc/traj_time2_gw.hip
@@ -128,9 +128,12 @@
 }
 
 __global__ __launch_bounds__(256) void time2_gw_reduce_kernel(const float* __restrict__ slabs, float* __restrict__ dwk, int64_t n4,
-                                                              int splits) {
+                                                              int splits, int64_t z4) {
     const int64_t i = (int64_t)blockIdx.x * 256 + threadIdx.x;
-    if (i >= n4) return;
+    if (i >= n4) {
+        if (i < n4 + z4) reinterpret_cast<float4*>(dwk)[i] = make_float4(0.f, 0.f, 0.f, 0.f);
+        return;
+    }
     float4 s = reinterpret_cast<const float4*>(slabs)[i];
 #pragma unroll 4
     for (int k = 1; k < splits; ++k) {
@@ -156,8 +159,8 @@
     return (size_t)gw_splits(R, heads) * C_ * C_ * sizeof(float);
 }
 
-extern "C" int focus_traj_time2_gw(const void* g, const void* q2, const void* wk, int64_t wk_ld, void* dq2, float* dwk, void* ws,
-                                   size_t ws_bytes, int R, int heads, int d, int dtype, void* stream) {
+static int time2_gw_impl(const void* g, const void* q2, const void* wk, int64_t wk_ld, void* dq2, float* dwk, void* ws,
+                         size_t ws_bytes, int R, int heads, int d, int dtype, int64_t zero_tail, void* stream) {
     if (!g || !q2 || !wk || !dq2 || !dwk || !ws) return FOCUS_ERR_NULL;
     if (!focus_traj_time2_gw_ok(R, heads, d, dtype) || (wk_ld & 7)) return FOCUS_ERR_SHAPE;
     if (!focus_aligned(g, 16) || !focus_aligned(q2, 16) || !focus_aligned(wk, 16) || !focus_aligned(dwk, 16)) return FOCUS_ERR_ALIGN;
@@ -174,7 +177,21 @@
                        (bf16_t*)dq2, (float*)ws, R, heads, tps);
     FOCUS_CHECK_LAUNCH();
     const int64_t n4 = (int64_t)C_ * C_ / 4;
-    hipLaunchKernelGGL(time2_gw_reduce_kernel, dim3((unsigned)cdiv64(n4, 256)), dim3(256), 0, s, (const float*)ws, dwk, n4, used);
+    const int64_t z4 = zero_tail / 4;
+    hipLaunchKernelGGL(time2_gw_reduce_kernel, dim3((unsigned)cdiv64(n4 + z4, 256)), dim3(256), 0, s, (const float*)ws, dwk, n4, used,
+                       z4);
     FOCUS_CHECK_LAUNCH();
     return FOCUS_OK;
 }
+
+extern "C" int focus_traj_time2_gw(const void* g, const void* q2, const void* wk, int64_t wk_ld, void* dq2, float* dwk, void* ws,
+                                   size_t ws_bytes, int R, int heads, int d, int dtype, void* stream) {
+    return time2_gw_impl(g, q2, wk, wk_ld, dq2, dwk, ws, ws_bytes, R, heads, d, dtype, 0, stream);
+}
+
+extern "C" int focus_traj_time2_gw_full(const void* g, const void* q2, const void* wk, int64_t wk_ld, void* dq2, float* dwk,
+                                        int64_t zero_tail, void* ws, size_t ws_bytes, int R, int heads, int d, int dtype,
+                                        void* stream) {
+    if (zero_tail < 0 || (zero_tail & 3)) return FOCUS_ERR_SHAPE;
+    return time2_gw_impl(g, q2, wk, wk_ld, dq2, dwk, ws, ws_bytes, R, heads, d, dtype, zero_tail, stream);
+}
diff --git a/focus_amd/ops.py b/focus_amd/ops.py
--- a/focus_amd/ops.py
+++ b/focus_amd/ops.py
@@ -139,6 +139,8 @@
 
 import os as _os
 
+FUSED_GLUE = _os.environ.get("FOCUS_FUSED_GLUE", "1") != "0"
+
 
 def wgrad_async(dy, x, want_bias):
     dw, db = linear_wgrad(dy, x, want_bias)
@@ -277,7 +279,8 @@
 def shadow(w, dtype, transposed=False):
     w = getattr(w, "_focus_base", w)
     if dtype == torch.float32 and not transposed:
-        return w.detach()
+        wd = w.detach()
+        return wd.reshape(wd.shape[0], -1) if wd.dim() > 2 else wd
     key = (id(w), dtype, transposed)
     hit = _shadow_cache.get(key)
     if hit is not None and hit[0]() is w and hit[1] == (w._version, w.data_ptr(), _shadow_gen):
@@ -289,7 +292,7 @@
         _lib.check(_lib.lib().focus_transpose_pad(_p(wd), _dt(wd), K, 0, _p(out), _dt(out), N, 0, N, K, 1, _stream()),
                    "shadow^T")
     else:
-        out = cast(wd, dtype)
+        out = cast(wd.reshape(wd.shape[0], -1) if wd.dim() > 2 else wd, dtype)
     global _shadow_epoch
     _shadow_epoch += 1
     _shadow_cache[key] = (weakref.ref(w, lambda _r, k=key: _shadow_cache.pop(k, None)),
@@ -1299,12 +1302,19 @@
         L = _lib.lib()
         wkT = shadow(w_kv, xt.dtype, transposed=True)
         out = torch.empty(B, S + 1, C, device=xt.device, dtype=xt.dtype)
-        out[:, 0].copy_(cls_out.reshape(B, C))
         attn2 = torch.empty(B, S, heads, F_, device=xt.device, dtype=torch.float32)
         nb = L.focus_traj_time2_workspace_bytes(B, S, F_, heads, d)
         ws = torch.empty(nb // 4, device=xt.device, dtype=torch.float32)
-        _lib.check(L.focus_traj_time2_fwd(_p(q2), _p(xt), _p(wkT), wkT.stride(0), _p(out, C), (S + 1) * C, _p(attn2),
-                                          _p(ws), nb, B, S, F_, heads, d, _dt(xt), _stream()), "traj_time2_fwd")
+        cls2 = cls_out.reshape(B, C)
+        if (FUSED_GLUE and cls2.dtype == xt.dtype and cls2.stride(1) == 1 and cls2.stride(0) % 8 == 0
+                and cls2.stride(0) >= C and cls2.data_ptr() % 16 == 0):
+            _lib.check(L.focus_traj_time2_fwd_cls(_p(q2), _p(xt), _p(wkT), wkT.stride(0), _p(cls2), cls2.stride(0), _p(out),
+                                                  (S + 1) * C, _p(attn2), _p(ws), nb, B, S, F_, heads, d, _dt(xt),
+                                                  _stream()), "traj_time2_fwd_cls")
+        else:
+            out[:, 0].copy_(cls2)
+            _lib.check(L.focus_traj_time2_fwd(_p(q2), _p(xt), _p(wkT), wkT.stride(0), _p(out, C), (S + 1) * C, _p(attn2),
+                                              _p(ws), nb, B, S, F_, heads, d, _dt(xt), _stream()), "traj_time2_fwd")
         ctx.save_for_backward(q2, xt, attn2, w_kv)
         ctx.heads, ctx.has_b, ctx.cls_shape = heads, b_kv is not None, cls_out.shape
         return out
@@ -1330,14 +1340,24 @@
                 and _os.environ.get("FOCUS_TIME2_GW", "1") != "0"):
             wk = shadow(w_kv, xt.dtype)
             dq2 = torch.empty(B, S, C, device=dev, dtype=xt.dtype)
-            dw = torch.empty(2 * C, C, device=dev, dtype=torch.float32)
             nbw = L.focus_traj_time2_gw_workspace_bytes(R, heads, d)
             wsw = torch.empty(nbw // 4, device=dev, dtype=torch.float32)
-            _lib.check(L.focus_traj_time2_gw(_p(g), _p(q2), _p(wk), wk.stride(0), _p(dq2), _p(dw), _p(wsw), nbw, R, heads, d,
-                                             _dt(xt), _stream()), "traj_time2_gw")
-            dw[C:].zero_()
-            if ctx.has_b and ctx.needs_input_grad[3]:
-                db = torch.zeros(2 * C, device=dev, dtype=torch.float32)
+            want_b = ctx.has_b and ctx.needs_input_grad[3]
+            if FUSED_GLUE:
+                buf = torch.empty(2 * C * C + (2 * C if want_b else 0), device=dev, dtype=torch.float32)
+                dw = buf[:2 * C * C].view(2 * C, C)
+                _lib.check(L.focus_traj_time2_gw_full(_p(g), _p(q2), _p(wk), wk.stride(0), _p(dq2), _p(buf),
+                                                      buf.numel() - C * C, _p(wsw), nbw, R, heads, d, _dt(xt), _stream()),
+                           "traj_time2_gw_full")
+                if want_b:
+                    db = buf[2 * C * C:]
+            else:
+                dw = torch.empty(2 * C, C, device=dev, dtype=torch.float32)
+                _lib.check(L.focus_traj_time2_gw(_p(g), _p(q2), _p(wk), wk.stride(0), _p(dq2), _p(dw), _p(wsw), nbw, R, heads,
+                                                 d, _dt(xt), _stream()), "traj_time2_gw")
+                dw[C:].zero_()
+                if want_b:
+                    db = torch.zeros(2 * C, device=dev, dtype=torch.float32)
             dcls = dcat[:, :1].reshape(ctx.cls_shape) if ctx.needs_input_grad[4] else None
             return dq2, dxt, dw, db, dcls, None
         if ctx.needs_input_grad[0]:
@@ -1622,6 +1642,38 @@
     return _OrvitAssembleFn.apply(x, obj, T, HW)
 
 
+class _OrvitAssembleObjFn(torch.autograd.Function):
+
+    @staticmethod
+    def forward(ctx, x, obj, cat, emb, T, HW):
+        _need_gpu(x, obj, cat, emb)
+        x, obj, emb, catd = x.contiguous(), obj.contiguous(), emb.contiguous(), cat.detach().contiguous()
+        B, _, C = x.shape
+        O = obj.shape[2]
+        assert x.shape[1] == 1 + T * HW and obj.shape == (B, T, O, C) and emb.shape == obj.shape
+        assert obj.dtype == x.dtype and emb.dtype == x.dtype and catd.dtype == torch.float32 and catd.shape == (T, O, C)
+        out = torch.empty(B, 1 + T * (HW + O), C, device=x.device, dtype=x.dtype)
+        _lib.check(_lib.lib().focus_orvit_assemble_obj(_p(x), _p(obj), _p(catd), _p(emb), _p(out), B, T, HW, O, C, _dt(x),
+                                                       _stream()), "orvit_assemble_obj")
+        ctx.args = (B, T, HW, O, C)
+        return out
+
+    @staticmethod
+    def backward(ctx, dall):
+        B, T, HW, O, C = ctx.args
+        dall = dall.contiguous()
+        dx = torch.empty(B, 1 + T * HW, C, device=dall.device, dtype=dall.dtype)
+        dobj = torch.empty(B, T, O, C, device=dall.device, dtype=dall.dtype)
+        dcat = torch.empty(T, O, C, device=dall.device, dtype=torch.float32)
+        _lib.check(_lib.lib().focus_orvit_assemble_obj_bwd(_p(dall), _p(dx), _p(dobj), _p(dcat), B, T, HW, O, C, _dt(dall),
+                                                           _stream()), "orvit_assemble_obj_bwd")
+        return dx, dobj, dcat, dobj, None, None
+
+
+def orvit_assemble_obj(x, obj, cat, emb, T, HW):
+    return _OrvitAssembleObjFn.apply(x, obj, cat, emb, T, HW)
+
+
 class _OrvitMergeFn(torch.autograd.Function):
 
     @staticmethod
@@ -1677,30 +1729,85 @@
 
 class _CellAmaxFn(torch.autograd.Function):
     @staticmethod
-    def forward(ctx, x):
+    def forward(ctx, x, relu):
         _need_gpu(x)
         x = x.contiguous()
         K, cells, C = x.shape
         y = torch.empty(K, C, device=x.device, dtype=x.dtype)
         arg = torch.empty(K, C, device=x.device, dtype=torch.int32)
-        _lib.check(_lib.lib().focus_cell_amax_fwd(_p(x), _p(y), _p(arg), K, cells, C, _dt(x), _stream()), "cell_amax")
-        ctx.save_for_backward(arg)
-        ctx.cells = cells
+        fn = _lib.lib().focus_cell_amax_relu_fwd if relu else _lib.lib().focus_cell_amax_fwd
+        _lib.check(fn(_p(x), _p(y), _p(arg), K, cells, C, _dt(x), _stream()), "cell_amax")
+        if relu:
+            ctx.save_for_backward(arg, y)
+        else:
+            ctx.save_for_backward(arg)
+        ctx.cells, ctx.relu = cells, relu
         return y
 
     @staticmethod
     def backward(ctx, dy):
-        (arg,) = ctx.saved_tensors
+        arg = ctx.saved_tensors[0]
         K, C = arg.shape
         dy = dy.contiguous()
         dx = torch.empty(K, ctx.cells, C, device=dy.device, dtype=dy.dtype)
-        _lib.check(_lib.lib().focus_cell_amax_bwd(_p(dy), _p(arg), _p(dx), K, ctx.cells, C, _dt(dy), _stream()),
-                   "cell_amax_bwd")
-        return dx
-
-
-def cell_amax(x):
-    return _CellAmaxFn.apply(x)
+        if ctx.relu:
+            _lib.check(_lib.lib().focus_cell_amax_relu_bwd(_p(dy), _p(ctx.saved_tensors[1]), _p(arg), _p(dx), K, ctx.cells, C,
+                                                           _dt(dy), _stream()), "cell_amax_relu_bwd")
+        else:
+            _lib.check(_lib.lib().focus_cell_amax_bwd(_p(dy), _p(arg), _p(dx), K, ctx.cells, C, _dt(dy), _stream()),
+                       "cell_amax_bwd")
+        return dx, None
+
+
+def cell_amax(x, relu=False):
+    return _CellAmaxFn.apply(x, bool(relu))
+
+
+class _BoxMlpFn(torch.autograd.Function):
+
+    @staticmethod
+    def forward(ctx, x, w0, w1):
+        _need_gpu(x, w0, w1)
+        x2 = x.reshape(-1, 4).contiguous()
+        w0d, w1d = w0.detach().contiguous(), w1.detach().contiguous()
+        R, (D, H) = x2.shape[0], w1d.shape
+        out = torch.empty(R, D, device=x.device, dtype=torch.bfloat16)
+        _lib.check(_lib.lib().focus_box_mlp_fwd(_p(x2), _p(w0d), _p(w1d), _p(out), R, H, D, _stream()), "box_mlp_fwd")
+        ctx.save_for_backward(x2, w0, w1, out)
+        ctx.set_materialize_grads(False)
+        return out.view(*x.shape[:-1], D)
+
+    @staticmethod
+    def backward(ctx, dout):
+        x2, w0, w1, out = ctx.saved_tensors
+        if dout is None:
+            return None, None, None
+        R, (D, H) = x2.shape[0], w1.shape
+        dout = dout.reshape(R, D).contiguous()
+        if dout.data_ptr() % 8:
+            dout = dout.clone()
+        L = _lib.lib()
+        dw0 = torch.empty(H, 4, device=out.device, dtype=torch.float32)
+        dw1 = torch.empty(D, H, device=out.device, dtype=torch.float32)
+        nb = L.focus_box_mlp_workspace_bytes(R, H, D)
+        ws = torch.empty(nb // 4, device=out.device, dtype=torch.float32)
+        _lib.check(L.focus_box_mlp_bwd(_p(x2), _p(w0.detach().contiguous()), _p(w1.detach().contiguous()), _p(out), _p(dout),
+                                       _p(dw0), _p(dw1), _p(ws), nb, R, H, D, _stream()), "box_mlp_bwd")
+        return None, dw0, dw1
+
+
+def box_mlp_ok(x, w0, w1, dtype):
+    if not FUSED_GLUE or dtype != torch.bfloat16 or x.dtype != torch.float32 or x.shape[-1] != 4:
+        return False
+    if w0.dtype != torch.float32 or w1.dtype != torch.float32 or w0.dim() != 2 or w1.dim() != 2:
+        return False
+    if w0.shape[1] != 4 or w1.shape[1] != w0.shape[0] or x.numel() == 0:
+        return False
+    return bool(_lib.lib().focus_box_mlp_ok(x.numel() // 4, w0.shape[0], w1.shape[0]))
+
+
+def box_mlp(x, w0, w1):
+    return _BoxMlpFn.apply(x, w0, w1)
 
 
 class _BoxLayoutFn(torch.autograd.Function):
diff --git a/focus_amd/slowfast/models/ORViT/orvit.py b/focus_amd/slowfast/models/ORViT/orvit.py
--- a/focus_amd/slowfast/models/ORViT/orvit.py
+++ b/focus_amd/slowfast/models/ORViT/orvit.py
@@ -23,7 +23,10 @@
 
 
 def _relu_pair(seq, x, dtype=None):
-    hid = torch.relu(ops.linear(x.float(), seq[0].weight))
+    x = x.float()
+    if dtype is not None and x.is_cuda and ops.box_mlp_ok(x, seq[0].weight, seq[2].weight, dtype):
+        return ops.box_mlp(x, seq[0].weight, seq[2].weight)
+    hid = torch.relu(ops.linear(x, seq[0].weight))
     if dtype is not None and dtype != hid.dtype:
         hid = hid.to(dtype)
     return torch.relu(ops.linear(hid, seq[2].weight))
@@ -123,11 +126,16 @@
             else:
                 crops = self.crop_layer.crop_stream(x, box_tensors, T, H, W)
                 pre = ops.mlp(crops, p2d[0].weight, None, p2d[2].weight, None, act=ops.EPI_RELU)
-        obj = torch.relu(ops.cell_amax(pre)).view(BS, T, O, d)
-        box_emb = _relu_pair(self.c_coord_to_feature, box_tensors, x.dtype)
-        obj = obj + self.box_categories.to(x.dtype) + box_emb
-
-        all_tokens = ops.orvit_assemble(x, obj, T, HW)
+        cat = self.box_categories
+        if ops.FUSED_GLUE and x.is_cuda and cat.dtype == torch.float32 and cat.shape == (T, O, d):
+            obj = ops.cell_amax(pre, relu=True).view(BS, T, O, d)
+            box_emb = _relu_pair(self.c_coord_to_feature, box_tensors, x.dtype)
+            all_tokens = ops.orvit_assemble_obj(x, obj, cat, box_emb.to(x.dtype), T, HW)
+        else:
+            obj = torch.relu(ops.cell_amax(pre)).view(BS, T, O, d)
+            box_emb = _relu_pair(self.c_coord_to_feature, box_tensors, x.dtype)
+            obj = obj + cat.to(x.dtype) + box_emb
+            all_tokens = ops.orvit_assemble(x, obj, T, HW)
         n1 = self.norm1
         y, _ = self.attn(ops.layer_norm(all_tokens, n1.weight, n1.bias, n1.eps), [T, HW + O, 1])
         mm = None
diff --git a/focus_amd/slowfast/models/optimizer.py b/focus_amd/slowfast/models/optimizer.py
--- a/focus_amd/slowfast/models/optimizer.py
+++ b/focus_amd/slowfast/models/optimizer.py
@@ -52,7 +52,7 @@
                 rows, cols = (p.shape[0], p.numel() // p.shape[0]) if p.dim() >= 2 else (1, p.numel())
                 tile = int(p.dim() == 2 and rows % 4 == 0 and cols % 4 == 0 and p.data_ptr() % 16 == 0
                            and st["exp_avg"].data_ptr() % 16 == 0 and st["exp_avg_sq"].data_ptr() % 16 == 0)
-                dst = ops.cached_shadow(p, torch.bfloat16, False) if p.dim() == 2 else None
+                dst = ops.cached_shadow(p, torch.bfloat16, False) if p.dim() >= 2 else None
                 dstT = ops.cached_shadow(p, torch.bfloat16, True) if tile else None
                 rec[i, 0], rec[i, 1], rec[i, 2] = p.data_ptr(), st["exp_avg"].data_ptr(), st["exp_avg_sq"].data_ptr()
                 rec[i, 3] = dst.data_ptr() if dst is not None else 0
diff --git a/focus_amd/slowfast/models/stem_helper.py b/focus_amd/slowfast/models/stem_helper.py
--- a/focus_amd/slowfast/models/stem_helper.py
+++ b/focus_amd/slowfast/models/stem_helper.py
@@ -23,5 +23,7 @@
         B, Cin, T, H, W = x.shape
         cols = ops.im2col_patches(x, kt, kh, kw, self.compute_dtype or x.dtype)
         w = self.proj.weight.view(self.proj.weight.shape[0], -1)
+        if not ops.FP8_WEIGHTS:
+            w._focus_base = self.proj.weight
         y = ops.linear(cols, w, self.proj.bias)
         return y.view(B, (T // kt) * (H // kh) * (W // kw), -1)
diff --git a/include/focus_amd.h b/include/focus_amd.h
--- a/include/focus_amd.h
+++ b/include/focus_amd.h
@@ -125,6 +125,9 @@
 int focus_traj_time2_bwd(const void* q2, const void* xt, const void* wkT, int64_t ldw, const float* attn2,
                          const void* dout, int64_t dout_bstride, void* dxt, void* g, void* dl, int B, int S, int F,
                          int heads, int d, int dtype, void* stream);
+int focus_traj_time2_fwd_cls(const void* q2, const void* xt, const void* wkT, int64_t ldw, const void* cls,
+                             int64_t cls_bstride, void* out, int64_t out_bstride, float* attn2, void* ws, size_t ws_bytes,
+                             int B, int S, int F, int heads, int d, int dtype, void* stream);
 
 int focus_roi_align_fwd(const void* feat, int64_t img_stride, int imgs_per_batch, int64_t batch_stride,
                         const float* rois, const int32_t* roi_img, void* out, int NI, int C, int H, int W, int K,
@@ -137,15 +140,28 @@
 int focus_roi_align_indices(const float* rois, int32_t* grid, int32_t* nbr, int H, int W, int K, int PH,
                             int PW, float spatial_scale, int sampling_ratio, int aligned, void* stream);
 
+int focus_box_mlp_ok(int R, int H, int D);
+size_t focus_box_mlp_workspace_bytes(int R, int H, int D);
+int focus_box_mlp_fwd(const float* x, const float* w0, const float* w1, void* out, int R, int H, int D, void* stream);
+int focus_box_mlp_bwd(const float* x, const float* w0, const float* w1, const void* out, const void* dout, float* dw0,
+                      float* dw1, void* ws, size_t ws_bytes, int R, int H, int D, void* stream);
+
 int focus_cell_amax_fwd(const void* x, void* y, int32_t* arg, int K, int cells, int C, int dtype,
                         void* stream);
 int focus_cell_amax_bwd(const void* dy, const int32_t* arg, void* dx, int K, int cells, int C, int dtype,
                         void* stream);
+int focus_cell_amax_relu_fwd(const void* x, void* y, int32_t* arg, int K, int cells, int C, int dtype, void* stream);
+int focus_cell_amax_relu_bwd(const void* dy, const void* y, const int32_t* arg, void* dx, int K, int cells, int C,
+                             int dtype, void* stream);
 
 int focus_orvit_assemble(const void* x, const void* obj, void* all, int B, int T, int HW, int O, int C, int dtype,
                          void* stream);
 int focus_orvit_assemble_bwd(const void* dall, void* dx, void* dobj, int B, int T, int HW, int O, int C, int dtype,
                              void* stream);
+int focus_orvit_assemble_obj(const void* x, const void* obj, const float* cat, const void* emb, void* all, int B, int T,
+                             int HW, int O, int C, int dtype, void* stream);
+int focus_orvit_assemble_obj_bwd(const void* dall, void* dx, void* dobj, float* dcat, int B, int T, int HW, int O, int C,
+                                 int dtype, void* stream);
 int focus_orvit_merge(const void* x, const void* y, const void* mm, const float* scale, void* out, int B, int T, int HW,
                       int O, int C, int dtype, void* stream);
 int focus_orvit_merge_bwd(const void* dout, const float* scale, void* dy, void* dmm, int B, int T, int HW, int O, int C,
@@ -271,6 +287,8 @@
 size_t focus_traj_time2_gw_workspace_bytes(int R, int heads, int d);
 int focus_traj_time2_gw(const void* g, const void* q2, const void* wk, int64_t wk_ld, void* dq2, float* dwk, void* ws,
                         size_t ws_bytes, int R, int heads, int d, int dtype, void* stream);
+int focus_traj_time2_gw_full(const void* g, const void* q2, const void* wk, int64_t wk_ld, void* dq2, float* dwk,
+                             int64_t zero_tail, void* ws, size_t ws_bytes, int R, int heads, int d, int dtype, void* stream);
 
 int focus_rows_ok(int64_t R, int V, int dtype);
 int focus_gumbel_fwd(const void* x, const float* e_soft, const float* e_hard, const void* seed, void* z, int64_t* target,
```
